# Atticuszz/GsplatLoc

Hardware: AMD Instinct MI355X
Metric: Gaussians/s fwd+bwd @1M splats 1200x680 (higher is better)
Workload: dtype f32

## Files before the change

gsplatloc_amd/_lib.py:

```python
from __future__ import annotations

import ctypes
import os
import subprocess
from ctypes import c_char_p, c_double, c_float, c_int, c_int64, c_size_t, c_void_p
from typing import Optional

_HERE = os.path.dirname(os.path.abspath(__file__))
_LIB_PATH = os.path.join(_HERE, "libgsloc_hip.so")
_lib: Optional[ctypes.CDLL] = None

P = c_void_p

_SIGNATURES = {
    "gsl_version": (c_char_p, []),
    "gsl_status_string": (c_char_p, [c_int]),
    "gsl_dev_poison_lds": (c_int, [ctypes.c_uint32, P]),
    "gsl_dev_tile_sort_launches": (c_int64, [c_int]),
    "gsl_project_fwd": (c_int, [P, P, P, P, P, c_int, c_int, c_int, c_float, c_float, c_float, c_float,
                                P, P, P, P, P, P]),
    "gsl_project_bwd_ws_bytes": (c_size_t, [c_int]),
    "gsl_project_bwd": (c_int, [P, P, P, P, P, c_int, c_int, c_int, c_float, P, P, P, P, P, P, P, P, P, P, P,
                                P, c_size_t, P]),
    "gsl_project_packed_ws_bytes": (c_size_t, [c_int, c_int]),
# ... 45 lines not shown
    "gsl_map_pose_align_batch": (c_int, [P, c_int64, P, c_int, c_float, c_float, c_float, c_float, P, c_int, c_int,
                                         c_float, c_float, c_float, c_float, c_int, c_double, c_int, c_double, c_double,
                                         c_double, c_double, P, P, P, P, P]),
    "gsl_map_photo_intensity": (c_int, [P, c_int, c_int, P, P]),
    "gsl_map_info_photo_max_rows": (c_int64, [c_float, c_float, c_float, c_float, c_int, c_int, c_float, c_float,
                                              c_float]),
    "gsl_map_pose_info_photo": (c_int, [P, c_int64, P, c_float, c_float, c_float, c_float, P, c_int, c_int, c_float,
                                        c_float, c_float, c_float, P, P, P, c_float, c_float, P, P]),
    "gsl_map_pose_align_photo": (c_int, [P, c_int64, P, c_float, c_float, c_float, c_float, P, c_int, c_int, c_float,
                                         c_float, c_float, c_float, c_int, c_double, c_int, c_double, c_double, c_double,
                                         c_double, P, P, P, P, P, P, c_float, c_float, P]),
    "gsl_map_pose_align_batch_photo": (c_int, [P, c_int64, P, c_int, c_float, c_float, c_float, c_float, P, c_int, c_int,
                                               c_float, c_float, c_float, c_float, c_int, c_double, c_int, c_double,
                                               c_double, c_double, c_double, P, P, P, P, P, P, c_float, c_float, P]),
    "gsl_map_pyramid_floats": (c_int64, [c_int, c_int, c_int]),
    "gsl_map_pyramid": (c_int, [P, P, c_int, c_int, c_int, c_float, P, P, P]),
    "gsl_map_place_cells": (c_int, []),
    "gsl_map_place_describe": (c_int, [P, c_int, c_int, P, P]),
    "gsl_map_place_match": (c_int, [P, P, c_int, P, P]),
    "gsl_map_refine": (c_int, [P, P, P, c_int64, P, c_float, c_float, c_float, c_float, c_float, c_float, c_float, P, P,
                               c_int, c_int, c_float, c_float, c_int, P, P]),
    "gsl_map_correct": (c_int, [P, P, c_int64, P, c_int, P, P]),
    "gsl_map_covis": (c_int, [P, P, c_int64, P, c_float, c_float, c_float, c_float, P, c_int, c_int, c_float, c_float,
                              c_float, c_int, P, P, P]),
    "gsl_sh_fwd": (c_int, [c_int, P, P, P, c_int, c_int, P, P]),
    "gsl_sh_bwd": (c_int, [c_int, P, P, P, c_int, c_int, P, P, P, P]),
    "gsl_isect_ws_bytes": (c_size_t, [c_int]),
    "gsl_isect_count": (c_int, [P, P, c_int, c_int, c_int, c_int, c_int, c_int, P, P, P, P, c_size_t, P]),
    "gsl_isect_fill": (c_int, [P, P, P, c_int, c_int, c_int, c_int, c_int, c_int, c_int, c_int, P, c_int64,
                               P, P, P, P, c_size_t, P]),
    "gsl_tile_sort": (c_int, [P, c_int, c_int, c_int64, P, P, P, c_int64, P]),
    "gsl_fused_ws_bytes": (c_size_t, [c_int, c_int]),
    "gsl_fused_project": (c_int, [P, P, P, P, P, c_int, c_int, P, P, c_int, c_int, c_int, c_float, c_float, c_float,
                                  c_float, c_int, c_int, c_int, c_int, c_int, P, P, P, P, P, P, P, P, P, c_size_t,
                                  P, P, c_int, P, P, P]),
    "gsl_fused_bin": (c_int, [P, P, c_int, c_int, c_int, c_int, c_int, c_int, P, c_int64, P, P, P, P, c_size_t, c_int,
                              P, c_int, P, P, c_int, P, P, P]),
    "gsl_fused_bin_clear": (c_int, [P, P, c_int, c_int, c_int, c_int, c_int, c_int, P, c_int64, P, P, P, P, c_size_t, c_int,
                                    P, c_int, P, P, c_int, P, P, P, P]),
    "gsl_fused_clear_rows": (c_int, [P, c_int, P]),
    "gsl_long_sort": (c_int, [P, c_int, c_int, c_int, c_int, c_int64, P, c_int, P, P, c_int, P, c_size_t, c_int, c_int, P,
                              P]),
    "gsl_fused_raster_fwd": (c_int, [P, P, P, c_int, c_int, c_int, c_int, c_int, c_int, c_int, c_int, P, P, c_int64,
                                     P, P, P, c_int, c_int, P, P, P, P, c_int, P, c_int, P, P, P, P]),
    "gsl_fused_raster_bwd": (c_int, [P, P, P, c_int, c_int, c_int, c_int, c_int, c_int, c_int, c_int, P, P, c_int64,
                                     P, P, P, P, P, P, c_int, c_int, P, P, P, P, c_int, P, P]),
    "gsl_long_ws_bytes": (c_size_t, [c_int]),
    "gsl_long_segment": (c_int, []),
    "gsl_long_sort_segment": (c_int, []),
    "gsl_long_raster_fwd": (c_int, [P, P, P, c_int, c_int, c_int, c_int, c_int, c_int, c_int, c_int, P, P, c_int64,
                                    P, P, P, c_int, c_int, P, P, c_int, P, c_size_t, c_int, c_int, P]),
    "gsl_long_raster_bwd": (c_int, [P, P, P, c_int, c_int, c_int, c_int, c_int, c_int, c_int, c_int, P, P, c_int64,
                                    P, P, P, P, P, P, c_int, c_int, P, P, c_int, P, c_int, P]),
    "gsl_loss_ws_bytes": (c_size_t, [c_int, c_int]),
    "gsl_loss_n_partials": (c_int, [c_int, c_int, c_int, c_int]),
    "gsl_tracking_loss": (c_int, [P, c_int, P, c_int, c_int, c_int, c_int, c_float, c_float, P, P, P, P, c_size_t,
                                  P]),
    "gsl_pose_init": (c_int, [P, P, P, c_float, c_float, P, P, P]),
    "gsl_normal_ws_bytes": (c_size_t, [c_int, c_int]),
    "gsl_normal_loss": (c_int, [P, c_int, P, c_int, c_int, c_int, c_int, c_float, c_float, c_float, c_float, c_float,
                                P, P, P, c_size_t, P]),
    "gsl_fused_viewmat_rows": (P, [P, c_int]),
    "gsl_pose_step": (c_int, [P, P, P, P, c_int, P, P, c_int, P, P, P, c_int, c_int, c_float, c_float, c_float, c_double, c_double,
                              c_float, c_float, c_float, c_double, c_int, c_int, c_int, c_int, P, P, P, P]),
    "gsl_pack_pose_reduce": (c_int, [P, P, c_int, P, P, P, c_int, P, P, P]),
    "gsl_photo_ws_bytes": (c_size_t, [c_int, c_int]),
    "gsl_photo_loss": (c_int, [P, c_int, P, c_int, c_int, c_float, c_float, P, P, P, c_size_t, P]),
    "gsl_pose_step_photo": (c_int, [P, P, P, P, c_int, P, P, c_int, P, P, P, c_int, c_int, c_float, c_float, c_float,
                                    c_double, c_double, c_float, c_float, c_float, c_double, c_int, c_int, c_int, c_int,
                                    P, P, P, P, P, c_float, c_float]),
    "gsl_pose_step_best": (c_int, [P, P, P, P, c_int, P, P, c_int, P, P, P, c_int, c_int, c_float, c_float, c_float,
                                   c_double, c_double, c_float, c_float, c_float, c_double, c_int, c_int, c_int, c_int,
                                   P, P, P, P, P, c_float, c_float, P]),
    "gsl_knn_ws_bytes": (c_size_t, [c_int]),
    "gsl_knn_cells": (c_int, []),
    "gsl_knn_count": (c_int, [P, c_int, P, P, c_size_t, P]),
    "gsl_knn_query": (c_int, [P, c_int, P, P, c_int, P, P, c_size_t, P]),
    "gsl_fused_project_bwd": (c_int, [P, P, P, P, P, c_int, c_int, P, P, c_int, c_int, c_int, c_float, c_int, c_int,
                                      P, P, P, P, P, P, P, P, P, P, P, c_size_t, c_int, P, P, P, P, c_int, c_int,
                                      c_int, c_int, c_int64, P, P, c_int, P, P]),
    "gsl_fused_project_bwd_keep": (c_int, [P, P, P, P, P, c_int, c_int, P, P, c_int, c_int, c_int, c_float, c_int, c_int,
                                           P, P, P, P, P, P, P, P, P, P, P, c_size_t, c_int, P, P, P, P, c_int, c_int,
                                           c_int, c_int, c_int64, P, P, c_int, P, P]),
    "gsl_tiny_raster_bwd": (c_int, [P, P, P, c_int, c_int, c_int, c_int, c_int, c_int, c_int, c_int, P, P, c_int64,
                                    P, P, P, P, P, P, P, c_int, c_int, P, c_int, P, c_float, c_float, P, P, P]),
    "gsl_isect_emit": (c_int, [P, P, P, P, c_int, c_int, c_int, c_int, c_int, c_int, c_int, P, P, P]),
    "gsl_isect_offsets": (c_int, [P, c_int64, c_int, c_int, c_int, P, P]),
    "gsl_rasterize_fwd": (c_int, [P, P, P, P, P, c_int, c_int, c_int, c_int, c_int, c_int, c_int, c_int, P, P,
                                  c_int64, P, P, P, P, P]),
    "gsl_vacc_bytes": (c_size_t, [c_int, c_int]),
    "gsl_rasterize_bwd": (c_int, [P, P, P, P, P, c_int, c_int, c_int, c_int, c_int, c_int, c_int, c_int, P, P,
                                  c_int64, P, P, P, P, P, P, P]),
    "gsl_vacc_unpack": (c_int, [P, c_int, c_int, P, P, P, P, P]),
    "gsl_fused_absgrad": (c_int, [P, P, P, c_int, c_int, c_int, c_int, c_int, c_int, P, P, c_int64, P, P, P, P, P, P,
                                  P, P, P]),
    "gsl_rasterize_absgrad": (c_int, [P, P, P, P, P, c_int, c_int, c_int, c_int, c_int, c_int, P, P, c_int64, P, P,
                                      P, P, P, P, P]),
}


def library_path() -> str:
    return _LIB_PATH


def exported_symbols():
    return sorted(_SIGNATURES)


def build_library(force: bool = False, verbose: bool = False) -> str:
    csrc = os.path.join(_HERE, "csrc")
    cmd = ["make", "-C", csrc, "-j", str(min(8, os.cpu_count() or 1)), "all"]
    if force:
        subprocess.run(["make", "-C", csrc, "clean"], check=True, capture_output=not verbose)
    res = subprocess.run(cmd, capture_output=True, text=True)
    if verbose or res.returncode != 0:
        print(res.stdout)
        print(res.stderr)
    if res.returncode != 0:
        raise RuntimeError("building libgsloc_hip.so failed:\n" + res.stderr[-4000:])
    return _LIB_PATH


def load_library() -> ctypes.CDLL:
    global _lib
    if _lib is not None:
        return _lib
    if not os.path.exists(_LIB_PATH):
        raise RuntimeError(
            f"{_LIB_PATH} not found: the HIP extension is required (no CPU fallback). "
            "Run `python -c 'import __graft_entry__ as g; g.build()'` or `make -C gsplatloc_amd/csrc`."
        )
    lib = ctypes.CDLL(_LIB_PATH)
    for name, (res, args) in _SIGNATURES.items():
        fn = getattr(lib, name)
        fn.restype = res
        fn.argtypes = args
    _lib = lib
    return lib


def check(status: int, what: str) -> None:
    if status != 0:
        msg = load_library().gsl_status_string(status).decode()
        raise RuntimeError(f"{what} failed: {msg} (status {status})")


def ptr(t) -> Optional[int]:
    return None if t is None else t.data_ptr()


def current_stream() -> int:
    import torch

    raw = getattr(torch._C, "_cuda_getCurrentRawStream", None)
    if raw is not None:
        return raw(torch.cuda.current_device())
    return torch.cuda.current_stream().cuda_stream
```

gsplatloc_amd/context.py:

```python
from __future__ import annotations

import math
import os
from typing import Dict, Optional, Tuple

import torch
from torch import Tensor

from . import stages
from ._lib import check, current_stream, load_library, ptr
from .stages import _MODES, MAX_STRIP_TILES, alloc_records, tile_n_bits


LONG_MIN = 2048
BIN_BYTES_MAX = 2 << 30
TINY_RCULL_MAX = 1.999
TINY_MAX_N = 400_000
FP16_EPS2D_MIN = 2e-5


class RenderContext:
    def __init__(self, N: int, width: int, height: int, render_mode: str = "RGB+ED", sh_degree: Optional[int] = 1,
                 K_sh: int = 4, device="cuda", eps2d: float = 0.3, near_plane: float = 0.01, far_plane: float = 1e10,
                 radius_clip: float = 0.0, antialiased: bool = False, tile_rows: Optional[Tuple[int, int]] = None,
                 capacity: Optional[int] = None, full_grads: bool = True,
                 pixel_rows: Optional[Tuple[int, int]] = None, staging: str = "fp32", deterministic: bool = False,
                 sort_in_forward: bool = False, reorder: Optional[bool] = None):
        if staging == "fp16" and not float(eps2d) >= FP16_EPS2D_MIN:
            raise ValueError(f"staging='fp16' needs eps2d >= {FP16_EPS2D_MIN} (got {eps2d}): the conic of a degenerate "
                             f"splat reaches 1/eps2d, and the half records end at 65504")
        self.lib = load_library()
        self.reorder = reorder
        self.order_ids = self.storage_of = None
        self._placed = None
        self._placed_key = None
        self._placed_src = None
        self.sort_in_forward = bool(sort_in_forward)
        self.N, self.W, self.H = int(N), int(width), int(height)
        self.mode = render_mode
        self.D, self.ed = _MODES[render_mode]
        self.rgb = self.D >= 3
        self.sh_degree = -1 if sh_degree is None else int(sh_degree)
        self.K_sh = int(K_sh) if (self.rgb and self.sh_degree >= 0) else 0
        self.eps2d, self.near, self.far, self.radius_clip = float(eps2d), float(near_plane), float(far_plane), float(radius_clip)
        self.antialiased = bool(antialiased)
        self.tw, self.th = (self.W + 15) // 16, (self.H + 15) // 16
        self.n_tiles = self.tw * self.th
        self.ty0, self.ty1 = tile_rows if tile_rows is not None else (0, self.th)
        assert 0 <= self.ty0 <= self.ty1 <= self.th
        assert (self.ty1 - self.ty0) * self.tw <= MAX_STRIP_TILES, "strip too large for the LDS tile histogram"
        lo, hi = self.ty0 * 16, min(self.ty1 * 16, self.H)
        self.row0, self.row1 = pixel_rows if pixel_rows is not None else (lo, hi)
        assert lo <= self.row0 <= self.row1 <= hi or self.ty0 == self.ty1, (pixel_rows, tile_rows)
        self.full_grads = bool(full_grads)
        dev = torch.device(device)
        self.device = dev
        f32, i32 = torch.float32, torch.int32
        N = self.N
        self.radii = torch.zeros(N, dtype=i32, device=dev)
        self.Q0, self.Q1, self.Q2 = alloc_records(N, self.rgb, dev, zero=True)
        assert staging in ("fp32", "fp16"), staging
        self.staging = staging
        self.Qh = torch.zeros(N, 8, dtype=i32, device=dev) if staging == "fp16" else None
        self.deterministic = bool(deterministic)
        self.vrow = None
        self.comps = torch.zeros(N, dtype=f32, device=dev) if self.antialiased else None
        self.offs = torch.zeros(self.n_tiles + 1, dtype=i32, device=dev)
        self.status = torch.zeros(8, dtype=i32, device=dev)
        self.n_is = self.status[4:5]
        self.hit_counts = torch.zeros(4 * self.n_tiles + 1, dtype=i32, device=dev)
        self.ws_bytes = self.lib.gsl_fused_ws_bytes(N, self.n_tiles)
        self.ws = torch.zeros(self.ws_bytes, dtype=torch.uint8, device=dev)
        self.render = torch.zeros(self.H, self.W, self.D, dtype=f32, device=dev)
        self.alphas = torch.zeros(self.H, self.W, 1, dtype=f32, device=dev)
        self.last_ids = torch.zeros(self.H, self.W, dtype=i32, device=dev)
        self.vacc = torch.zeros(N, 16, dtype=f32, device=dev)
        self._rows_dirty = False
        self._sort_cleared = False
        self.v_viewmat = torch.zeros(4, 4, dtype=f32, device=dev)
        if self.full_grads:
            self.v_means = torch.zeros(N, 3, dtype=f32, device=dev)
            self.v_quats = torch.zeros(N, 4, dtype=f32, device=dev)
            self.v_scales = torch.zeros(N, 3, dtype=f32, device=dev)
            self.v_opacities = torch.zeros(N, dtype=f32, device=dev)
            if self.rgb:
                shape = (N, self.K_sh, 3) if self.sh_degree >= 0 else (N, 3)
                self.v_colors = torch.zeros(*shape, dtype=f32, device=dev)
                self.vc_state = torch.ones(1, dtype=i32, device=dev)
            else:
                self.v_colors = None
        else:
            self.v_means = self.v_quats = self.v_scales = self.v_opacities = self.v_colors = None
        if not hasattr(self, "vc_state"):
            self.vc_state = None
        self.capacity = 0
        self.tiny = False
        self.flags = self.status[0:4]
        self.last_n_isects = 0
        self.tiles_per_gauss = None
        self.record_hits = True
        self.generation = 0
        self.bins, self.bin_cap = None, 0
        self._counters_dirty = False
        self._hits_valid = False
        self.trec = self.vcT = None
        self.long_min, self.max_seg, self.long_ws, self.long_ws_bytes, self.long_passes = 0, 0, None, 0, 0
        self._mean_list = 0.0
        self.keys = self.flatten_ids = self.hits = None
        if capacity is not None:
            self._alloc_isects(int(capacity))
        self._inputs = None

    def _alloc_isects(self, capacity: int) -> None:
        self.capacity = max(int(capacity), 1)
        self.keys = torch.zeros(self.capacity, dtype=torch.int64, device=self.device)
        self.flatten_ids = torch.zeros(self.capacity, dtype=torch.int32, device=self.device)
        self.hits = (torch.zeros(4 * self.capacity, dtype=torch.int32, device=self.device)
                     if self.capacity < (1 << 28) else None)
        if self.deterministic:
            self.vrow = torch.zeros(self.capacity, 16, dtype=torch.float32, device=self.device)

    def calibrate(self, means, quats, scales, opacities, colors, viewmat, K, headroom: float = 1.3) -> int:
        self.bins, self.bin_cap = None, 0
        self.order_ids = self.storage_of = self._placed = self._placed_key = self._placed_src = None
        self._project(means, quats, scales, opacities, colors, viewmat, K)
        if self._choose_placement():
            self._project(*self._place(means, quats, scales, opacities, colors), viewmat, K)
        n = int(self.n_is.item())
        self._alloc_isects(int(n * headroom) + 1024)
        sizes = (self.offs[1:] - self.offs[:-1]) if self.n_tiles else self.offs[:0]
        longest = int(sizes.max()) if self.n_tiles else 0
        self._alloc_bins(int(longest * max(headroom, 1.5)) + 64)
        self._choose_backward()
        self._alloc_long(sizes, headroom)
        return n

    REORDER_MIN_N = 65536
    REORDER_MAX_N = 1_500_000

    def _choose_placement(self) -> bool:
        want = self.reorder
        if want is None:
            want = (os.environ.get("GSLOC_REORDER", "1") != "0" and self.REORDER_MIN_N <= self.N <= self.REORDER_MAX_N
                    and not self.deterministic and not self._screen_coherent_order())
        if not want or self.N < 2:
            return False
        assert not self.deterministic, "deterministic mode finds a Gaussian's rows by key: no tile-order placement"
        vis = self.Q1[:, 3] > 0
        tx = torch.clamp(torch.floor(self.Q0[:, 0] / 16.0), 0, self.tw - 1).to(torch.int64)
        ty = torch.clamp(torch.floor(self.Q0[:, 1] / 16.0), 0, self.th - 1).to(torch.int64)
        tile = torch.where(vis, ty * self.tw + tx, torch.full_like(tx, self.n_tiles))
        perm = torch.sort(tile, stable=True).indices
        self.order_ids = perm.to(torch.int32).contiguous()
        self.storage_of = torch.empty_like(self.order_ids)
        self.storage_of[perm] = torch.arange(self.N, dtype=torch.int32, device=self.device)
        self._perm64 = perm.contiguous()
        return True

    def _place(self, means, quats, scales, opacities, colors):
# ... 142 lines not shown
                self.ws.zero_()
            self._counters_dirty = True
        stages.fused_project(means, quats, scales, opacities, colors if self.rgb else None, self.sh_degree, self.K_sh,
                             viewmat, K, self.N, self.W, self.H, self.eps2d, self.near, self.far, self.radius_clip,
                             int(self.antialiased), self.tw, self.th, self.ty0, self.ty1, self.radii, self.Q0, self.Q1,
                             self.Q2, self.comps, self.tiles_per_gauss, self.offs, self.n_is, self.ws, Qh=self.Qh,
                             bins=self.bins, bin_cap=self.bin_cap, flags=self.flags, order_ids=self.order_ids)

    def _bin(self) -> None:
        self._sort_cleared = False
        if self.sorts_in_forward():
            return
        args = (self.Q0, self.radii, self.N, self.tw, self.th, self.ty0, self.ty1, tile_n_bits(self.n_tiles), self.offs,
                self.capacity, self.keys, self.flatten_ids, self.ws)
        modes = dict(write_sorted_keys=int(self.deterministic), bins=self.bins, bin_cap=self.bin_cap, n_isects=self.n_is,
                     flags=self.flags, long_min=self.long_min if self.bins is not None else 0, order_ids=self.order_ids,
                     storage_of=self.storage_of)
        if self.sort_clears_rows():
            stages.fused_bin_clear(*args, self.vacc, **modes)
            self._rows_dirty, self._sort_cleared = False, True
        else:
            stages.fused_bin(*args, **modes)
        if self.long_min and self.bins is not None:
            stages.long_sort(self.offs, self.tw, self.th, self.ty0, self.ty1, self.capacity, self.bins, self.bin_cap,
                             self.keys, self.flatten_ids, self.long_min, self.long_ws, self.max_seg, self.long_passes,
                             storage_of=self.storage_of)

    def _frame(self) -> tuple:
        return (self.Q0, self.Q1, self.Q2, self.D, int(self.ed), self.W, self.H, self.tw, self.th, self.ty0, self.ty1,
                self.offs, self.flatten_ids, self.capacity, self.render, self.alphas, self.last_ids)

    def _raster_fwd(self) -> None:
        sif = self.sorts_in_forward()
        hits = self.hits if self.record_hits else None
        own_sort = dict(sort_bins=self.bins, bin_cap=self.bin_cap, n_isects=self.n_is, flags=self.flags,
                        storage_of=self.storage_of) if sif else {}
        stages.fused_raster_fwd(*self._frame(), self.row0, self.row1, Qh=self.Qh,
                                binned_ws=self.ws if self.bins is not None else None, isect_hits=hits,
                                isect_hit_counts=self.hit_counts if hits is not None else None,
                                long_min=self.long_min, **own_sort)
        if not sif:
            self._counters_dirty = False
        self._hits_valid = hits is not None
        if self.long_min:
            stages.long_raster_fwd(*self._frame(), self.row0, self.row1, self.long_min, self.long_ws, self.max_seg,
                                   int(self.bins is not None), Qh=self.Qh, isect_hits=hits)

    def _raster_bwd(self, v_render: Tensor, v_alphas: Tensor, tracking_loss=None) -> None:
        common = self._frame() + (v_render, v_alphas)
        clear = self.sorts_in_forward() and self._counters_dirty
        clear_ws = self.ws if clear else None
        hits = self.hits if self._hits_valid else None
        if self._rows_dirty:
            stages.fused_clear_rows(self.vacc, self.N)
            self._rows_dirty = False
        if self.tiny:
            depth_gt, depth_lambda, edge_lambda, partials = tracking_loss if tracking_loss is not None else (None, 0, 0, None)
            stages.tiny_raster_bwd(*common, self.trec, self.vcT, self.row0, self.row1, flags=self.flags,
                                   long_min=self.long_min, loss_depth_gt=depth_gt, depth_lambda=float(depth_lambda),
                                   edge_lambda=float(edge_lambda), loss_partials=partials, clear_ws=clear_ws)
        else:
            stages.fused_raster_bwd(*common, self.vacc, self.row0, self.row1, Qh=self.Qh, vrow=self.vrow, isect_hits=hits,
                                    isect_hit_counts=self.hit_counts if self._hits_valid else None,
                                    long_min=self.long_min, clear_ws=clear_ws)
        if clear:
            self._counters_dirty = False
        if self.long_min:
            stages.long_raster_bwd(*common, self.vacc, self.row0, self.row1, self.long_min, self.long_ws, self.max_seg,
                                   Qh=self.Qh, isect_hits=hits)

    def _project_bwd(self, full: bool, reduce: bool = True) -> None:
        means, quats, scales, opacities, colors, viewmat, K = self._inputs
        mode = {}
        if self.tiny:
            mode = dict(Q0=self.Q0, tiny_trec=self.trec, tiny_vcT=self.vcT)
        elif self.vrow is not None:
            mode = dict(vrow=self.vrow, sorted_keys=self.keys, tile_offsets=self.offs, Q0=self.Q0, tile_w=self.tw,
                        tile_h=self.th, ty0=self.ty0, ty1=self.ty1, capacity=self.capacity)
        grads = (self.v_means, self.v_quats, self.v_scales, self.v_opacities) if full else (None, None, None, None)
        project_bwd = stages.fused_project_bwd
        if self._sort_cleared and self.sort_clears_rows():
            project_bwd = stages.fused_project_bwd_keep
            self._rows_dirty = True
        project_bwd(means, quats, scales, opacities, colors if self.rgb else None, self.sh_degree, self.K_sh, viewmat, K,
                    self.N, self.W, self.H, self.eps2d, int(self.antialiased), self.D, self.radii, self.Q1, self.comps,
                    self.vacc if (not self.tiny or self.long_min) else None, *grads,
                    self.v_colors if (full and self.rgb) else None, self.v_viewmat, self.ws, self.n_tiles, int(reduce),
                    v_colors_state=self.vc_state if (full and self.rgb) else None, **mode)

    def forward(self, means: Tensor, quats: Tensor, scales: Tensor, opacities: Tensor, colors: Optional[Tensor],
                viewmat: Tensor, K: Tensor) -> Tuple[Tensor, Tensor]:
        assert self.keys is not None, "call calibrate() (or pass capacity=) before forward()"
        means, quats, scales, opacities, colors = self._place(means, quats, scales, opacities, colors)
        self._project(means, quats, scales, opacities, colors, viewmat, K)
        self._bin()
        self._raster_fwd()
        self._inputs = (means, quats, scales, opacities, colors, viewmat, K)
        self.generation += 1
        return self.render, self.alphas

    def forward_checked(self, means, quats, scales, opacities, colors, viewmat, K) -> Optional[str]:
        assert self.keys is not None, "call calibrate() (or pass capacity=) before forward()"
        means, quats, scales, opacities, colors = self._place(means, quats, scales, opacities, colors)
        self._project(means, quats, scales, opacities, colors, viewmat, K)
        self._bin()
        why = self.overflow_status()
        if why is not None:
            return why
        self._raster_fwd()
        self._inputs = (means, quats, scales, opacities, colors, viewmat, K)
        self.generation += 1
        return None

    def overflow_status(self) -> Optional[str]:
        st = self.status.tolist()
        self.last_n_isects = min(int(st[4]), self.capacity)
        if st[4] > self.capacity:
            return f"intersection capacity exceeded ({st[4]} > {self.capacity})"
        if self.bins is not None and st[1]:
            return f"a tile list outgrew its bin ({st[2]} > {self.bin_cap})"
        if self.bins is not None and st[3]:
            return "tile counters were not cleared"
        if self.tiny and st[0]:
            return "a splat outgrew the tiny-splat backward"
        if self.long_ws is not None and self.long_overflowed():
            return "long tile lists outgrew their workspace"
        return None

    def can_fuse_tracking_loss(self) -> bool:
        return bool(self.tiny and self.ty0 == 0 and self.ty1 == self.th and self.row0 == 0 and self.row1 >= self.H
                    and self.D in (1, 4))

    def backward(self, v_render: Tensor, v_alphas: Tensor, full: Optional[bool] = None,
                 reduce_viewmat: bool = True, tracking_loss=None) -> Dict[str, Tensor]:
        assert self._inputs is not None, "forward() first"
        full = self.full_grads if full is None else full
        assert not full or self.full_grads, "context was built with full_grads=False"
        assert tracking_loss is None or self.can_fuse_tracking_loss()
        self._raster_bwd(v_render, v_alphas, tracking_loss)
        self._project_bwd(full, reduce_viewmat)
        out = {"viewmat": self.v_viewmat}
        if full:
            out.update(means=self.v_means, quats=self.v_quats, scales=self.v_scales, opacities=self.v_opacities,
                       colors=self.v_colors)
        return out

    def render_autograd(self, means, quats, scales, opacities, colors, viewmat, K) -> Tuple[Tensor, Tensor]:
        return _CtxRender.apply(self, means, quats, scales, opacities, colors, viewmat, K)


class _CtxRender(torch.autograd.Function):
    @staticmethod
    def forward(ctx, rc: RenderContext, means, quats, scales, opacities, colors, viewmat, K):
        render, alphas = rc.forward(means, quats, scales, opacities, colors, viewmat, K)
        ctx.rc = rc
        ctx.mark_non_differentiable()
        return render, alphas

    @staticmethod
    def backward(ctx, v_render, v_alphas):
        rc = ctx.rc
        ni = ctx.needs_input_grad
        full = rc.full_grads and any(ni[1:6])
        g = rc.backward(v_render.contiguous(), v_alphas.contiguous(), full=full)
        if full:
            g = rc.grads_in_input_order(g)
        return (None, g["means"] if (full and ni[1]) else None, g["quats"] if (full and ni[2]) else None,
                g["scales"] if (full and ni[3]) else None, g["opacities"] if (full and ni[4]) else None,
# ... 39 lines not shown
```

gsplatloc_amd/csrc/fused_project.hip:

```cpp
#include "gsloc_internal.h"
#include "project_dev.h"
#include "sh_dev.h"
#include "tile_dev.h"

namespace gsl {

__device__ __forceinline__ float cull_radius(float ca, float cb, float cc, float op) {
  float tau = __logf(255.f * op) * 1.01f + 0.01f;
  float det = ca * cc - cb * cb;
  if (!(tau > 0.f)) return -1.f;
  if (!(det > 0.f) || !(ca > 0.f) || !(cc > 0.f)) return 1e30f;
  float hd = 0.5f * (ca - cc);
  float root = sqrtf(hd * hd + cb * cb);
  float lmin = det / (0.5f * (ca + cc) + root);
  if (!(lmin > 0.f)) return 1e30f;
  return sqrtf(2.f * tau / lmin) * 1.0001f + 1e-3f;
}

template <bool RGB, bool BINNED>
__global__ __launch_bounds__(GSL_BIN_THREADS) void k_fproject(
    const float* __restrict__ means, const float* __restrict__ quats, const float* __restrict__ scales,
    const float* __restrict__ opacities, const float* __restrict__ colors, int sh_degree, int K_sh,
    const float* __restrict__ V, const float* __restrict__ Kmat, int N, int W, int H, float eps2d, float near_plane,
    float far_plane, float radius_clip, int antialiased, int tile_w, int tile_h, int ty0, int ty1,
    int32_t* __restrict__ radii, float4* __restrict__ Q0, float4* __restrict__ Q1, float4* __restrict__ Q2,
    float* __restrict__ comps, int32_t* __restrict__ tiles_per_gauss, int32_t* __restrict__ tile_counts,
    uint4* __restrict__ Qh, uint64_t* __restrict__ bins, int bin_cap, int32_t* __restrict__ bin_state,
    int32_t* __restrict__ flags, const int32_t* __restrict__ order_ids) {
  extern __shared__ int s_hist[];
  int nst = (ty1 - ty0) * tile_w, tbase = ty0 * tile_w;
  if (BINNED && bin_state && nst > 0 && blockIdx.x == 0 && threadIdx.x == 0) {
    if (atomicExch(bin_state, 1) != 0 && flags) flags[3] = 1;
  }
  int* const s_rng = s_hist + nst;
  for (int k = threadIdx.x; k < nst; k += GSL_BIN_THREADS) s_hist[k] = 0;
  if (threadIdx.x == 0) { s_rng[0] = nst; s_rng[1] = -1; }
  __syncthreads();
  int i = blockIdx.x * GSL_BIN_THREADS + threadIdx.x;
  Cam cam = load_cam(V, Kmat);
  int xmin = 0, ymin = 0, xmax = 0, ymax = 0;
  uint64_t key = 0;
  if (i < N) {
    ProjMid p;
    float q[4], s[3];
    load_gaussian(means, quats, scales, i, cam, p, q, s);
    float op_in = opacities[i];
    float shc[12];
#pragma unroll
    for (int k = 0; k < 12; ++k) shc[k] = 0.f;
    if (RGB) {
      if (sh_degree < 0) {
#pragma unroll
        for (int k = 0; k < 3; ++k) shc[k] = colors[3 * (size_t)i + k];
      } else {
        const float* cf = colors + (size_t)i * K_sh * 3;
#pragma unroll
        for (int k = 0; k < 3; ++k) shc[k] = cf[k];
        if (sh_degree >= 1) {
#pragma unroll
          for (int k = 3; k < 12; ++k) shc[k] = cf[k];
        }
      }
    }
    asm volatile("" : "+v"(p.mean[0]), "+v"(p.mean[1]), "+v"(p.mean[2]), "+v"(q[0]), "+v"(q[1]), "+v"(q[2]), "+v"(q[3]),
                 "+v"(s[0]), "+v"(s[1]), "+v"(s[2]), "+v"(op_in), "+v"(shc[0]), "+v"(shc[1]), "+v"(shc[2]), "+v"(shc[3]),
                 "+v"(shc[4]), "+v"(shc[5]), "+v"(shc[6]), "+v"(shc[7]), "+v"(shc[8]), "+v"(shc[9]), "+v"(shc[10]),
                 "+v"(shc[11]));
    int radius = 0;
    float4 o0 = make_float4(0.f, 0.f, 0.f, 0.f), o1 = make_float4(0.f, 0.f, 0.f, -1.f);
    float comp = 0.f;
    if (p.mc[2] >= near_plane && p.mc[2] <= far_plane) {
      p.covar = quat_scale_to_covar(q, s);
      p.covar_c = mul_bt(mul(cam.R, p.covar), cam.R);
      persp_mid(cam, W, H, p);
      float a, b, c;
      cov2d_from(p.J, p.covar_c, a, b, c);
      float det_orig = a * c - b * b;
      a += eps2d;
      c += eps2d;
      float det = a * c - b * b;
      if (det > 0.f) {
        float bb = 0.5f * (a + c);
        float v1 = bb + sqrtf(fmaxf(0.01f, bb * bb - det));
        float rad = ceilf(3.f * sqrtf(v1));
        float mx = cam.fx * p.mc[0] * p.rz + cam.cx;
        float my = cam.fy * p.mc[1] * p.rz + cam.cy;
        bool ok = rad > radius_clip;
        ok = ok && !(mx + rad <= 0.f || mx - rad >= (float)W || my + rad <= 0.f || my - rad >= (float)H);
        if (ok) {
          float inv = 1.f / det;
          radius = (int)rad;
          comp = sqrtf(fmaxf(0.f, det_orig / det));
          float op = op_in;
          if (antialiased) op *= comp;
          float ca = c * inv, cb = -b * inv, cc = a * inv;
          o0 = make_float4(mx, my, p.mc[2], op);
          o1 = make_float4(ca, cb, cc, cull_radius(ca, cb, cc, op));
        }
      }
    }
    radii[i] = radius;
    GSL_Q(Q0, i) = o0;
    GSL_Q(Q1, i) = o1;
    if (comps) comps[i] = comp;
    float c0 = 0.f, c1 = 0.f, c2 = 0.f;
    if (RGB) {
      if (sh_degree < 0) {
        c0 = shc[0]; c1 = shc[1]; c2 = shc[2];
      } else {
        if (radius > 0) {
          M3 Ri;
          float cp[3];
          cam_inverse(cam, Ri, cp);
          float x = p.mean[0] - cp[0], y = p.mean[1] - cp[1], z = p.mean[2] - cp[2];
          float inorm = rsqrtf(x * x + y * y + z * z);
          float Y[16];
          sh_basis(sh_degree, x * inorm, y * inorm, z * inorm, Y);
          int nK = (sh_degree + 1) * (sh_degree + 1);
          const float* cf = colors + (size_t)i * K_sh * 3;
#pragma unroll
          for (int k = 0; k < 4; ++k)
            if (k < nK) { c0 += Y[k] * shc[3 * k]; c1 += Y[k] * shc[3 * k + 1]; c2 += Y[k] * shc[3 * k + 2]; }
          for (int k = 4; k < nK; ++k) {
            c0 += Y[k] * cf[3 * k]; c1 += Y[k] * cf[3 * k + 1]; c2 += Y[k] * cf[3 * k + 2];
          }
        }
        c0 = fmaxf(c0 + 0.5f, 0.f); c1 = fmaxf(c1 + 0.5f, 0.f); c2 = fmaxf(c2 + 0.5f, 0.f);
      }
      if (!Qh) GSL_Q(Q2, i) = make_float4(c0, c1, c2, 0.f);
    }
    if (Qh) store_half_record(Qh, (size_t)i, o0, o1, make_float4(c0, c1, c2, 0.f));
    if (radius > 0) {
      strip_rect(o0.x, o0.y, radius, 16, tile_w, tile_h, ty0, ty1, xmin, ymin, xmax, ymax);
      key = ((uint64_t)__float_as_uint(o0.z) << 32) | (uint32_t)(order_ids ? order_ids[i] : i);
    }
    if (tiles_per_gauss) tiles_per_gauss[i] = (xmax - xmin) * (ymax - ymin);
  }
  {
    const bool has = (ymin < ymax) && (xmin < xmax);
    int lo = has ? ymin * tile_w + xmin - tbase : nst, hi = has ? (ymax - 1) * tile_w + (xmax - 1) - tbase : -1;
#pragma unroll
    for (int o = 32; o >= 1; o >>= 1) {
      lo = min(lo, __shfl_xor(lo, o, 64));
      hi = max(hi, __shfl_xor(hi, o, 64));
    }
    if ((threadIdx.x & 63) == 0 && hi >= 0) { atomicMin(&s_rng[0], lo); atomicMax(&s_rng[1], hi); }
  }
  for (int y = ymin; y < ymax; ++y)
    for (int x = xmin; x < xmax; ++x) atomicAdd(&s_hist[y * tile_w + x - tbase], 1);
  __syncthreads();
  const int k_lo = __builtin_amdgcn_readfirstlane(s_rng[0]), k_hi = __builtin_amdgcn_readfirstlane(s_rng[1]);
  if (!BINNED) {
    for (int k = k_lo + (int)threadIdx.x; k <= k_hi; k += GSL_BIN_THREADS) {
      int c = s_hist[k];
      if (c) atomicAdd(&tile_counts[tbase + k], c);
    }
    return;
  }
  int res[GSL_MAX_STRIP_TILES / GSL_BIN_THREADS];
#pragma unroll
  for (int u = 0; u < GSL_MAX_STRIP_TILES / GSL_BIN_THREADS; ++u) {
    res[u] = 0;
    if (k_lo + u * GSL_BIN_THREADS <= k_hi) {
      int k = k_lo + (int)threadIdx.x + u * GSL_BIN_THREADS;
      int c = (k <= k_hi) ? s_hist[k] : 0;
      res[u] = c ? atomicAdd(&tile_counts[tbase + k], c) : 0;
    }
  }
#pragma unroll
  for (int u = 0; u < GSL_MAX_STRIP_TILES / GSL_BIN_THREADS; ++u) {
    if (k_lo + u * GSL_BIN_THREADS <= k_hi) {
      int k = k_lo + (int)threadIdx.x + u * GSL_BIN_THREADS;
      if (k <= k_hi && s_hist[k]) s_hist[k] = res[u];
    }
  }
  __syncthreads();
  for (int y = ymin; y < ymax; ++y)
    for (int x = xmin; x < xmax; ++x) {
      int lt = y * tile_w + x - tbase;
      int slot = atomicAdd(&s_hist[lt], 1);
      if (slot < bin_cap) bins[(size_t)(tbase + lt) * (size_t)bin_cap + slot] = key;
    }
}

}

extern "C" size_t gsl_fused_ws_bytes(int N, int n_tiles) {
  size_t nb = ((size_t)(N > 0 ? N : 1) + 255) / 256;
  return gsl::fused_vm_rows_offset(n_tiles > 0 ? n_tiles : 1) + (nb + GSL_VM_STAGE_ROWS) * 16 * sizeof(float);
}

extern "C" const float* gsl_fused_viewmat_rows(const void* ws, int n_tiles) {
  if (!ws || n_tiles <= 0) return nullptr;
  return (const float*)((const char*)ws + gsl::fused_vm_rows_offset(n_tiles));
}

extern "C" int gsl_fused_project(const float* means, const float* quats, const float* scales, const float* opacities,
                                 const float* colors, int sh_degree, int K_sh, const float* viewmat, const float* K,
                                 int N, int width, int height, float eps2d, float near_plane, float far_plane,
                                 float radius_clip, int antialiased, int tile_w, int tile_h, int ty0, int ty1,
                                 int32_t* radii, float* Q0, float* Q1, float* Q2, float* compensations,
                                 int32_t* tiles_per_gauss, int32_t* tile_offsets, int32_t* n_isects, void* ws,
                                 size_t ws_bytes, void* Qh, void* bins, int bin_cap, int32_t* flags,
                                 const int32_t* order_ids, void* stream) {
  if (N < 0 || width <= 0 || height <= 0 || tile_w <= 0 || tile_h <= 0 || ty0 < 0 || ty1 > tile_h || ty0 > ty1)
    return GSL_ERR_BAD_ARG;
  if (N > GSL_MAX_GAUSSIANS) return GSL_ERR_BAD_ARG;
  if (tile_w * 16 < width || tile_h * 16 < height) return GSL_ERR_BAD_ARG;
  int n_tiles = tile_w * tile_h, nst = (ty1 - ty0) * tile_w;
  if (nst > GSL_MAX_STRIP_TILES) return GSL_ERR_BAD_ARG;
  if (!viewmat || !K || !tile_offsets || !n_isects) return GSL_ERR_BAD_ARG;
  if (N > 0 && (!means || !quats || !scales || !opacities || !radii || !Q0 || !Q1)) return GSL_ERR_BAD_ARG;
  if (Q2 && !colors) return GSL_ERR_BAD_ARG;
  if (Q2 && sh_degree >= 0 && (sh_degree > 3 || K_sh < (sh_degree + 1) * (sh_degree + 1))) return GSL_ERR_BAD_ARG;
  if (antialiased && !compensations) return GSL_ERR_BAD_ARG;
  if (!ws || ws_bytes < gsl_fused_ws_bytes(N, n_tiles)) return GSL_ERR_WORKSPACE;
  if (bins && bin_cap <= 0) return GSL_ERR_BAD_ARG;
  hipStream_t st = (hipStream_t)stream;
  int32_t* counts = (int32_t*)ws;
  int32_t* cursors = counts + n_tiles;
  GSL_CLAMP_DEPTH_WINDOW(near_plane, far_plane);
  if (!bins && gsl::zero_u32(counts, (size_t)n_tiles, st) != GSL_OK) return GSL_ERR_HIP;
  if (N > 0) {
    dim3 grid((N + GSL_BIN_THREADS - 1) / GSL_BIN_THREADS), block(GSL_BIN_THREADS);
    size_t lds = (size_t)(nst + 2) * sizeof(int);
#define CALL_P(RGBV, BINV)                                                                                            \
  hipLaunchKernelGGL((gsl::k_fproject<RGBV, BINV>), grid, block, lds, st, means, quats, scales, opacities, colors,    \
                     sh_degree, K_sh, viewmat, K, N, width, height, eps2d, near_plane, far_plane, radius_clip,        \
                     antialiased, tile_w, tile_h, ty0, ty1, radii, (float4*)Q0, (float4*)Q1, (float4*)Q2,             \
                     compensations, tiles_per_gauss, counts, (uint4*)Qh, (uint64_t*)bins, bin_cap,                   \
                     bins ? gsl::fused_bin_state(ws, n_tiles) : (int32_t*)nullptr, flags, order_ids)
    if (Q2) { if (bins) CALL_P(true, true); else CALL_P(true, false); }
    else { if (bins) CALL_P(false, true); else CALL_P(false, false); }
#undef CALL_P
    GSL_CHECK_LAUNCH();
  }
  if (bins) return GSL_OK;
  gsl::launch_tile_scan(st, counts, n_tiles, tile_offsets, n_isects, cursors);
  GSL_CHECK_LAUNCH();
  return GSL_OK;
}

namespace gsl {
static int fused_bin(const float* Q0, const int32_t* radii, int N, int tile_w, int tile_h, int ty0, int ty1,
                     int32_t* tile_offsets, int64_t capacity, uint64_t* sort_keys, int32_t* flatten_ids,
                     int64_t* isect_ids, void* ws, size_t ws_bytes, int write_sorted_keys, void* bins, int bin_cap,
                     int32_t* n_isects, int32_t* flags, int long_min, const int32_t* order_ids,
                     const int32_t* storage_of, bool clear, float* rows, void* stream) {
  if (N < 0 || tile_w <= 0 || tile_h <= 0 || ty0 < 0 || ty1 > tile_h || ty0 > ty1 || capacity < 0)
    return GSL_ERR_BAD_ARG;
  if (clear && (N > GSL_MAX_GAUSSIANS || (N > 0 && !rows))) return GSL_ERR_BAD_ARG;
  if (!clear || N == 0) rows = nullptr;
  const int n_rows = rows ? N : 0;
  int n_tiles = tile_w * tile_h, nst = (ty1 - ty0) * tile_w;
  if (nst > GSL_MAX_STRIP_TILES || !tile_offsets) return GSL_ERR_BAD_ARG;
  if (bins) {
    if (bin_cap <= 0 || !n_isects) return GSL_ERR_BAD_ARG;
    if (!ws || ws_bytes < gsl_fused_ws_bytes(N, n_tiles)) return GSL_ERR_WORKSPACE;
    if (capacity > 0 && (!sort_keys || !flatten_ids)) return GSL_ERR_BAD_ARG;
    return gsl::tile_sort_keys(tile_offsets, 0, n_tiles, capacity, sort_keys, flatten_ids, isect_ids, 0,
                               write_sorted_keys, (uint64_t*)bins, bin_cap, (const int32_t*)ws, n_isects, flags,
                               write_sorted_keys ? 0 : long_min, nst, storage_of, rows, n_rows, stream);
  }
  if (N == 0 || capacity == 0 || nst == 0)
    return rows ? gsl::zero_u32(rows, (size_t)16 * (size_t)N, (hipStream_t)stream) : GSL_OK;
  if (!Q0 || !radii || !sort_keys || !flatten_ids) return GSL_ERR_BAD_ARG;
  if (!ws || ws_bytes < gsl_fused_ws_bytes(N, n_tiles)) return GSL_ERR_WORKSPACE;
  hipStream_t st = (hipStream_t)stream;
  int32_t* cursors = (int32_t*)ws + n_tiles;
  gsl::launch_record_scatter(st, Q0, radii, order_ids, N, tile_w, tile_h, ty0, ty1, tile_offsets, cursors,
                             (long long)capacity, sort_keys);
  GSL_CHECK_LAUNCH();
  return gsl::tile_sort_keys(tile_offsets, ty0 * tile_w, nst, capacity, sort_keys, flatten_ids, isect_ids, 0,
                             write_sorted_keys, nullptr, 0, nullptr, nullptr, nullptr, 0, 0, storage_of, rows, n_rows,
                             stream);
}
}

extern "C" int gsl_fused_bin(const float* Q0, const int32_t* radii, int N, int tile_w, int tile_h, int ty0, int ty1,
                             int tile_n_bits, int32_t* tile_offsets, int64_t capacity, uint64_t* sort_keys,
                             int32_t* flatten_ids, int64_t* isect_ids, void* ws, size_t ws_bytes,
                             int write_sorted_keys, void* bins, int bin_cap, int32_t* n_isects, int32_t* flags,
                             int long_min, const int32_t* order_ids, const int32_t* storage_of, void* stream) {
  (void)tile_n_bits;
  return gsl::fused_bin(Q0, radii, N, tile_w, tile_h, ty0, ty1, tile_offsets, capacity, sort_keys, flatten_ids, isect_ids,
                        ws, ws_bytes, write_sorted_keys, bins, bin_cap, n_isects, flags, long_min, order_ids, storage_of,
                        false, nullptr, stream);
}

extern "C" int gsl_fused_bin_clear(const float* Q0, const int32_t* radii, int N, int tile_w, int tile_h, int ty0, int ty1,
                                   int tile_n_bits, int32_t* tile_offsets, int64_t capacity, uint64_t* sort_keys,
                                   int32_t* flatten_ids, int64_t* isect_ids, void* ws, size_t ws_bytes,
                                   int write_sorted_keys, void* bins, int bin_cap, int32_t* n_isects, int32_t* flags,
                                   int long_min, const int32_t* order_ids, const int32_t* storage_of, float* rows,
                                   void* stream) {
  (void)tile_n_bits;
  return gsl::fused_bin(Q0, radii, N, tile_w, tile_h, ty0, ty1, tile_offsets, capacity, sort_keys, flatten_ids, isect_ids,
                        ws, ws_bytes, write_sorted_keys, bins, bin_cap, n_isects, flags, long_min, order_ids, storage_of,
                        true, rows, stream);
}

extern "C" int gsl_fused_clear_rows(float* rows, int N, void* stream) {
  if (N < 0 || (N > 0 && !rows)) return GSL_ERR_BAD_ARG;
  return gsl::zero_u32(rows, (size_t)16 * (size_t)N, (hipStream_t)stream);
}
```

gsplatloc_amd/csrc/fused_project_bwd.hip:

```cpp
#include "gsloc_internal.h"
#include "pose_dev.h"
#include "project_dev.h"
#include "sh_dev.h"
#include "tile_dev.h"
#include "tiny_dev.h"

namespace gsl {

template <bool FULL, int D, bool KEEP>
__global__ __launch_bounds__(256) void k_fproject_bwd(
    const float* __restrict__ means, const float* __restrict__ quats, const float* __restrict__ scales,
    const float* __restrict__ opacities, const float* __restrict__ colors, int sh_degree, int K_sh,
    const float* __restrict__ V, const float* __restrict__ Kmat, int N, int W, int H, float eps2d, int antialiased,
    const int32_t* __restrict__ radii, const float4* __restrict__ Q1, const float* __restrict__ comps,
    float4* __restrict__ vacc, float* __restrict__ v_means, float* __restrict__ v_quats,
    float* __restrict__ v_scales, float* __restrict__ v_opacities, float* __restrict__ v_colors,
    float* __restrict__ partials, const float4* __restrict__ vrow, const uint64_t* __restrict__ skeys,
    const int32_t* __restrict__ tile_offsets, const float4* __restrict__ Q0, int tile_w, int tile_h, int ty0, int ty1,
    long long capacity, float4* __restrict__ trec, const float* __restrict__ vcT, int32_t* __restrict__ vc_state) {
  constexpr bool RGB = D >= 3;
  int i = blockIdx.x * 256 + threadIdx.x;
  Cam cam = load_cam(V, Kmat);
  const bool vc_zero = FULL && RGB && vc_state && *vc_state == 1;
  __shared__ float4 srow[256][3];
  if (trec) {
#pragma unroll 1
    for (int half = 0; half < 2; ++half) {
      TinySlabIn in[2];
#pragma unroll
      for (int u = 0; u < 2; ++u) {
        int t = (2 * half + u) * 256 + threadIdx.x;
        in[u] = tiny_slab_load(radii, Q0, Q1, trec, blockIdx.x * 256 + (t >> 2), t & 3, N);
      }
      GSL_TINY_SLAB_PIN(in[0]);
      GSL_TINY_SLAB_PIN(in[1]);
#pragma unroll
      for (int u = 0; u < 2; ++u) {
        int t = (2 * half + u) * 256 + threadIdx.x;
        int lg = t >> 2, r = t & 3, gid = blockIdx.x * 256 + lg;
        float v[6 + D];
        tiny_slab_fold<D>(in[u], W, H, trec, vcT, gid, r, v);
        float pad[12];
#pragma unroll
        for (int k = 0; k < 12; ++k) pad[k] = (k < 6 + D) ? v[k] : 0.f;
        if (r == 0) srow[lg][0] = make_float4(pad[0], pad[1], pad[2], pad[3]);
        if (r == 1) srow[lg][1] = make_float4(pad[4], pad[5], pad[6], pad[7]);
        if (r == 2) srow[lg][2] = make_float4(pad[8], pad[9], pad[10], pad[11]);
      }
    }
    __syncthreads();
  }
  float acc15[15];
#pragma unroll
  for (int k = 0; k < 15; ++k) acc15[k] = 0.f;
  float vmean[3] = {0.f, 0.f, 0.f}, vq[4] = {0.f, 0.f, 0.f, 0.f}, vs[3] = {0.f, 0.f, 0.f};
  float vop = 0.f;
  float vrgb[3] = {0.f, 0.f, 0.f};
  bool live = (i < N) && (radii[i] > 0);
  bool sh_live = false;
  if (live) {
    float4 r0, r1, r2;
    float4 z = make_float4(0.f, 0.f, 0.f, 0.f);
    if (vrow) {
      r0 = r1 = r2 = z;
      float4 q0 = GSL_Q(Q0, i);
      int xmin, ymin, xmax, ymax;
      tile_rect(q0.x, q0.y, radii[i], 16, tile_w, tile_h, xmin, ymin, xmax, ymax);
      ymin = max(ymin, ty0);
      ymax = min(ymax, ty1);
      uint64_t want = ((uint64_t)__float_as_uint(q0.z) << 32) | (uint32_t)i;
      for (int y = ymin; y < ymax; ++y)
        for (int x = xmin; x < xmax; ++x) {
          long long lo = tile_offsets[y * tile_w + x], hi = tile_offsets[y * tile_w + x + 1];
          if (hi > capacity) hi = capacity;
          while (lo < hi) {
            long long mid = (lo + hi) >> 1;
            if (skeys[mid] < want) lo = mid + 1; else hi = mid;
          }
          if (lo < capacity && skeys[lo] == want) {
            float4 a = vrow[4 * lo], b = vrow[4 * lo + 1], c = vrow[4 * lo + 2];
            r0.x += a.x; r0.y += a.y; r0.z += a.z; r0.w += a.w;
            r1.x += b.x; r1.y += b.y; r1.z += b.z; r1.w += b.w;
            r2.x += c.x; r2.y += c.y; r2.z += c.z; r2.w += c.w;
          }
        }
    } else if (trec) {
      r0 = srow[threadIdx.x][0]; r1 = srow[threadIdx.x][1]; r2 = srow[threadIdx.x][2];
      if (vacc) {
        float4 a = vacc[4 * (size_t)i], b = vacc[4 * (size_t)i + 1], c = vacc[4 * (size_t)i + 2];
        if (a.x != 0.f || a.y != 0.f || a.z != 0.f || a.w != 0.f || b.x != 0.f || b.y != 0.f || b.z != 0.f || b.w != 0.f ||
            c.x != 0.f || c.y != 0.f || c.z != 0.f || c.w != 0.f) {
          r0.x += a.x; r0.y += a.y; r0.z += a.z; r0.w += a.w;
          r1.x += b.x; r1.y += b.y; r1.z += b.z; r1.w += b.w;
          r2.x += c.x; r2.y += c.y; r2.z += c.z; r2.w += c.w;
          vacc[4 * (size_t)i] = z; vacc[4 * (size_t)i + 1] = z; vacc[4 * (size_t)i + 2] = z;
        }
      }
    } else {
      r0 = vacc[4 * (size_t)i]; r1 = vacc[4 * (size_t)i + 1]; r2 = vacc[4 * (size_t)i + 2];
      if (!KEEP) { vacc[4 * (size_t)i] = z; vacc[4 * (size_t)i + 1] = z; vacc[4 * (size_t)i + 2] = z; }
    }
    float vm2x = r0.x, vm2y = r0.y, v_ca = r0.z, v_cb = r0.w, v_cc = r1.x, vop_eff = r1.y;
    float col[4] = {r1.z, r1.w, r2.x, r2.y};
    float vdepth = (D == 1) ? col[0] : ((D == 4) ? col[3] : 0.f);
    if (RGB) { vrgb[0] = col[0]; vrgb[1] = col[1]; vrgb[2] = col[2]; }
    float comp = 0.f, vcomp = 0.f;
    vop = vop_eff;
    if (antialiased) {
      comp = comps[i];
      vcomp = vop_eff * opacities[i];
      vop = vop_eff * comp;
    }
    ProjMid p;
    float q[4], s[3];
    load_gaussian(means, quats, scales, i, cam, p, q, s);
    p.covar = quat_scale_to_covar(q, s);
    p.covar_c = mul_bt(mul(cam.R, p.covar), cam.R);
    persp_mid(cam, W, H, p);
    float4 q1 = GSL_Q(Q1, i);
    project_vjp<FULL>(cam, eps2d, p, q, s, q1.x, q1.y, q1.z, vm2x, vm2y, vdepth, v_ca, v_cb, v_cc, antialiased != 0,
                      comp, vcomp, acc15, vmean, vq, vs);
    sh_live = RGB && (sh_degree >= 0) && (vrgb[0] != 0.f || vrgb[1] != 0.f || vrgb[2] != 0.f);
    if (sh_live) {
      M3 Ri;
      float cp[3];
      cam_inverse(cam, Ri, cp);
      float rx = p.mean[0] - cp[0], ry = p.mean[1] - cp[1], rz = p.mean[2] - cp[2];
      float inorm = rsqrtf(rx * rx + ry * ry + rz * rz);
      float x = rx * inorm, y = ry * inorm, zz = rz * inorm;
      float Y[16];
      sh_basis(sh_degree, x, y, zz, Y);
      int nK = (sh_degree + 1) * (sh_degree + 1);
      const float* cf = colors + (size_t)i * K_sh * 3;
      float c0 = 0.5f, c1 = 0.5f, c2 = 0.5f;
      for (int k = 0; k < nK; ++k) {
        c0 += Y[k] * cf[3 * k]; c1 += Y[k] * cf[3 * k + 1]; c2 += Y[k] * cf[3 * k + 2];
      }
      if (!(c0 > 0.f)) vrgb[0] = 0.f;
      if (!(c1 > 0.f)) vrgb[1] = 0.f;
      if (!(c2 > 0.f)) vrgb[2] = 0.f;
      float sk[16];
      for (int k = 0; k < nK; ++k) {
        sk[k] = cf[3 * k] * vrgb[0] + cf[3 * k + 1] * vrgb[1] + cf[3 * k + 2] * vrgb[2];
        if (FULL) {
          if (k == 0 && vc_state) *vc_state = 2;
          v_colors[((size_t)i * K_sh + k) * 3] = Y[k] * vrgb[0];
          v_colors[((size_t)i * K_sh + k) * 3 + 1] = Y[k] * vrgb[1];
          v_colors[((size_t)i * K_sh + k) * 3 + 2] = Y[k] * vrgb[2];
        }
      }
      if (FULL)
        for (int k = nK * 3; k < K_sh * 3; ++k) v_colors[(size_t)i * K_sh * 3 + k] = 0.f;
      float g[3];
      sh_basis_grad(sh_degree, x, y, zz, sk, g);
      float dd = g[0] * x + g[1] * y + g[2] * zz;
      float gd[3] = {(g[0] - dd * x) * inorm, (g[1] - dd * y) * inorm, (g[2] - dd * zz) * inorm};
#pragma unroll
      for (int k = 0; k < 3; ++k) {
        vmean[k] += gd[k];
        acc15[12 + k] = -gd[k];
      }
    }
  }
  if (FULL && i < N) {
#pragma unroll
    for (int k = 0; k < 3; ++k) v_means[3 * (size_t)i + k] = vmean[k];
#pragma unroll
    for (int k = 0; k < 4; ++k) v_quats[4 * (size_t)i + k] = vq[k];
#pragma unroll
    for (int k = 0; k < 3; ++k) v_scales[3 * (size_t)i + k] = vs[k];
    v_opacities[i] = vop;
    if (RGB && !sh_live) {
      if (sh_degree < 0) {
        const bool nz = vrgb[0] != 0.f || vrgb[1] != 0.f || vrgb[2] != 0.f;
        if (nz && vc_state) *vc_state = 2;
        if (nz || !vc_zero) {
          v_colors[3 * (size_t)i] = vrgb[0]; v_colors[3 * (size_t)i + 1] = vrgb[1]; v_colors[3 * (size_t)i + 2] = vrgb[2];
        }
      } else if (!vc_zero) {
        if (K_sh == 4) {
          float4* dst = reinterpret_cast<float4*>(v_colors + (size_t)i * 12);
          float4 z4 = make_float4(0.f, 0.f, 0.f, 0.f);
          dst[0] = z4; dst[1] = z4; dst[2] = z4;
        } else {
          for (int k = 0; k < K_sh * 3; ++k) v_colors[(size_t)i * K_sh * 3 + k] = 0.f;
        }
      }
    }
  }
  if (partials != nullptr) {
    __shared__ float red[4][15];
    int lane = threadIdx.x & 63, wv = threadIdx.x >> 6;
#pragma unroll
    for (int k = 0; k < 15; ++k) {
      float sum = wave_sum(acc15[k]);
      if (lane == 0) red[wv][k] = sum;
    }
    __syncthreads();
    if (threadIdx.x < 15)
      partials[(size_t)blockIdx.x * 16 + threadIdx.x] =
          red[0][threadIdx.x] + red[1][threadIdx.x] + red[2][threadIdx.x] + red[3][threadIdx.x];
  }
}

__global__ __launch_bounds__(256) void k_freduce_rows(const float* __restrict__ partials, int nb, float* __restrict__ out) {
  __shared__ float red[4][16];
  int span = (nb + (int)gridDim.x - 1) / (int)gridDim.x;
  int r0 = blockIdx.x * span, r1 = min(nb, r0 + span);
  int q = threadIdx.x & 3;
  const float4* rows = reinterpret_cast<const float4*>(partials) + q;
  float4 a = make_float4(0.f, 0.f, 0.f, 0.f);
  for (int b = r0 + (threadIdx.x >> 2); b < r1; b += 64) {
    float4 x = rows[(size_t)b * 4];
    a.x += x.x; a.y += x.y; a.z += x.z; a.w += x.w;
  }
  float v4[4] = {a.x, a.y, a.z, a.w};
  int lane = threadIdx.x & 63, wv = threadIdx.x >> 6;
#pragma unroll
  for (int c = 0; c < 4; ++c) {
    float x = v4[c];
#pragma unroll
    for (int o = 4; o < 64; o <<= 1) x += __shfl_xor(x, o, 64);
    if (lane < 4) red[wv][4 * q + c] = x;
  }
  __syncthreads();
  if (threadIdx.x < 16)
    out[(size_t)blockIdx.x * 16 + threadIdx.x] =
        threadIdx.x < 15 ? (red[0][threadIdx.x] + red[1][threadIdx.x]) + (red[2][threadIdx.x] + red[3][threadIdx.x]) : 0.f;
}

__global__ __launch_bounds__(1024) void k_freduce_viewmat(const float* __restrict__ partials, int nb,
                                                         const float* __restrict__ V, const float* __restrict__ Kmat,
                                                         float* __restrict__ v_viewmat, int32_t* __restrict__ vc_state) {
  __shared__ float red[16][15];
  __shared__ float tot[15];
  float v = reduce_viewmat_rows_wide(partials, nb, V, Kmat, red, tot);
  if (threadIdx.x < 16) v_viewmat[threadIdx.x] = v;
  if (vc_state && threadIdx.x == 0) *vc_state = (*vc_state == 2) ? 0 : 1;
}

static int fused_project_bwd(const float* means, const float* quats, const float* scales, const float* opacities,
                             const float* colors, int sh_degree, int K_sh, const float* viewmat, const float* K, int N,
                             int width, int height, float eps2d, int antialiased, int channels, const int32_t* radii,
                             const float* Q1, const float* compensations, float* vacc, float* v_means, float* v_quats,
                             float* v_scales, float* v_opacities, float* v_colors, float* v_viewmat, void* ws,
                             size_t ws_bytes, int n_tiles, const float* vrow, const uint64_t* sorted_keys,
                             const int32_t* tile_offsets, const float* Q0, int tile_w, int tile_h, int ty0, int ty1,
                             int64_t capacity, float* tiny_trec, const float* tiny_vcT, int reduce_viewmat,
                             int32_t* v_colors_state, bool keep, void* stream) {
  if (N < 0 || width <= 0 || height <= 0 || n_tiles <= 0) return GSL_ERR_BAD_ARG;
  if (keep && (vrow || tiny_trec || (N > 0 && !vacc))) return GSL_ERR_BAD_ARG;
  if (reduce_viewmat && !v_viewmat) return GSL_ERR_BAD_ARG;
  if (channels != 1 && channels != 3 && channels != 4) return GSL_ERR_BAD_ARG;
  bool full = v_means != nullptr;
  if (full != (v_quats != nullptr) || full != (v_scales != nullptr) || full != (v_opacities != nullptr))
    return GSL_ERR_BAD_ARG;
  if (full && channels >= 3 && !v_colors) return GSL_ERR_BAD_ARG;
  if (antialiased && !compensations) return GSL_ERR_BAD_ARG;
  hipStream_t st = (hipStream_t)stream;
  if (N == 0) {
    if (reduce_viewmat && gsl::zero_u32(v_viewmat, 16, st) != GSL_OK) return GSL_ERR_HIP;
    return GSL_OK;
  }
  if (!means || !quats || !scales || !opacities || !viewmat || !K || !radii || !Q1) return GSL_ERR_BAD_ARG;
  if (!vrow && !vacc && !tiny_trec) return GSL_ERR_BAD_ARG;
  if (tiny_trec && (!tiny_vcT || !Q0 || vrow)) return GSL_ERR_BAD_ARG;
  if (vrow && (!sorted_keys || !tile_offsets || !Q0 || tile_w <= 0 || tile_h <= 0 || tile_w * tile_h != n_tiles ||
               ty0 < 0 || ty1 > tile_h || ty0 > ty1 || capacity < 0))
    return GSL_ERR_BAD_ARG;
  if (channels >= 3 && !colors) return GSL_ERR_BAD_ARG;
  if (!ws || ws_bytes < gsl_fused_ws_bytes(N, n_tiles)) return GSL_ERR_WORKSPACE;
  float* partials = (float*)((char*)ws + gsl::fused_vm_rows_offset(n_tiles));
  int grid = (N + 255) / 256;
  int32_t* vcs = (full && channels >= 3) ? v_colors_state : nullptr;
#define CALL_PB(FF, DD)                                                                                               \
  do {                                                                                                                \
    auto kern = keep ? gsl::k_fproject_bwd<FF, DD, true> : gsl::k_fproject_bwd<FF, DD, false>;                        \
    hipLaunchKernelGGL(kern, dim3(grid), dim3(256), 0, st, means, quats, scales, opacities, colors, sh_degree, K_sh,  \
                       viewmat, K, N, width, height, eps2d, antialiased, radii, (const float4*)Q1, compensations,     \
                       (float4*)vacc, v_means, v_quats, v_scales, v_opacities, v_colors, partials,                    \
                       (const float4*)vrow, sorted_keys, tile_offsets, (const float4*)Q0, tile_w, tile_h, ty0, ty1,   \
                       (long long)capacity, (float4*)tiny_trec, tiny_vcT, vcs);                                       \
  } while (0)
  if (full) {
    if (channels == 1) CALL_PB(true, 1); else if (channels == 3) CALL_PB(true, 3); else CALL_PB(true, 4);
  } else {
    if (channels == 1) CALL_PB(false, 1); else if (channels == 3) CALL_PB(false, 3); else CALL_PB(false, 4);
  }
#undef CALL_PB
  GSL_CHECK_LAUNCH();
  if (reduce_viewmat) {
    if (grid > 8192) {
      float* stage = partials + (size_t)grid * 16;
      hipLaunchKernelGGL(gsl::k_freduce_rows, dim3(GSL_VM_STAGE_ROWS), dim3(256), 0, st, partials, grid, stage);
      hipLaunchKernelGGL(gsl::k_freduce_viewmat, dim3(1), dim3(1024), 0, st, stage, GSL_VM_STAGE_ROWS, viewmat, K, v_viewmat, vcs);
    } else {
      hipLaunchKernelGGL(gsl::k_freduce_viewmat, dim3(1), dim3(1024), 0, st, partials, grid, viewmat, K, v_viewmat, vcs);
    }
    GSL_CHECK_LAUNCH();
  }
  return GSL_OK;
}
}

#define GSL_PROJECT_BWD_PARAMS                                                                                         \
  const float *means, const float *quats, const float *scales, const float *opacities, const float *colors,           \
      int sh_degree, int K_sh, const float *viewmat, const float *K, int N, int width, int height, float eps2d,       \
      int antialiased, int channels, const int32_t *radii, const float *Q1, const float *compensations, float *vacc,  \
      float *v_means, float *v_quats, float *v_scales, float *v_opacities, float *v_colors, float *v_viewmat,         \
      void *ws, size_t ws_bytes, int n_tiles, const float *vrow, const uint64_t *sorted_keys,                         \
      const int32_t *tile_offsets, const float *Q0, int tile_w, int tile_h, int ty0, int ty1, int64_t capacity,       \
      float *tiny_trec, const float *tiny_vcT, int reduce_viewmat, int32_t *v_colors_state, void *stream
#define GSL_PROJECT_BWD_ARGS(KEEP)                                                                                    \
  means, quats, scales, opacities, colors, sh_degree, K_sh, viewmat, K, N, width, height, eps2d, antialiased,         \
      channels, radii, Q1, compensations, vacc, v_means, v_quats, v_scales, v_opacities, v_colors, v_viewmat, ws,     \
      ws_bytes, n_tiles, vrow, sorted_keys, tile_offsets, Q0, tile_w, tile_h, ty0, ty1, capacity, tiny_trec,          \
      tiny_vcT, reduce_viewmat, v_colors_state, KEEP, stream
extern "C" int gsl_fused_project_bwd(GSL_PROJECT_BWD_PARAMS) {
  return gsl::fused_project_bwd(GSL_PROJECT_BWD_ARGS(false));
}
extern "C" int gsl_fused_project_bwd_keep(GSL_PROJECT_BWD_PARAMS) {
  return gsl::fused_project_bwd(GSL_PROJECT_BWD_ARGS(true));
}
#undef GSL_PROJECT_BWD_PARAMS
#undef GSL_PROJECT_BWD_ARGS
```

gsplatloc_amd/csrc/gsloc_internal.h:

```cpp
#pragma once
#include "gsloc_common.h"

namespace gsl {

struct LongWs;
struct InfoPhoto;

int zero_u32(void* p, size_t n_dwords, hipStream_t st);

void launch_count_scan(hipStream_t st, const uint32_t* counts, int nb, uint32_t* bases, int32_t* total);

void launch_tile_scan(hipStream_t st, int32_t* counts, int n_tiles, int32_t* tile_offsets, int32_t* n_isects,
                      int32_t* cursors);
void launch_record_scatter(hipStream_t st, const float* Q0, const int32_t* radii, const int32_t* order_ids, int N,
                           int tile_w, int tile_h, int ty0, int ty1, const int32_t* tile_offsets, int32_t* cursors,
                           long long capacity, uint64_t* keys);

int tile_sort_keys(int32_t* tile_offsets, int tile_begin, int n_strip_tiles, int64_t capacity, uint64_t* sort_keys,
                   int32_t* flatten_ids, int64_t* isect_ids, int64_t cam_enc, int write_sorted_keys, uint64_t* bins,
                   int bin_cap, const int32_t* counts, int32_t* n_isects, int32_t* flags, int long_min, int occupied_tiles,
                   const int32_t* storage_of, float* clear_rows, int clear_n, void* stream);

void launch_long_map(hipStream_t st, const int32_t* tile_offsets, int tile_begin, int n_strip_tiles, long long capacity,
                     int long_min, int max_seg, int max_list, const LongWs& w);

int launch_mraster_bwd(const float* Q0, const float* Q1, const float* Q2, int channels, int ed, int width, int height,
                       int tile_w, int ty0, int ty1, const int32_t* tile_offsets, const int32_t* flatten_ids,
                       int64_t capacity, const float* render, const float* alphas, const int32_t* last_ids,
                       const float* v_render, const float* v_alphas, float* vrow, int row0, int row1, const void* Qh,
                       hipStream_t st);

int map_pose_info_launch(const float* means, int64_t n_rows, const float* w2c, float fx, float fy, float cx, float cy,
                         const float* depth, int width, int height, float keep, float beyond, float kappa,
                         float near_plane, int64_t* out, hipStream_t st);

int map_pose_info_photo_launch(const float* means, int64_t n_rows, const float* w2c, float fx, float fy, float cx,
                               float cy, const float* depth, int width, int height, float keep, float beyond,
                               float kappa, float near_plane, int64_t* out, const InfoPhoto& photo, int64_t* extra,
                               hipStream_t st);

#define GSL_VM_STAGE_ROWS 64
static inline size_t fused_vm_rows_offset(int n_tiles) { return ((size_t)2 * (size_t)n_tiles * sizeof(int32_t) + 15) & ~(size_t)15; }
static inline int32_t* fused_bin_state(void* ws, int n_tiles) {
  return (ws && n_tiles > 0) ? (int32_t*)((char*)ws + fused_vm_rows_offset(n_tiles)) + 15 : nullptr;
}

static inline bool frame_ok(int width, int height, int tile_w, int tile_h, int ty0, int ty1, int64_t capacity, int row0,
                            int row1, bool cover = true) {
  if (width <= 0 || height <= 0 || tile_w <= 0 || tile_h <= 0 || ty0 < 0 || ty1 > tile_h || ty0 > ty1 || capacity < 0 ||
      row0 < 0 || row0 > row1)
    return false;
  return !cover || (tile_w * 16 >= width && tile_h * 16 >= height);
}
static inline bool records_ok(const void* Qh, const float* Q0, const float* Q1, const float* Q2, int channels) {
  return Qh || (Q0 && Q1 && (channels < 3 || Q2));
}
static inline bool ed_ok(int channels, int ed) { return !(ed && channels == 3); }

}

#define GSL_DISPATCH_CH_ED(D, ED, CALL)                            \
  if (D == 1) { if (ED) CALL(1, true); else CALL(1, false); }      \
  else if (D == 3) { CALL(3, false); }                             \
  else if (D == 4) { if (ED) CALL(4, true); else CALL(4, false); } \
  else return GSL_ERR_BAD_ARG;
```

gsplatloc_amd/csrc/project_dev.h:

```cpp
#pragma once
#include "gsloc_common.h"

namespace gsl {

struct ProjOut {
  float mx, my, depth;
  float ca, cb, cc;
  float comp;
  int radius;
};

struct ProjMid {
  float mean[3];
  float mc[3];
  M3 covar;
  M3 covar_c;
  float J[6];
  float tx, ty, rz;
  bool x_in, y_in;
};

__device__ __forceinline__ void persp_mid(const Cam& cam, int W, int H, ProjMid& p) {
  float x = p.mc[0], y = p.mc[1], z = p.mc[2];
  float lim_x = 1.3f * (0.5f * (float)W / cam.fx);
  float lim_y = 1.3f * (0.5f * (float)H / cam.fy);
  float rz = 1.f / z;
  float rz2 = rz * rz;
  float xr = x * rz, yr = y * rz;
  p.x_in = (xr <= lim_x) && (xr >= -lim_x);
  p.y_in = (yr <= lim_y) && (yr >= -lim_y);
  p.tx = z * fminf(lim_x, fmaxf(-lim_x, xr));
  p.ty = z * fminf(lim_y, fmaxf(-lim_y, yr));
  p.rz = rz;
  p.J[0] = cam.fx * rz; p.J[1] = 0.f; p.J[2] = -cam.fx * p.tx * rz2;
  p.J[3] = 0.f; p.J[4] = cam.fy * rz; p.J[5] = -cam.fy * p.ty * rz2;
}

__device__ __forceinline__ void cov2d_from(const float J[6], const M3& Sc, float& a, float& b, float& c) {
  float r0[3], r1[3];
#pragma unroll
  for (int j = 0; j < 3; ++j) {
    r0[j] = J[0] * Sc(0, j) + J[1] * Sc(1, j) + J[2] * Sc(2, j);
    r1[j] = J[3] * Sc(0, j) + J[4] * Sc(1, j) + J[5] * Sc(2, j);
  }
  a = r0[0] * J[0] + r0[1] * J[1] + r0[2] * J[2];
  b = r0[0] * J[3] + r0[1] * J[4] + r0[2] * J[5];
  c = r1[0] * J[3] + r1[1] * J[4] + r1[2] * J[5];
}

__device__ __forceinline__ void load_gaussian(const float* __restrict__ means, const float* __restrict__ quats,
                                              const float* __restrict__ scales, int i, const Cam& cam,
                                              ProjMid& p, float q[4], float s[3]) {
#pragma unroll
  for (int k = 0; k < 3; ++k) p.mean[k] = means[3 * (size_t)i + k];
#pragma unroll
  for (int k = 0; k < 3; ++k)
    p.mc[k] = cam.R(k, 0) * p.mean[0] + cam.R(k, 1) * p.mean[1] + cam.R(k, 2) * p.mean[2] + cam.t[k];
#pragma unroll
  for (int k = 0; k < 4; ++k) q[k] = quats[4 * (size_t)i + k];
#pragma unroll
  for (int k = 0; k < 3; ++k) s[k] = scales[3 * (size_t)i + k];
}

__device__ __forceinline__ ProjOut project_pair(const float* __restrict__ means, const float* __restrict__ quats,
                                                const float* __restrict__ scales, int i, const Cam& cam, int W, int H,
                                                float eps2d, float near_plane, float far_plane, float radius_clip) {
  ProjMid p;
  float q[4], s[3];
  load_gaussian(means, quats, scales, i, cam, p, q, s);
  ProjOut o;
  o.radius = 0; o.mx = o.my = o.depth = o.ca = o.cb = o.cc = o.comp = 0.f;
  if (p.mc[2] >= near_plane && p.mc[2] <= far_plane) {
    p.covar = quat_scale_to_covar(q, s);
    p.covar_c = mul_bt(mul(cam.R, p.covar), cam.R);
    persp_mid(cam, W, H, p);
    float a, b, c;
    cov2d_from(p.J, p.covar_c, a, b, c);
    float det_orig = a * c - b * b;
    a += eps2d;
    c += eps2d;
    float det = a * c - b * b;
    if (det > 0.f) {
      float bb = 0.5f * (a + c);
      float v1 = bb + sqrtf(fmaxf(0.01f, bb * bb - det));
      float radius = ceilf(3.f * sqrtf(v1));
      float mx = cam.fx * p.mc[0] * p.rz + cam.cx;
      float my = cam.fy * p.mc[1] * p.rz + cam.cy;
      bool ok = radius > radius_clip;
      ok = ok && !(mx + radius <= 0.f || mx - radius >= (float)W || my + radius <= 0.f || my - radius >= (float)H);
      if (ok) {
        float inv = 1.f / det;
        o.radius = (int)radius;
        o.mx = mx; o.my = my; o.depth = p.mc[2];
        o.ca = c * inv; o.cb = -b * inv; o.cc = a * inv;
        o.comp = sqrtf(fmaxf(0.f, det_orig / det));
      }
    }
  }
  return o;
}

__device__ __forceinline__ void quat_vjp(const float qin[4], const M3& vR, float vq[4]) {
  float inv = rsqrtf(qin[0] * qin[0] + qin[1] * qin[1] + qin[2] * qin[2] + qin[3] * qin[3]);
  float w = qin[0] * inv, x = qin[1] * inv, y = qin[2] * inv, z = qin[3] * inv;
  float g[4];
  g[0] = 2.f * (x * (vR(2, 1) - vR(1, 2)) + y * (vR(0, 2) - vR(2, 0)) + z * (vR(1, 0) - vR(0, 1)));
  g[1] = 2.f * (-2.f * x * (vR(1, 1) + vR(2, 2)) + y * (vR(1, 0) + vR(0, 1)) + z * (vR(2, 0) + vR(0, 2)) +
                w * (vR(2, 1) - vR(1, 2)));
  g[2] = 2.f * (x * (vR(1, 0) + vR(0, 1)) - 2.f * y * (vR(0, 0) + vR(2, 2)) + z * (vR(2, 1) + vR(1, 2)) +
                w * (vR(0, 2) - vR(2, 0)));
  g[3] = 2.f * (x * (vR(2, 0) + vR(0, 2)) + y * (vR(2, 1) + vR(1, 2)) - 2.f * z * (vR(0, 0) + vR(1, 1)) +
                w * (vR(1, 0) - vR(0, 1)));
  float d = g[0] * w + g[1] * x + g[2] * y + g[3] * z;
  vq[0] = (g[0] - d * w) * inv;
  vq[1] = (g[1] - d * x) * inv;
  vq[2] = (g[2] - d * y) * inv;
  vq[3] = (g[3] - d * z) * inv;
}


template <bool FULL>
__device__ __forceinline__ void project_vjp(const Cam& cam, float eps2d, const ProjMid& p, const float q[4],
                                            const float s[3], float ca, float cb, float cc, float vm2x, float vm2y,
                                            float vdepth, float v_ca, float v_cb, float v_cc, bool has_comp,
                                            float comp, float vcomp, float vRt[12], float vmean[3], float vq[4],
                                            float vs[3]) {
  {
    float va = v_ca, vb = 0.5f * v_cb, vc = v_cc;
    float t00 = ca * va + cb * vb, t01 = ca * vb + cb * vc;
    float t10 = cb * va + cc * vb, t11 = cb * vb + cc * vc;
    float g00 = -(t00 * ca + t01 * cb), g01 = -(t00 * cb + t01 * cc);
    float g10 = -(t10 * ca + t11 * cb), g11 = -(t10 * cb + t11 * cc);
    if (has_comp) {
      float det_conic = ca * cc - cb * cb;
      float v_sqr = vcomp * 0.5f / (comp + 1e-6f);
      float om = 1.f - comp * comp;
      g00 += v_sqr * (om * ca - eps2d * det_conic);
      g01 += v_sqr * (om * cb);
      g10 += v_sqr * (om * cb);
      g11 += v_sqr * (om * cc - eps2d * det_conic);
    }
    const float* J = p.J;
    float GJ0[3], GJ1[3];
#pragma unroll
    for (int j = 0; j < 3; ++j) {
      GJ0[j] = g00 * J[j] + g01 * J[3 + j];
      GJ1[j] = g10 * J[j] + g11 * J[3 + j];
    }
    M3 vSc;
#pragma unroll
    for (int r = 0; r < 3; ++r)
#pragma unroll
      for (int c = 0; c < 3; ++c) vSc(r, c) = J[r] * GJ0[c] + J[3 + r] * GJ1[c];
    float GtJ0[3], GtJ1[3];
#pragma unroll
    for (int j = 0; j < 3; ++j) {
      GtJ0[j] = g00 * J[j] + g10 * J[3 + j];
      GtJ1[j] = g01 * J[j] + g11 * J[3 + j];
    }
    float vJ[6];
#pragma unroll
    for (int c = 0; c < 3; ++c) {
      float a0 = 0.f, a1 = 0.f;
#pragma unroll
      for (int k = 0; k < 3; ++k) {
        a0 += GJ0[k] * p.covar_c(c, k) + GtJ0[k] * p.covar_c(k, c);
        a1 += GJ1[k] * p.covar_c(c, k) + GtJ1[k] * p.covar_c(k, c);
      }
      vJ[c] = a0;
      vJ[3 + c] = a1;
    }
    float x = p.mc[0], y = p.mc[1];
    float rz = p.rz, rz2 = rz * rz, rz3 = rz2 * rz;
    float vmc[3];
    vmc[0] = cam.fx * rz * vm2x;
    vmc[1] = cam.fy * rz * vm2y;
    vmc[2] = -(cam.fx * x * vm2x + cam.fy * y * vm2y) * rz2;
// ... 46 lines not shown
```

gsplatloc_amd/csrc/raster_g16.hip:

```cpp
#include "gsloc_internal.h"
#include "composite_dev.h"
#include "long_dev.h"

namespace gsl {

#define G16_M_LO8 0x00FF00FF00FF00FFull
#define G16_M_B2 0x0F0F0F0F0F0F0F0Full
#define G16_M_B1 0x3333333333333333ull
#define G16_M_B0 0x5555555555555555ull

constexpr int G16_NG = GSL_NG;
constexpr int G16_GL = 64 / G16_NG;
static_assert(G16_NG == 4 || G16_NG == 8, "pixel groups are DPP rows or half rows");

__device__ __forceinline__ float row_scatter8(const float (&v)[8]) {
  float n0, n1, n2, n3, m0, m1;
  asm volatile(
      "s_nop 1\n\t"
      "v_add_f32_dpp %0, %6, %6 row_mirror row_mask:0xf bank_mask:0xf\n\t"
      "v_add_f32_dpp %1, %7, %7 row_mirror row_mask:0xf bank_mask:0xf\n\t"
      "v_add_f32_dpp %2, %8, %8 row_mirror row_mask:0xf bank_mask:0xf\n\t"
      "v_add_f32_dpp %3, %9, %9 row_mirror row_mask:0xf bank_mask:0xf\n\t"
      "v_add_f32_dpp %0, %10, %10 row_mirror row_mask:0xf bank_mask:0xc\n\t"
      "v_add_f32_dpp %1, %11, %11 row_mirror row_mask:0xf bank_mask:0xc\n\t"
// ... 17 lines not shown
    float keep = sel(G16_M_LO8, v[i], v[i + 8]), send = sel(G16_M_LO8, v[i + 8], v[i]);
    a[i] = keep + dpp_get<0x140>(send);
  }
  float n[4], m[2];
#pragma unroll
  for (int i = 0; i < 4; ++i) {
    float keep = sel(G16_M_B2, a[i], a[i + 4]), send = sel(G16_M_B2, a[i + 4], a[i]);
    n[i] = keep + dpp_get<0x141>(send);
  }
#pragma unroll
  for (int i = 0; i < 2; ++i) {
    float keep = sel(G16_M_B1, n[i], n[i + 2]), send = sel(G16_M_B1, n[i + 2], n[i]);
    m[i] = keep + dpp_get<0x4E>(send);
  }
  float keep = sel(G16_M_B0, m[0], m[1]), send = sel(G16_M_B0, m[1], m[0]);
  return keep + dpp_get<0xB1>(send);
}

__device__ __forceinline__ float4 half_scatter8(const float (&v)[8]) {
  float n0, n1, n2, n3;
  asm volatile(
      "s_nop 1\n\t"
      "v_add_f32_dpp %0, %4, %4 row_half_mirror row_mask:0xf bank_mask:0xf\n\t"
      "v_add_f32_dpp %1, %5, %5 row_half_mirror row_mask:0xf bank_mask:0xf\n\t"
      "v_add_f32_dpp %2, %6, %6 row_half_mirror row_mask:0xf bank_mask:0xf\n\t"
      "v_add_f32_dpp %3, %7, %7 row_half_mirror row_mask:0xf bank_mask:0xf\n\t"
      "v_add_f32_dpp %0, %8, %8 row_half_mirror row_mask:0xf bank_mask:0xa\n\t"
      "v_add_f32_dpp %1, %9, %9 row_half_mirror row_mask:0xf bank_mask:0xa\n\t"
      "v_add_f32_dpp %2, %10, %10 row_half_mirror row_mask:0xf bank_mask:0xa\n\t"
      "s_nop 1\n\t"
      : "=&v"(n0), "=&v"(n1), "=&v"(n2), "=&v"(n3)
      : "v"(v[0]), "v"(v[1]), "v"(v[2]), "v"(v[3]), "v"(v[4]), "v"(v[5]), "v"(v[6]));
  n0 += dpp_get<0x4E>(n0); n1 += dpp_get<0x4E>(n1); n2 += dpp_get<0x4E>(n2); n3 += dpp_get<0x4E>(n3);
  n0 += dpp_get<0xB1>(n0); n1 += dpp_get<0xB1>(n1); n2 += dpp_get<0xB1>(n2); n3 += dpp_get<0xB1>(n3);
  return make_float4(n0, n1, n2, n3);
}

__device__ __forceinline__ void half_scatter16(const float (&v)[16], float4& lo, float4& hi) {
  float a[8];
#pragma unroll
  for (int i = 0; i < 8; ++i) {
    float keep = sel(G16_M_B2, v[i], v[i + 8]), send = sel(G16_M_B2, v[i + 8], v[i]);
    a[i] = keep + dpp_get<0x141>(send);
  }
#pragma unroll
  for (int i = 0; i < 8; ++i) a[i] += dpp_get<0x4E>(a[i]);
#pragma unroll
  for (int i = 0; i < 8; ++i) a[i] += dpp_get<0xB1>(a[i]);
  lo = make_float4(a[0], a[1], a[2], a[3]);
  hi = make_float4(a[4], a[5], a[6], a[7]);
}

#ifdef GSL_G16_STATS
__device__ unsigned long long g16_stats[8];
#define G16_STAT(i, n) do { unsigned long long n__ = (unsigned long long)(n); if (lane == 0) atomicAdd(&g16_stats[i], n__); } while (0)
#else
#define G16_STAT(i, n) do { } while (0)
#endif

#ifndef GSL_QB
#define GSL_QB 64
#endif
#define GSL_QBS (GSL_QB + 1)
#ifndef GSL_Q_LCAP
#define GSL_Q_LCAP 24
#endif

template <int D, int CG>
struct QStage {
  static constexpr int NV = 6 + CG;
  static constexpr int NS = (NV <= 8) ? 8 : 16;
  static constexpr int A = 6 + D;
  static constexpr int LCAP = ((NS == 8) ? GSL_Q_LCAP : GSL_Q_LCAP / 2) * 4 / G16_NG;
  float4 s0[GSL_QBS];
  float4 s1[GSL_QBS];
  float4 s2[(D >= 3 && CG == D) ? GSL_QBS : 1];
  int32_t id[GSL_QBS];
  uint32_t posn[G16_NG / 4][GSL_QBS];
  alignas(16) float pair[G16_NG * LCAP * NS];
  uint8_t rlist[G16_NG][GSL_QBS + 4];
  uint8_t nzlist[64];
};

template <int D, int CG>
__device__ __forceinline__ void qraster_bwd_body(
    QStage<D, CG>& sb, const float4* __restrict__ Q0, const float4* __restrict__ Q1, const float4* __restrict__ Q2,
    const uint4* __restrict__ Qh, const int32_t* __restrict__ flatten_ids, float* __restrict__ vacc, long long rs,
    long long re, int lane, int quad, float px, float py, float tx0, float ty0, int bin_final, float T_init,
    float Bp_init, const float (&vc)[D], const uint32_t* __restrict__ qhits, int n_qhits) {
  constexpr bool RGB = D >= 3;
  constexpr int NV = QStage<D, CG>::NV;
  constexpr int NS = QStage<D, CG>::NS;
  constexpr int A = QStage<D, CG>::A;
  constexpr int LCAP = QStage<D, CG>::LCAP;
  constexpr int NG = G16_NG, GL = G16_GL;
  constexpr int PP = 12;
  static_assert(A <= PP && NG * LCAP * NS >= 64 * PP, "64 packed gradient rows reuse the pair slots");
  static_assert(GSL_QB < 127 && GSL_QB >= 64, "7-bit list positions with 127 reserved; a chunk appends up to 64 entries");
  const int grp = lane / GL, p = lane & (GL - 1);
  const float tcx = tx0 + 8.f, tcy = ty0 + 8.f;
  const float lx = px - tcx, ly = py - tcy;
  const float lxx = lx * lx, lxy = lx * ly, lyy = ly * ly;
  float T = T_init;
  float Bp = Bp_init;
  const int myslot = (NG == 8) ? (p >> 2) * (NS / 2) : ((NS == 8) ? (p >> 1) : p);
  const bool writer = (NG == 8) ? ((p & 3) == 0) : ((NS == 8) ? ((p & 1) == 0) : true);
  float* const mypair = &sb.pair[grp * LCAP * NS + myslot];
  uint8_t* const mylist = sb.rlist[grp];
  const unsigned long long lt = (1ull << lane) - 1ull;
  const float qx0 = tx0 + 8.f * (float)(quad & 1), qy0 = ty0 + 8.f * (float)(quad >> 1);
  int grp_final[NG];
  {
    int rf = bin_final;
    rf = max(rf, __shfl_xor(rf, 1, 64));
    rf = max(rf, __shfl_xor(rf, 2, 64));
    rf = max(rf, __shfl_xor(rf, 4, 64));
    if (GL == 16) rf = max(rf, __shfl_xor(rf, 8, 64));
#pragma unroll
    for (int g = 0; g < NG; ++g) grp_final[g] = __builtin_amdgcn_readlane(rf, GL * g);
  }
  if (lane == 0) {
    sb.s0[GSL_QB] = make_float4(0.f, 0.f, 0.f, 0.f);
    sb.s1[GSL_QB] = make_float4(0.f, 0.f, 0.f, 0.f);
    if (RGB && CG == D) sb.s2[GSL_QB] = make_float4(0.f, 0.f, 0.f, 0.f);
  }
  int pos = __builtin_amdgcn_readfirstlane(qhits ? n_qhits : (int)re);
  const int pos_end = __builtin_amdgcn_readfirstlane(qhits ? 0 : (int)rs);
  while (pos > pos_end) {
    int staged = 0;
    int cnt[NG];
#pragma unroll
    for (int g = 0; g < NG; ++g) cnt[g] = 0;
    __syncthreads();
    while (pos > pos_end && staged <= GSL_QB - 64) {
      long long idx = (long long)(pos - 1 - lane);
      bool in = idx >= (long long)pos_end;
      unsigned nib = 0;
      int gid = 0;
      float4 r0 = make_float4(0.f, 0.f, 0.f, 0.f), r1 = r0, r2 = r0;
      if (in) {
        if (qhits) {
          unsigned e = qhits[idx];
          nib = e >> GSL_HIT_SHIFT;
          idx = (long long)(e & GSL_HIT_INDEX_MASK);
          gid = flatten_ids[idx];
          load_record(Q0, Q1, Q2, Qh, gid, RGB && CG == D, r0, r1, r2);
        } else {
          gid = flatten_ids[idx];
          load_record(Q0, Q1, Q2, Qh, gid, RGB && CG == D, r0, r1, r2);
          if (r1.w >= 0.f) {
            float rr = r1.w * r1.w;
#pragma unroll
            for (int g = 0; g < NG; ++g) {
              const int b = (NG == 8) ? (g >> 1) : g;
              const float cy = (NG == 8) ? 2.f * (float)(g & 1) + 1.f : 2.f, hy = (NG == 8) ? 0.5f : 1.5f;
              float ex = fmaxf(fabsf(r0.x - (qx0 + 4.f * (float)(b & 1) + 2.f)) - 1.5f, 0.f);
              float ey = fmaxf(fabsf(r0.y - (qy0 + 4.f * (float)(b >> 1) + cy)) - hy, 0.f);
              bool h = (ex * ex + ey * ey <= rr) && ((int)idx <= grp_final[g]);
              nib |= (h ? 1u : 0u) << g;
            }
          }
        }
      }
      unsigned long long R = __ballot(nib != 0);
      int slot = staged + __popcll(R & lt);
      unsigned pack[NG / 4];
#pragma unroll
      for (int w = 0; w < NG / 4; ++w) pack[w] = 0x0FFFFFFFu;
#pragma unroll
      for (int g = 0; g < NG; ++g) {
        unsigned long long Bg = __ballot(nib & (1u << g));
        if (__builtin_amdgcn_inverse_ballot_w64(Bg)) {
          int q = cnt[g] + __popcll(Bg & lt);
          sb.rlist[g][q] = (uint8_t)slot;
          pack[g >> 2] ^= (127u ^ (unsigned)q) << (7 * (g & 3));
        }
        cnt[g] += __popcll(Bg);
      }
      if (__builtin_amdgcn_inverse_ballot_w64(R)) {
        sb.id[slot] = gid;
        sb.s0[slot] = r0;
        const float3 cn = stage_conic(r1);
        sb.s1[slot] = make_float4(cn.x, cn.y, cn.z, __int_as_float((int)idx));
        if (RGB && CG == D) sb.s2[slot] = r2;
#pragma unroll
        for (int w = 0; w < NG / 4; ++w) sb.posn[w][slot] = pack[w];
      }
      staged += __popcll(R);
      pos -= 64;
    }
    if (staged == 0) continue;
    int kmax = 0, cnt_tot = 0, cnt_my = 0;
#pragma unroll
    for (int g = 0; g < NG; ++g) {
      kmax = max(kmax, cnt[g]);
      cnt_tot += cnt[g];
      cnt_my = (grp == g) ? cnt[g] : cnt_my;
    }
    G16_STAT(6, kmax);
    G16_STAT(7, cnt_tot);
    (void)cnt_tot;
    for (int k = cnt_my + p; k < kmax + 3; k += GL) mylist[k] = (uint8_t)GSL_QB;
    __syncthreads();
    constexpr int NU = (GSL_QB + 63) / 64;
    float mo[NU][NV];
#pragma unroll
    for (int u = 0; u < NU; ++u)
#pragma unroll
      for (int q = 0; q < NV; ++q) mo[u][q] = 0.f;
    auto trip = [&](int t, const float4& c0, const float4& c1, float4& r, float4& r2) {
      float dx = c0.x - px, dy = c0.y - py;
      float sigma = sigma_log2e(c1.x, c1.y, c1.z, dx, dy);
      float vis = __builtin_amdgcn_exp2f(-sigma);
      float opv = c0.w * vis;
      float alpha = fminf(GSL_ALPHA_MAX, opv);
      unsigned long long validm = __ballot(__float_as_int(c1.w) <= bin_final) & __ballot(sigma >= 0.f) &
                                  __ballot(alpha >= GSL_ALPHA_MIN);
      G16_STAT(0, 1);
      r = make_float4(0.f, 0.f, 0.f, 0.f);
      r2 = r;
      if (validm) {
        G16_STAT(1, 1);
#ifdef GSL_G16_STATS
        {
          int groups_hit = 0;
          for (int g = 0; g < NG; ++g) groups_hit += ((validm >> (GL * g)) & ((1ull << GL) - 1ull)) != 0;
          G16_STAT(3, groups_hit);
        }
#endif
        G16_STAT(5, __popcll(validm));
        unsigned long long capm = __ballot(opv <= GSL_ALPHA_MAX);
        float am = sel(validm, alpha, 0.f);
        float ra = __builtin_amdgcn_rcpf(1.f - am);
        T *= ra;
        float fac = am * T;
        const float cdot = (CG == D) ? colour_dot<D>(sb.s2, t, c0.z, vc) : c0.z * vc[D - 1];
        float v_alpha = T * cdot - ra * Bp;
        Bp += fac * cdot;
        float w = sel(validm & capm, vis, 0.f) * v_alpha;
        float val[NS];
        val[0] = w; val[1] = w * lx; val[2] = w * ly; val[3] = w * lxx; val[4] = w * lxy; val[5] = w * lyy;
        if (CG == D) {
#pragma unroll
          for (int ch = 0; ch < D; ++ch) val[6 + ch] = fac * vc[ch];
        } else {
          val[6] = fac * vc[D - 1];
        }
#pragma unroll
        for (int q = NV; q < NS; ++q) val[q] = 0.f;
        static_assert(NS != 8 || NV == 7, "the 8-value scatters treat value 7 as padding");
        if (NG == 8) {
          if (NS == 8) r = half_scatter8(reinterpret_cast<const float(&)[8]>(val));
          else half_scatter16(reinterpret_cast<const float(&)[16]>(val), r, r2);
        } else {
          if (NS == 8) r.x = row_scatter8(reinterpret_cast<const float(&)[8]>(val));
          else r.x = row_scatter16(reinterpret_cast<const float(&)[16]>(val));
        }
      }
    };
    auto put = [&](float* dst, const float4& r, const float4& r2) {
      if (NG == 8) {
        *reinterpret_cast<float4*>(dst) = r;
        if (NS == 16) *reinterpret_cast<float4*>(dst + 4) = r2;
// ... 24 lines not shown
      if (writer) put(dst - NS, rb, rb2);
      __syncthreads();
#pragma unroll
      for (int u = 0; u < NU; ++u) {
        int slot = lane + 64 * u;
        if (slot < staged) {
#pragma unroll
          for (int w = 0; w < NG / 4; ++w) {
            unsigned pk = sb.posn[w][slot];
#pragma unroll
            for (int g4 = 0; g4 < 4; ++g4) {
              const int g = 4 * w + g4;
              const unsigned q = ((pk >> (7 * g4)) & 127u) - (unsigned)k0;
              if (q < (unsigned)LCAP) {
                const float4* src = reinterpret_cast<const float4*>(&sb.pair[(g * LCAP + q) * NS]);
                float4 a = src[0], c = src[1];
                mo[u][0] += a.x; mo[u][1] += a.y; mo[u][2] += a.z; mo[u][3] += a.w;
                mo[u][4] += c.x; mo[u][5] += c.y; mo[u][6] += c.z;
                if (NV > 7) mo[u][7 < NV ? 7 : 0] += c.w;
                if (NS == 16) {
                  float4 e = src[2];
                  if (NV > 8) mo[u][8 < NV ? 8 : 0] += e.x;
                  if (NV > 9) mo[u][9 < NV ? 9 : 0] += e.y;
                }
              }
            }
          }
        }
      }
      __syncthreads();
    }
#pragma unroll
    for (int u = 0; u < NU; ++u) {
      int slot = lane + 64 * u;
      bool nz = false;
      float row[A];
#pragma unroll
      for (int k = 0; k < A; ++k) row[k] = 0.f;
      if (slot < staged) {
        {
          unsigned bits = 0u;
#pragma unroll
          for (int k = 0; k < NV; ++k) bits |= __float_as_uint(mo[u][k]);
          nz = (bits << 1) != 0u;
        }
        if (nz) {
          float4 r0 = sb.s0[slot], r1 = sb.s1[slot];
          float X = r0.x - tcx, Y = r0.y - tcy, S = mo[u][0];
          float Sx = X * S - mo[u][1], Sy = Y * S - mo[u][2];
          float Sxx = X * (X * S - 2.f * mo[u][1]) + mo[u][3];
          float Sxy = X * (Y * S - mo[u][2]) - Y * mo[u][1] + mo[u][4];
          float Syy = Y * (Y * S - 2.f * mo[u][2]) + mo[u][5];
          float no = -r0.w;
          r1.x *= 2.f / GSL_LOG2E; r1.y *= 1.f / GSL_LOG2E; r1.z *= 2.f / GSL_LOG2E;
          row[0] = no * (r1.x * Sx + r1.y * Sy);
          row[1] = no * (r1.y * Sx + r1.z * Sy);
          row[2] = 0.5f * no * Sxx;
          row[3] = no * Sxy;
          row[4] = 0.5f * no * Syy;
          row[5] = S;
          if (CG == D) {
#pragma unroll
            for (int ch = 0; ch < D; ++ch) row[6 + ch] = mo[u][6 + ch];
          } else {
            row[6 + D - 1] = mo[u][6];
          }
        }
      }
      float* packed = sb.pair;
      if (nz) {
#pragma unroll
        for (int k = 0; k < A; ++k) packed[lane * PP + k] = row[k];
      }
      unsigned long long mask = __ballot(nz);
      int cntz = __popcll(mask);
      if (nz) sb.nzlist[__popcll(mask & lt)] = (uint8_t)lane;
      __syncthreads();
      constexpr int RPI = 64 / A;
      const int arow = lane / A, f = lane - arow * A;
      for (int i0 = 0; i0 < cntz; i0 += RPI) {
        int gi = i0 + arow;
        if (gi < cntz && arow < RPI) {
          int sl = sb.nzlist[gi];
          const unsigned off = ((unsigned)sb.id[sl + 64 * u] << 6) | ((unsigned)f << 2);
          atomicAdd(reinterpret_cast<float*>(reinterpret_cast<char*>(vacc) + off), packed[sl * PP + f]);
        }
      }
      __syncthreads();
    }
  }
}

template <int D, bool ED, int CG, bool LONG>
__device__ __forceinline__ void qraster_bwd_item(
    QStage<D, CG>& sb, int b, int n_items, const float4* __restrict__ Q0, const float4* __restrict__ Q1,
    const float4* __restrict__ Q2, int W, int H, int tile_w, int ty0, const int32_t* __restrict__ tile_offsets,
    const int32_t* __restrict__ flatten_ids, long long capacity, const float* __restrict__ render,
    const float* __restrict__ alphas, const int32_t* __restrict__ last_ids, const float* __restrict__ v_render,
    const float* __restrict__ v_alphas, float* __restrict__ vacc, int row0, int row1, const uint4* __restrict__ Qh,
    const uint32_t* __restrict__ isect_hits, int32_t* __restrict__ isect_hit_counts, int long_min, LongWs lw,
    int32_t* __restrict__ rgb_flag, int32_t* __restrict__ clear_counts, int32_t* __restrict__ clear_state) {
  if (!LONG && (CG == 1 || D == 3) && clear_counts && (b & 3) == 0 && threadIdx.x == 0) {
    clear_counts[ty0 * tile_w + (b >> 2)] = 0;
    if (b == 0 && clear_state) *clear_state = 0;
  }
  const int wi = LONG ? b : xcd_span_item(b, n_items);
  const int quad = wi & 3, item = wi >> 2;
  int tile, sgm = 0, gseg = 0;
  if (LONG) {
    gseg = item;
    if (gseg >= lw.n_seg[0]) return;
    tile = lw.seg_tile[gseg];
    sgm = lw.seg_idx[gseg];
    if (tile < 0) return;
  } else {
    tile = ty0 * tile_w + item;
  }
  const int lane = threadIdx.x;
  const TilePixel tp = quadrant_pixel<true>(tile, tile_w, quad, lane);
  bool inside = pixel_inside(tp, W, H, row0, row1);

  ListSpan sp = tile_span(tile_offsets, tile, capacity);
  if (sp.rs >= sp.re) return;
  if (!LONG && long_min > 0 && sp.re - sp.rs > long_min) return;
  if (LONG) sp = segment_span(sp, sgm);
  size_t pid = pixel_index(tp, W, inside);
  int bin_final = last_composited(last_ids, pid, inside);
  trim_span(sp, wave_max(bin_final));
  if (sp.rs >= sp.re) return;
  float vc[D];
  load_upstream<D>(v_render, pid, inside, vc);
  if (D == 4) {
    bool rgb_grad = (vc[0] != 0.f) || (vc[1] != 0.f) || (vc[2] != 0.f);
    bool any_rgb = __ballot(rgb_grad) != 0ull;
    if ((CG == 1) == any_rgb) {
      if (CG == 1 && rgb_flag && lane == 0) atomicOr(rgb_flag, 1);
      return;
    }
  }
  const BwdStart st = bwd_start<D, ED>(alphas, render, v_alphas, pid, inside, vc);
  float T_init = st.T_final, Bp_init = st.Bp();
  if (LONG) {
    int nseg = lw.seg_cnt[gseg];
    long long seg_end = min(tile_offsets[tile] + (long long)(sgm + 1) * GSL_SEG, (long long)tile_offsets[tile + 1]);
    int pslot = quad * 64 + lane;
    if (inside && (long long)bin_final >= seg_end) {
      T_init = fabsf(lw.Tend[(size_t)gseg * 256 + pslot]);
      const float4* C4 = reinterpret_cast<const float4*>(lw.C);
      bool stop = false;
      for (int s0 = sgm + 1; s0 < nseg && !stop; s0 += 8) {
        float t8[8];
        float4 c8[8];
#pragma unroll
        for (int u = 0; u < 8; ++u) {
          size_t slot = (size_t)(gseg - sgm + min(s0 + u, nseg - 1)) * 256 + pslot;
          t8[u] = lw.Tend[slot];
          c8[u] = C4[slot];
        }
#pragma unroll
        for (int u = 0; u < 8; ++u) {
          if (stop || s0 + u >= nseg) continue;
          if (t8[u] == 2.f) { stop = true; continue; }
          float cc[4] = {c8[u].x, c8[u].y, c8[u].z, c8[u].w};
          float dot = 0.f;
#pragma unroll
          for (int k = 0; k < D; ++k) dot += vc[k] * cc[k];
          Bp_init += dot;
          if (t8[u] < 0.f) stop = true;
        }
      }
    }
  }
  const uint32_t* qh = nullptr;
  int nqh = 0;
  if (isect_hits) {
    const ListSpan whole = tile_span(tile_offsets, tile, capacity), list = LONG ? segment_span(whole, sgm) : whole;
    nqh = LONG ? lw.seg_qcnt[gseg * 4 + quad] : isect_hit_counts[tile * 4 + quad];
    qh = isect_hits + 4 * list.rs + (long long)quad * (list.re - list.rs);
    if (nqh == 0) return;
  }
  qraster_bwd_body<D, CG>(sb, Q0, Q1, Q2, Qh, flatten_ids, vacc, sp.rs, sp.re, lane, quad, tp.px, tp.py, (float)(tp.txi * 16),
                          (float)(tp.tyi * 16), bin_final, T_init, Bp_init, vc, qh, nqh);
}

template <int D, bool ED, int CG, bool LONG>
__global__ __launch_bounds__(64) void k_qraster_bwd(
    const float4* __restrict__ Q0, const float4* __restrict__ Q1, const float4* __restrict__ Q2, int W, int H,
    int tile_w, int ty0, const int32_t* __restrict__ tile_offsets, const int32_t* __restrict__ flatten_ids,
    long long capacity, const float* __restrict__ render, const float* __restrict__ alphas,
    const int32_t* __restrict__ last_ids, const float* __restrict__ v_render, const float* __restrict__ v_alphas,
    float* __restrict__ vacc, int row0, int row1, const uint4* __restrict__ Qh,
    const uint32_t* __restrict__ isect_hits, int32_t* __restrict__ isect_hit_counts, int long_min, LongWs lw,
    int32_t* __restrict__ rgb_flag, int32_t* __restrict__ clear_counts, int32_t* __restrict__ clear_state, int n_items) {
  __shared__ QStage<D, CG> sb;
  if (D == 4 && CG == D && rgb_flag && *rgb_flag == 0) return;
  for (int b = (int)blockIdx.x; b < n_items; b += (int)gridDim.x) {
    qraster_bwd_item<D, ED, CG, LONG>(sb, b, n_items, Q0, Q1, Q2, W, H, tile_w, ty0, tile_offsets, flatten_ids, capacity,
                                      render, alphas, last_ids, v_render, v_alphas, vacc, row0, row1, Qh, isect_hits,
                                      isect_hit_counts, long_min, lw, rgb_flag, clear_counts, clear_state);
    __syncthreads();
  }
}

}

#ifdef GSL_G16_STATS
extern "C" int gsl_g16_stats(unsigned long long* host_out, int reset) {
  if (hipMemcpyFromSymbol(host_out, HIP_SYMBOL(gsl::g16_stats), sizeof(unsigned long long) * 8) != hipSuccess) return -3;
  if (reset) {
    unsigned long long z[8] = {0};
    if (hipMemcpyToSymbol(HIP_SYMBOL(gsl::g16_stats), z, sizeof(z)) != hipSuccess) return -3;
  }
  return 0;
}
#endif

static int g16_raster_bwd_launch(const float* Q0, const float* Q1, const float* Q2, int channels, int ed, int width,
                                 int height, int tile_w, int ty0, int ty1, const int32_t* tile_offsets,
                                 const int32_t* flatten_ids, int64_t capacity, const float* render,
                                 const float* alphas, const int32_t* last_ids, const float* v_render,
                                 const float* v_alphas, float* vacc, int row0, int row1, const void* Qh,
                                 const uint32_t* isect_hits, const int32_t* isect_hit_counts, int long_min,
                                 void* long_ws, int max_seg, int rgb_flag_index, void* clear_ws, void* stream) {
  hipStream_t st = (hipStream_t)stream;
  int nblk = long_ws ? max_seg : (ty1 - ty0) * tile_w;
  gsl::LongWs lw = gsl::long_ws_views(long_ws ? long_ws : (void*)0, long_ws ? max_seg : 0);
  const bool lng = long_ws != nullptr;
  int32_t* rgb_flag = isect_hit_counts ? const_cast<int32_t*>(isect_hit_counts) + rgb_flag_index : nullptr;
  int32_t* clear_counts = (int32_t*)clear_ws;
  int32_t* clear_state = gsl::fused_bin_state(clear_ws, rgb_flag_index / 4);
#define CALL_QL(DD, EE, CC, LL)                                                                                  \
  hipLaunchKernelGGL((gsl::k_qraster_bwd<DD, EE, CC, LL>), dim3(grid), dim3(64), 0, st, (const float4*)Q0,       \
                     (const float4*)Q1, (const float4*)Q2, width, height, tile_w, ty0, tile_offsets, flatten_ids, \
                     (long long)capacity, render, alphas, last_ids, v_render, v_alphas, vacc, row0, row1,         \
                     (const uint4*)Qh, isect_hits, const_cast<int32_t*>(isect_hit_counts), long_min, lw, rgb_flag, \
                     clear_counts, clear_state, n_items)
#define CALL_Q(DD, EE, CC)                                                                    \
  do {                                                                                        \
    const int n_items = 4 * nblk;                                                             \
    const int grid = ((DD) == 4 && (CC) == 4 && rgb_flag && n_items > 2048) ? 2048 : n_items; \
    if (lng) CALL_QL(DD, EE, CC, true); else CALL_QL(DD, EE, CC, false);                      \
  } while (0)
#define CALL_QD(DD, EE) do { CALL_Q(DD, EE, ((DD) == 4 ? 1 : (DD))); if ((DD) == 4) CALL_Q(DD, EE, DD); } while (0)
  GSL_DISPATCH_CH_ED(channels, ed, CALL_QD)
#undef CALL_QD
#undef CALL_Q
#undef CALL_QL
  GSL_CHECK_LAUNCH();
  return GSL_OK;
}

extern "C" int gsl_fused_raster_bwd(const float* Q0, const float* Q1, const float* Q2, int channels, int ed,
                                   int width, int height, int tile_w, int tile_h, int ty0, int ty1,
                                   const int32_t* tile_offsets, const int32_t* flatten_ids, int64_t capacity,
                                   const float* render, const float* alphas, const int32_t* last_ids,
                                   const float* v_render, const float* v_alphas, float* vacc, int row0, int row1,
                                   const void* Qh, float* vrow, const uint32_t* isect_hits,
                                   const int32_t* isect_hit_counts, int long_min, void* clear_ws, void* stream) {
  if (!gsl::frame_ok(width, height, tile_w, tile_h, ty0, ty1, capacity, row0, row1)) return GSL_ERR_BAD_ARG;
  if (!tile_offsets || !render || !alphas || !last_ids || !v_render || !v_alphas) return GSL_ERR_BAD_ARG;
  if (!gsl::ed_ok(channels, ed)) return GSL_ERR_BAD_ARG;
  if (capacity == 0 || ty0 == ty1 || row0 == row1) return GSL_OK;
  if (!flatten_ids || (!vacc && !vrow)) return GSL_ERR_BAD_ARG;
  if (isect_hits && !isect_hit_counts) return GSL_ERR_BAD_ARG;
  if (!gsl::records_ok(Qh, Q0, Q1, Q2, channels)) return GSL_ERR_BAD_ARG;
  if (vrow && clear_ws) return GSL_ERR_BAD_ARG;
  if (vrow)
    return gsl::launch_mraster_bwd(Q0, Q1, Q2, channels, ed, width, height, tile_w, ty0, ty1, tile_offsets, flatten_ids,
                                   capacity, render, alphas, last_ids, v_render, v_alphas, vrow, row0, row1, Qh,
                                   (hipStream_t)stream);
  return g16_raster_bwd_launch(Q0, Q1, Q2, channels, ed, width, height, tile_w, ty0, ty1, tile_offsets, flatten_ids,
                               capacity, render, alphas, last_ids, v_render, v_alphas, vacc, row0, row1, Qh,
                               isect_hits, isect_hit_counts, long_min, nullptr, 0, 4 * tile_w * tile_h, clear_ws,
                                   stream);
}

extern "C" int gsl_long_raster_bwd(const float* Q0, const float* Q1, const float* Q2, int channels, int ed, int width,
                                   int height, int tile_w, int tile_h, int ty0, int ty1, const int32_t* tile_offsets,
                                   const int32_t* flatten_ids, int64_t capacity, const float* render,
                                   const float* alphas, const int32_t* last_ids, const float* v_render,
                                   const float* v_alphas, float* vacc, int row0, int row1, const void* Qh,
                                   const uint32_t* isect_hits, int long_min, void* long_ws, int max_seg,
                                   void* stream) {
  if (!gsl::frame_ok(width, height, tile_w, tile_h, ty0, ty1, capacity, row0, row1, false) || long_min <= 0 ||
      max_seg <= 0 || !long_ws)
    return GSL_ERR_BAD_ARG;
  if (!tile_offsets || !render || !alphas || !last_ids || !v_render || !v_alphas || !vacc) return GSL_ERR_BAD_ARG;
  if (!gsl::ed_ok(channels, ed)) return GSL_ERR_BAD_ARG;
  if (capacity == 0 || ty0 == ty1 || row0 == row1) return GSL_OK;
  if (!flatten_ids || !gsl::records_ok(Qh, Q0, Q1, Q2, channels)) return GSL_ERR_BAD_ARG;
  return g16_raster_bwd_launch(Q0, Q1, Q2, channels, ed, width, height, tile_w, ty0, ty1, tile_offsets, flatten_ids,
                               capacity, render, alphas, last_ids, v_render, v_alphas, vacc, row0, row1, Qh,
                               isect_hits, nullptr, long_min, long_ws, max_seg, 0, nullptr, stream);
}
```

gsplatloc_amd/csrc/sort_dev.h:

```cpp
#pragma once
#include "gsloc_common.h"

namespace gsl {

__device__ __forceinline__ uint64_t shfl_xor_u64(uint64_t v, int mask) {
  unsigned lo = (unsigned)v, hi = (unsigned)(v >> 32);
  lo = (unsigned)__shfl_xor((int)lo, mask, 64);
  hi = (unsigned)__shfl_xor((int)hi, mask, 64);
  return ((uint64_t)hi << 32) | lo;
}
#define GSL_SORT_PAD 0x7FF0000000000000ull
__device__ __forceinline__ void cswap(uint64_t& a, uint64_t& b) {
  const double x = __longlong_as_double((long long)a), y = __longlong_as_double((long long)b);
  double lo, hi;
  asm("v_min_f64 %0, %1, %2" : "=v"(lo) : "v"(x), "v"(y));
  asm("v_max_f64 %0, %1, %2" : "=v"(hi) : "v"(x), "v"(y));
  a = (uint64_t)__double_as_longlong(lo);
  b = (uint64_t)__double_as_longlong(hi);
}
__device__ __forceinline__ uint64_t pick(uint64_t a, uint64_t o, unsigned long long keep_min_mask) {
  const unsigned long long take = ~(__ballot(o < a) ^ keep_min_mask);
  return ((uint64_t)sel(take, (unsigned)(o >> 32), (unsigned)(a >> 32)) << 32) |
         sel(take, (unsigned)o, (unsigned)a);
}
// ... 55 lines not shown
  }
#pragma unroll 1
  for (int tb = 1; tb <= 6; ++tb) {
    int mask = (1 << tb) - 1;
    const unsigned long long keep_min = __ballot(((lane >> (tb - 1)) & 1) == 0);
    switch (tb) {
      case 1: flip_stage<KPT>(k, XDpp<0xB1>(), keep_min); break;
      case 2: flip_stage<KPT>(k, XDpp<0x1B>(), keep_min); break;
      case 3: flip_stage<KPT>(k, XDpp<0x141>(), keep_min); break;
      case 4: flip_stage<KPT>(k, XDpp<0x140>(), keep_min); break;
      default: flip_stage<KPT>(k, XShfl{mask}, keep_min); break;
    }
#pragma unroll 1
    for (int b = tb - 2; b >= 0; --b) {
      const unsigned long long km = __ballot(((lane >> b) & 1) == 0);
      switch (b) {
        case 0: clean_stage<KPT>(k, XDpp<0xB1>(), km); break;
        case 1: clean_stage<KPT>(k, XDpp<0x4E>(), km); break;
        case 2: clean_stage<KPT>(k, XDppXor4(), km); break;
        case 3: clean_stage<KPT>(k, XDpp<0x128>(), km); break;
        default: clean_stage<KPT>(k, XShfl{1 << b}, km); break;
      }
    }
#pragma unroll
    for (int lj = LK - 1; lj >= 0; --lj)
#pragma unroll
      for (int r = 0; r < KPT; ++r) {
        int p = r ^ (1 << lj);
        if (r < p) cswap(k[r], k[p]);
      }
  }
}

__device__ __forceinline__ int prefix_count_share(const int32_t* __restrict__ counts, int n, int cap, int tid) {
  int acc = 0;
  for (int base = 0; base < n; base += 256 * 8) {
    int v[8];
#pragma unroll
    for (int u = 0; u < 8; ++u) {
      const int i = base + u * 256 + tid;
      v[u] = (i < n) ? counts[i] : 0;
    }
#pragma unroll
    for (int u = 0; u < 8; ++u) acc += min(v[u], cap);
  }
  return acc;
}

__device__ __forceinline__ void binned_tile_span(const int32_t* counts, int t, bool last, int bin_cap, int32_t* tile_offsets,
                                                 int32_t* n_isects, int32_t* flags, int* s_scan, int tid, long long& s,
                                                 long long& e) {
  const int lane = tid & 63, wv = tid >> 6;
  int acc = prefix_count_share(counts, t, bin_cap, tid);
#pragma unroll
  for (int o = 32; o >= 1; o >>= 1) acc += __shfl_xor(acc, o, 64);
  if (lane == 0) s_scan[wv] = acc;
  if (tid == 0) {
    int c_own = counts[t];
    s_scan[4] = min(c_own, bin_cap);
    if (c_own > bin_cap && flags) { flags[1] = 1; atomicMax(&flags[2], c_own); }
  }
  __syncthreads();
  s = s_scan[0] + s_scan[1] + s_scan[2] + s_scan[3];
  e = s + s_scan[4];
  if (tid == 0) {
    tile_offsets[t] = (int32_t)s;
    if (last) {
      tile_offsets[t + 1] = (int32_t)e;
      if (n_isects) n_isects[0] = (int32_t)e;
    }
  }
}

__device__ __forceinline__ void write_sorted_key(uint64_t v, long long pos, int t, uint64_t* __restrict__ keys_out,
                                                 int32_t* __restrict__ flatten_ids, int64_t* __restrict__ isect_ids,
                                                 int64_t cam_enc, const int32_t* __restrict__ storage_of) {
  flatten_ids[pos] = list_id(storage_of, v);
  if (isect_ids) isect_ids[pos] = cam_enc | ((int64_t)t << 32) | (int64_t)(v >> 32);
  if (keys_out) keys_out[pos] = v;
}

struct RowClear {
  float4* rows;
  int n4, per;
  __device__ __forceinline__ void run(int part, int t, int width) const {
    const int b = part * per, e = min(n4, b + per);
    const float4 z = make_float4(0.f, 0.f, 0.f, 0.f);
    for (int i = b + t; i < e; i += width) rows[i] = z;
  }
};
__device__ __forceinline__ void keys_arrived() { __builtin_amdgcn_s_waitcnt(0x0F70); }

__device__ __forceinline__ int merge_diag(const uint64_t* __restrict__ A, int lenA, const uint64_t* __restrict__ B, int lenB,
                                          int d) {
  int lo = max(0, d - lenB), hi = min(d, lenA);
  while (lo < hi) {
    int mid = (lo + hi) >> 1;
    if (A[mid] <= B[d - 1 - mid]) lo = mid + 1;
    else hi = mid;
  }
  return lo;
}

template <int LK, bool CLR = false>
__device__ __forceinline__ void wg_sort_tile(const uint64_t* __restrict__ src, int n, long long s, int t, int tid,
                                             uint64_t* __restrict__ lds, uint64_t* __restrict__ keys_out,
                                             int32_t* __restrict__ flatten_ids, int64_t* __restrict__ isect_ids,
                                             int64_t cam_enc, const int32_t* __restrict__ storage_of = nullptr,
                                             const RowClear clr = RowClear{nullptr, 0, 0}, int clr_part = 0) {
  constexpr int KPT = 1 << LK, RUN = 64 * KPT;
  const int lane = tid & 63, wv = tid >> 6;
  uint64_t k[KPT];
  const int e0 = wv * RUN + lane * KPT;
#pragma unroll
  for (int r = 0; r < KPT; ++r) k[r] = (e0 + r < n) ? src[e0 + r] : GSL_SORT_PAD;
  if (CLR) {
    keys_arrived();
    if (clr.rows) clr.run(clr_part, tid, 256);
  }
  wave_sort_regs<LK>(k, lane);
  uint64_t* bufA = lds;
  uint64_t* bufB = lds + 4 * RUN;
#pragma unroll
  for (int r = 0; r < KPT; ++r) bufA[e0 + r] = k[r];
  __syncthreads();
  {
    const int p = tid >> 7, l = tid & 127;
    const uint64_t* A = bufA + p * 2 * RUN;
    const uint64_t* B = A + RUN;
    const int d0 = l * KPT;
    int ia = merge_diag(A, RUN, B, RUN, d0), ib = d0 - ia;
#pragma unroll
    for (int q = 0; q < KPT; ++q) {
      uint64_t v;
      if (ib >= RUN || (ia < RUN && A[ia] <= B[ib])) v = A[ia++];
      else v = B[ib++];
      bufB[p * 2 * RUN + d0 + q] = v;
    }
  }
  __syncthreads();
  {
    const uint64_t* A = bufB;
    const uint64_t* B = bufB + 2 * RUN;
    const int d0 = tid * KPT;
    if (d0 < n) {
      int ia = merge_diag(A, 2 * RUN, B, 2 * RUN, d0), ib = d0 - ia;
#pragma unroll
      for (int q = 0; q < KPT; ++q) {
        uint64_t v;
        if (ib >= 2 * RUN || (ia < 2 * RUN && A[ia] <= B[ib])) v = A[ia++];
        else v = B[ib++];
        if (d0 + q < n) write_sorted_key(v, s + d0 + q, t, keys_out, flatten_ids, isect_ids, cam_enc, storage_of);
      }
    }
  }
}

}
```

gsplatloc_amd/csrc/tile_sort.hip:

```cpp
#include <atomic>
#include <cstdlib>
#include <cstring>
#include "gsloc_internal.h"
#include "long_dev.h"
#include "sort_dev.h"

namespace gsl {

#define GSL_SORT_LDS_CAP 4096

__device__ __forceinline__ void bitonic_flip_step(uint64_t* a, int n, int half, int k, int tid, int nthreads) {
  int hk = k >> 1;
  for (int i = tid; i < half; i += nthreads) {
    int blk = i / hk, off = i - blk * hk;
    int lo = blk * k + off;
    int hi = blk * k + (k - 1 - off);
    if (hi < n) {
      uint64_t x = a[lo], y = a[hi];
      if (x > y) { a[lo] = y; a[hi] = x; }
    }
  }
  __syncthreads();
}
__device__ __forceinline__ void bitonic_half_step(uint64_t* a, int n, int half, int j, int tid, int nthreads) {
// ... 292 lines not shown
  {
    int ia_lo = merge_diag_wave(A, lenA, B, lenB, o, lane);
    int ia_hi = merge_diag_wave(A, lenA, B, lenB, o + out_len, lane);
    if (lane == 0) {
      s_split[0] = ia_lo;
      s_split[1] = o - ia_lo;
      s_split[2] = ia_hi;
      s_split[3] = o + out_len - ia_hi;
    }
  }
  __syncthreads();
  int ia0 = s_split[0], ib0 = s_split[1], na = s_split[2] - ia0, nb = s_split[3] - ib0;
  for (int q = lane; q < na; q += 64) sk[q] = A[ia0 + q];
  for (int q = lane; q < nb; q += 64) sk[na + q] = B[ib0 + q];
  __syncthreads();
  constexpr int KPL = GSL_SORT_SEG / 64;
  int d0 = min(lane * KPL, out_len), d1 = min(lane * KPL + KPL, out_len);
  int ia = merge_diag(sk, na, sk + na, nb, d0), ib = d0 - ia;
  for (int d = d0; d < d1; ++d) {
    uint64_t v;
    if (ib >= nb || (ia < na && sk[ia] <= sk[na + ib])) v = sk[ia++];
    else v = sk[na + ib++];
    dst[pair_start + o + d] = v;
    if (last) flatten_ids[s + pair_start + o + d] = list_id(storage_of, v);
  }
}

__global__ __launch_bounds__(256) void k_tile_sort_wg(int32_t* __restrict__ tile_offsets, int tile_begin,
                                                      int n_strip_tiles, long long capacity,
                                                      uint64_t* __restrict__ keys, int32_t* __restrict__ flatten_ids,
                                                      int64_t* __restrict__ isect_ids, int64_t cam_enc,
                                                      int write_sorted_keys, uint64_t* __restrict__ bins, int bin_cap,
                                                      const int32_t* __restrict__ counts, int32_t* __restrict__ n_isects,
                                                      int32_t* __restrict__ flags, int long_min,
                                                      const int32_t* __restrict__ storage_of, const RowClear clr) {
  __shared__ uint64_t skeys[GSL_SORT_LDS_CAP];
  __shared__ int s_scan[5];
  const int tid = threadIdx.x;
  const int t = tile_begin + blockIdx.x;
  long long s, e;
  if (counts) {
    binned_tile_span(counts, t, (int)blockIdx.x == n_strip_tiles - 1, bin_cap, tile_offsets, n_isects, flags, s_scan, tid, s, e);
  } else {
    s = tile_offsets[t];
    e = tile_offsets[t + 1];
  }
  if (e > capacity) e = capacity;
  int n = (int)max(e - s, (long long)0);
  if (bins && n > bin_cap) n = bin_cap;
  if (clr.rows && (n == 0 || n > 2048)) clr.run(blockIdx.x, tid, 256);
  if (n == 0) return;
  uint64_t* src = bins ? bins + (size_t)t * (size_t)bin_cap : keys + s;
  uint64_t* kout = write_sorted_keys ? keys : nullptr;
  if (n <= 1024) {
    wg_sort_tile<2, true>(src, n, s, t, tid, skeys, kout, flatten_ids, isect_ids, cam_enc, storage_of, clr, blockIdx.x);
  } else if (n <= 2048) {
    wg_sort_tile<3, true>(src, n, s, t, tid, skeys, kout, flatten_ids, isect_ids, cam_enc, storage_of, clr, blockIdx.x);
  } else {
    if (long_min > 0 && bins && n > long_min) return;
    bitonic_sort_long(src, n, skeys, tid);
    for (int i = tid; i < n; i += 256)
      write_sorted_key(src[i], s + i, t, write_sorted_keys && bins ? keys : nullptr, flatten_ids, isect_ids, cam_enc, storage_of);
  }
}

}

namespace gsl {
static std::atomic<int64_t> g_tile_sort_launches[3];
}

extern "C" int64_t gsl_dev_tile_sort_launches(int variant) {
  if (variant < 0 || variant > 2) return -1;
  return gsl::g_tile_sort_launches[variant].load(std::memory_order_relaxed);
}

extern "C" int gsl_tile_sort(const int32_t* tile_offsets, int tile_begin, int n_strip_tiles, int64_t capacity,
                             uint64_t* sort_keys, int32_t* flatten_ids, int64_t* isect_ids, int64_t cam_enc,
                             void* stream) {
  if (!tile_offsets || tile_begin < 0 || n_strip_tiles < 0 || capacity < 0) return GSL_ERR_BAD_ARG;
  if (n_strip_tiles == 0 || capacity == 0) return GSL_OK;
  if (!sort_keys || !flatten_ids) return GSL_ERR_BAD_ARG;
  return gsl::tile_sort_keys(const_cast<int32_t*>(tile_offsets), tile_begin, n_strip_tiles, capacity, sort_keys, flatten_ids,
                             isect_ids, cam_enc, 0, nullptr, 0, nullptr, nullptr, nullptr, 0, 0, nullptr, nullptr, 0, stream);
}

int gsl::tile_sort_keys(int32_t* tile_offsets, int tile_begin, int n_strip_tiles, int64_t capacity, uint64_t* sort_keys,
                        int32_t* flatten_ids, int64_t* isect_ids, int64_t cam_enc, int write_sorted_keys, uint64_t* bins,
                        int bin_cap, const int32_t* counts, int32_t* n_isects, int32_t* flags, int long_min,
                        int occupied_tiles, const int32_t* storage_of, float* clear_rows, int clear_n, void* stream) {
  if (!tile_offsets || tile_begin < 0 || n_strip_tiles < 0 || capacity < 0) return GSL_ERR_BAD_ARG;
  if (counts && (!bins || tile_begin != 0)) return GSL_ERR_BAD_ARG;
  if (clear_n < 0 || clear_n > GSL_MAX_GAUSSIANS || (clear_n > 0 && !clear_rows)) return GSL_ERR_BAD_ARG;
  if (clear_n == 0) clear_rows = nullptr;
  if (n_strip_tiles == 0 || (capacity == 0 && !counts))
    return clear_rows ? gsl::zero_u32(clear_rows, (size_t)16 * (size_t)clear_n, (hipStream_t)stream) : GSL_OK;
  if (capacity > 0 && (!sort_keys || !flatten_ids)) return GSL_ERR_BAD_ARG;
  const int occ = occupied_tiles > 0 ? occupied_tiles : n_strip_tiles;
  const long long mean_list = capacity / (long long)occ;
  const char* force = getenv("GSL_DEV_TILE_SORT");
  int variant;
  if (force && !strcmp(force, "wg")) variant = 2;
  else if (force && !strcmp(force, "wave16")) variant = 0;
  else if (force && !strcmp(force, "wave32")) variant = 1;
  else if (!(force && !strcmp(force, "wave")) && mean_list > 320 && occ <= 2048) variant = 2;
  else variant = mean_list <= 1150 ? 0 : 1;
  const int parts = variant == 2 ? n_strip_tiles : (n_strip_tiles + 3) / 4 * 4, width = variant == 2 ? 256 : 64;
  const int n4 = 4 * clear_n;
  const gsl::RowClear clr{(float4*)clear_rows, n4, ((n4 + parts - 1) / parts + width - 1) / width * width};
  auto launch = [&](auto kernel, int tiles_per_wg) {
    hipLaunchKernelGGL(kernel, dim3((n_strip_tiles + tiles_per_wg - 1) / tiles_per_wg), dim3(256), 0, (hipStream_t)stream,
                       tile_offsets, tile_begin, n_strip_tiles, (long long)capacity, sort_keys, flatten_ids, isect_ids,
                       cam_enc, write_sorted_keys, bins, bin_cap, counts, n_isects, flags, long_min, storage_of, clr);
  };
  if (variant == 2) launch(gsl::k_tile_sort_wg, 1);
  else if (variant == 0) launch(gsl::k_tile_sort<4>, 4);
  else launch(gsl::k_tile_sort<5>, 4);
  gsl::g_tile_sort_launches[variant].fetch_add(1, std::memory_order_relaxed);
  GSL_CHECK_LAUNCH();
  return GSL_OK;
}

extern "C" int gsl_long_sort(const int32_t* tile_offsets, int tile_w, int tile_h, int ty0, int ty1, int64_t capacity,
                             uint64_t* bins, int bin_cap, uint64_t* sort_keys, int32_t* flatten_ids, int long_min,
                             void* long_ws, size_t long_ws_bytes, int max_seg, int passes, const int32_t* storage_of,
                             void* stream) {
  if (tile_w <= 0 || tile_h <= 0 || ty0 < 0 || ty1 > tile_h || ty0 > ty1 || capacity < 0 || long_min <= 0 ||
      max_seg <= 0 || passes < 0 || passes > 12 || bin_cap <= 0)
    return GSL_ERR_BAD_ARG;
  if (!tile_offsets || !bins || !sort_keys || !flatten_ids || !long_ws) return GSL_ERR_BAD_ARG;
  if (long_ws_bytes < gsl_long_ws_bytes(max_seg)) return GSL_ERR_WORKSPACE;
  if (ty0 == ty1 || capacity == 0) return GSL_OK;
  hipStream_t st = (hipStream_t)stream;
  gsl::LongWs w = gsl::long_ws_views(long_ws, max_seg);
  gsl::launch_long_map(st, tile_offsets, ty0 * tile_w, (ty1 - ty0) * tile_w, (long long)capacity, long_min, max_seg,
                       GSL_SORT_SEG << passes, w);
  hipLaunchKernelGGL(gsl::k_long_sort_seg, dim3(max_seg), dim3(64), 0, st, tile_offsets, (long long)capacity, bins,
                     bin_cap, sort_keys, w);
  for (int p = 0; p < passes; ++p)
    hipLaunchKernelGGL(gsl::k_long_merge, dim3(max_seg), dim3(64), 0, st, tile_offsets, (long long)capacity, bins, bin_cap,
                       sort_keys, p, p == passes - 1 ? 1 : 0, flatten_ids, w, storage_of);
  GSL_CHECK_LAUNCH();
  return GSL_OK;
}
```

gsplatloc_amd/stages.py:

```python
from __future__ import annotations

import math

import torch

from ._lib import check, current_stream, load_library, ptr

MAX_STRIP_TILES = 8192
_MODES = {"RGB": (3, False), "D": (1, False), "ED": (1, True), "RGB+D": (4, False), "RGB+ED": (4, True)}


def tile_n_bits(n_tiles: int) -> int:
    return int(math.floor(math.log2(n_tiles))) + 1


def alloc_records(N: int, rgb: bool, dev, zero: bool = False):
    make = torch.zeros if zero else torch.empty
    Q0, Q1 = (make(N, 4, dtype=torch.float32, device=dev) for _ in range(2))
    Q2 = make(N, 4, dtype=torch.float32, device=dev) if rgb else None
    return Q0, Q1, Q2


def fused_project(means, quats, scales, opacities, colors, sh_degree, K_sh, viewmat, K, N, width, height, eps2d, near_plane,
                  far_plane, radius_clip, antialiased, tile_w, tile_h, ty0, ty1, radii, Q0, Q1, Q2, compensations,
                  tiles_per_gauss, tile_offsets, n_isects, ws, *, Qh=None, bins=None, bin_cap=0, flags=None, order_ids=None):
    check(load_library().gsl_fused_project(
        means.data_ptr(), quats.data_ptr(), scales.data_ptr(), opacities.data_ptr(), ptr(colors), sh_degree, K_sh,
        viewmat.data_ptr(), K.data_ptr(), N, width, height, eps2d, near_plane, far_plane, radius_clip, antialiased, tile_w,
        tile_h, ty0, ty1, radii.data_ptr(), Q0.data_ptr(), Q1.data_ptr(), ptr(Q2), ptr(compensations), ptr(tiles_per_gauss),
        tile_offsets.data_ptr(), n_isects.data_ptr(), ws.data_ptr(), ws.numel(), ptr(Qh), ptr(bins), bin_cap, ptr(flags),
        ptr(order_ids), current_stream()), "gsl_fused_project")


def fused_bin(Q0, radii, N, tile_w, tile_h, ty0, ty1, tile_n_bits, tile_offsets, capacity, sort_keys, flatten_ids, ws, *,
              isect_ids=None, write_sorted_keys=0, bins=None, bin_cap=0, n_isects=None, flags=None, long_min=0,
              order_ids=None, storage_of=None):
    check(load_library().gsl_fused_bin(
        Q0.data_ptr(), radii.data_ptr(), N, tile_w, tile_h, ty0, ty1, tile_n_bits, tile_offsets.data_ptr(), capacity,
        sort_keys.data_ptr(), ptr(flatten_ids), ptr(isect_ids), ws.data_ptr(), ws.numel(), write_sorted_keys, ptr(bins),
        bin_cap, ptr(n_isects), ptr(flags), long_min, ptr(order_ids), ptr(storage_of), current_stream()), "gsl_fused_bin")


def fused_bin_clear(Q0, radii, N, tile_w, tile_h, ty0, ty1, tile_n_bits, tile_offsets, capacity, sort_keys, flatten_ids, ws,
                    rows, *, isect_ids=None, write_sorted_keys=0, bins=None, bin_cap=0, n_isects=None, flags=None,
                    long_min=0, order_ids=None, storage_of=None):
    check(load_library().gsl_fused_bin_clear(
        Q0.data_ptr(), radii.data_ptr(), N, tile_w, tile_h, ty0, ty1, tile_n_bits, tile_offsets.data_ptr(), capacity,
        sort_keys.data_ptr(), ptr(flatten_ids), ptr(isect_ids), ws.data_ptr(), ws.numel(), write_sorted_keys, ptr(bins),
        bin_cap, ptr(n_isects), ptr(flags), long_min, ptr(order_ids), ptr(storage_of), ptr(rows), current_stream()),
        "gsl_fused_bin_clear")


def fused_clear_rows(rows, N):
    check(load_library().gsl_fused_clear_rows(ptr(rows), N, current_stream()), "gsl_fused_clear_rows")


def fused_raster_fwd(Q0, Q1, Q2, channels, ed, width, height, tile_w, tile_h, ty0, ty1, tile_offsets, flatten_ids, capacity,
                     render, alphas, last_ids, row0, row1, *, Qh=None, binned_ws=None, isect_hits=None, isect_hit_counts=None,
                     long_min=0, sort_bins=None, bin_cap=0, n_isects=None, flags=None, storage_of=None):
    check(load_library().gsl_fused_raster_fwd(
        ptr(Q0), ptr(Q1), ptr(Q2), channels, ed, width, height, tile_w, tile_h, ty0, ty1, tile_offsets.data_ptr(),
        ptr(flatten_ids), capacity, render.data_ptr(), alphas.data_ptr(), last_ids.data_ptr(), row0, row1, ptr(Qh),
        ptr(binned_ws), ptr(isect_hits), ptr(isect_hit_counts), long_min, ptr(sort_bins), bin_cap, ptr(n_isects), ptr(flags),
        ptr(storage_of), current_stream()), "gsl_fused_raster_fwd")


def fused_raster_bwd(Q0, Q1, Q2, channels, ed, width, height, tile_w, tile_h, ty0, ty1, tile_offsets, flatten_ids, capacity,
                     render, alphas, last_ids, v_render, v_alphas, vacc, row0, row1, *, Qh=None, vrow=None, isect_hits=None,
                     isect_hit_counts=None, long_min=0, clear_ws=None):
    check(load_library().gsl_fused_raster_bwd(
        ptr(Q0), ptr(Q1), ptr(Q2), channels, ed, width, height, tile_w, tile_h, ty0, ty1, tile_offsets.data_ptr(),
        ptr(flatten_ids), capacity, render.data_ptr(), alphas.data_ptr(), last_ids.data_ptr(), v_render.data_ptr(),
        v_alphas.data_ptr(), ptr(vacc), row0, row1, ptr(Qh), ptr(vrow), ptr(isect_hits), ptr(isect_hit_counts), long_min,
        ptr(clear_ws), current_stream()), "gsl_fused_raster_bwd")


def tiny_raster_bwd(Q0, Q1, Q2, channels, ed, width, height, tile_w, tile_h, ty0, ty1, tile_offsets, flatten_ids, capacity,
                    render, alphas, last_ids, v_render, v_alphas, trec, vcT, row0, row1, *, flags=None, long_min=0,
                    loss_depth_gt=None, depth_lambda=0.0, edge_lambda=0.0, loss_partials=None, clear_ws=None):
    check(load_library().gsl_tiny_raster_bwd(
        ptr(Q0), ptr(Q1), ptr(Q2), channels, ed, width, height, tile_w, tile_h, ty0, ty1, tile_offsets.data_ptr(),
        ptr(flatten_ids), capacity, render.data_ptr(), alphas.data_ptr(), last_ids.data_ptr(), v_render.data_ptr(),
        v_alphas.data_ptr(), trec.data_ptr(), vcT.data_ptr(), row0, row1, ptr(flags), long_min, ptr(loss_depth_gt),
        depth_lambda, edge_lambda, ptr(loss_partials), ptr(clear_ws), current_stream()), "gsl_tiny_raster_bwd")


def long_sort(tile_offsets, tile_w, tile_h, ty0, ty1, capacity, bins, bin_cap, sort_keys, flatten_ids, long_min, long_ws,
              max_seg, passes, *, storage_of=None):
    check(load_library().gsl_long_sort(
        tile_offsets.data_ptr(), tile_w, tile_h, ty0, ty1, capacity, bins.data_ptr(), bin_cap, sort_keys.data_ptr(),
        flatten_ids.data_ptr(), long_min, long_ws.data_ptr(), long_ws.numel(), max_seg, passes, ptr(storage_of),
        current_stream()), "gsl_long_sort")


def long_raster_fwd(Q0, Q1, Q2, channels, ed, width, height, tile_w, tile_h, ty0, ty1, tile_offsets, flatten_ids, capacity,
                    render, alphas, last_ids, row0, row1, long_min, long_ws, max_seg, map_ready, *, Qh=None, isect_hits=None):
    check(load_library().gsl_long_raster_fwd(
        ptr(Q0), ptr(Q1), ptr(Q2), channels, ed, width, height, tile_w, tile_h, ty0, ty1, tile_offsets.data_ptr(),
        flatten_ids.data_ptr(), capacity, render.data_ptr(), alphas.data_ptr(), last_ids.data_ptr(), row0, row1, ptr(Qh),
        ptr(isect_hits), long_min, long_ws.data_ptr(), long_ws.numel(), max_seg, map_ready, current_stream()),
        "gsl_long_raster_fwd")


def long_raster_bwd(Q0, Q1, Q2, channels, ed, width, height, tile_w, tile_h, ty0, ty1, tile_offsets, flatten_ids, capacity,
                    render, alphas, last_ids, v_render, v_alphas, vacc, row0, row1, long_min, long_ws, max_seg, *, Qh=None,
                    isect_hits=None):
    check(load_library().gsl_long_raster_bwd(
        ptr(Q0), ptr(Q1), ptr(Q2), channels, ed, width, height, tile_w, tile_h, ty0, ty1, tile_offsets.data_ptr(),
        flatten_ids.data_ptr(), capacity, render.data_ptr(), alphas.data_ptr(), last_ids.data_ptr(), v_render.data_ptr(),
        v_alphas.data_ptr(), vacc.data_ptr(), row0, row1, ptr(Qh), ptr(isect_hits), long_min, long_ws.data_ptr(), max_seg,
        current_stream()), "gsl_long_raster_bwd")


def fused_project_bwd(means, quats, scales, opacities, colors, sh_degree, K_sh, viewmat, K, N, width, height, eps2d,
                      antialiased, channels, radii, Q1, compensations, vacc, v_means, v_quats, v_scales, v_opacities,
                      v_colors, v_viewmat, ws, n_tiles, reduce_viewmat, *, vrow=None, sorted_keys=None, tile_offsets=None,
                      Q0=None, tile_w=0, tile_h=0, ty0=0, ty1=0, capacity=0, tiny_trec=None, tiny_vcT=None,
                      v_colors_state=None):
    check(load_library().gsl_fused_project_bwd(
        means.data_ptr(), quats.data_ptr(), scales.data_ptr(), opacities.data_ptr(), ptr(colors), sh_degree, K_sh,
        viewmat.data_ptr(), K.data_ptr(), N, width, height, eps2d, antialiased, channels, radii.data_ptr(), Q1.data_ptr(),
        ptr(compensations), ptr(vacc), ptr(v_means), ptr(v_quats), ptr(v_scales), ptr(v_opacities), ptr(v_colors),
        ptr(v_viewmat), ws.data_ptr(), ws.numel(), n_tiles, ptr(vrow), ptr(sorted_keys), ptr(tile_offsets), ptr(Q0), tile_w,
        tile_h, ty0, ty1, capacity, ptr(tiny_trec), ptr(tiny_vcT), reduce_viewmat, ptr(v_colors_state), current_stream()),
        "gsl_fused_project_bwd")


def fused_project_bwd_keep(means, quats, scales, opacities, colors, sh_degree, K_sh, viewmat, K, N, width, height, eps2d,
                           antialiased, channels, radii, Q1, compensations, vacc, v_means, v_quats, v_scales, v_opacities,
                           v_colors, v_viewmat, ws, n_tiles, reduce_viewmat, *, vrow=None, sorted_keys=None,
                           tile_offsets=None, Q0=None, tile_w=0, tile_h=0, ty0=0, ty1=0, capacity=0, tiny_trec=None,
                           tiny_vcT=None, v_colors_state=None):
    check(load_library().gsl_fused_project_bwd_keep(
        means.data_ptr(), quats.data_ptr(), scales.data_ptr(), opacities.data_ptr(), ptr(colors), sh_degree, K_sh,
        viewmat.data_ptr(), K.data_ptr(), N, width, height, eps2d, antialiased, channels, radii.data_ptr(), Q1.data_ptr(),
        ptr(compensations), ptr(vacc), ptr(v_means), ptr(v_quats), ptr(v_scales), ptr(v_opacities), ptr(v_colors),
        ptr(v_viewmat), ws.data_ptr(), ws.numel(), n_tiles, ptr(vrow), ptr(sorted_keys), ptr(tile_offsets), ptr(Q0), tile_w,
        tile_h, ty0, ty1, capacity, ptr(tiny_trec), ptr(tiny_vcT), reduce_viewmat, ptr(v_colors_state), current_stream()),
        "gsl_fused_project_bwd_keep")


def fused_absgrad(Q0, Q1, Q2, channels, ed, width, height, tile_w, tile_h, tile_offsets, flatten_ids, capacity, render,
                  alphas, last_ids, v_render, v_alphas, absgrad, *, isect_hits=None, isect_hit_counts=None):
    check(load_library().gsl_fused_absgrad(
        ptr(Q0), ptr(Q1), ptr(Q2), channels, ed, width, height, tile_w, tile_h, tile_offsets.data_ptr(), ptr(flatten_ids),
        capacity, render.data_ptr(), alphas.data_ptr(), last_ids.data_ptr(), v_render.data_ptr(), v_alphas.data_ptr(),
        ptr(isect_hits), ptr(isect_hit_counts), absgrad.data_ptr(), current_stream()), "gsl_fused_absgrad")
```

include/gsloc_hip.h:

```cpp
#ifndef GSLOC_HIP_H
#define GSLOC_HIP_H

#include <stddef.h>
#include <stdint.h>

#ifdef __cplusplus
extern "C" {
#endif

typedef enum gsl_status {
  GSL_OK = 0,
  GSL_ERR_BAD_ARG = -1,
  GSL_ERR_WORKSPACE = -2,
  GSL_ERR_HIP = -3
} gsl_status;

const char* gsl_version(void);
const char* gsl_status_string(int status);
int gsl_dev_poison_lds(uint32_t pattern, void* stream);
int64_t gsl_dev_tile_sort_launches(int variant);
int gsl_project_fwd(const float* means, const float* quats, const float* scales,
                    const float* viewmat, const float* K, int N, int width, int height,
                    float eps2d, float near_plane, float far_plane, float radius_clip,
                    int32_t* radii, float* means2d, float* depths, float* conics,
// ... 201 lines not shown
                      const float* opacities, const float* backgrounds, int channels, int width,
                      int height, int tile_size, int tile_w, int tile_h, int ty0, int ty1,
                      const int32_t* tile_offsets, const int32_t* flatten_ids, int64_t capacity,
                      const float* render_alphas, const int32_t* last_ids, const float* t_final,
                      const float* v_render_colors, const float* v_render_alphas, float* vacc,
                      void* stream);
int gsl_vacc_unpack(const float* vacc, int n_gaussians, int channels, float* v_means2d,
                    float* v_conics, float* v_colors, float* v_opacities, void* stream);

size_t gsl_fused_ws_bytes(int N, int n_tiles);
int gsl_fused_project(const float* means, const float* quats, const float* scales,
                      const float* opacities, const float* colors, int sh_degree, int K_sh,
                      const float* viewmat, const float* K, int N, int width, int height,
                      float eps2d, float near_plane, float far_plane, float radius_clip,
                      int antialiased, int tile_w, int tile_h, int ty0, int ty1, int32_t* radii,
                      float* Q0, float* Q1, float* Q2, float* compensations,
                      int32_t* tiles_per_gauss, int32_t* tile_offsets, int32_t* n_isects, void* ws,
                      size_t ws_bytes, void* Qh, void* bins, int bin_cap, int32_t* flags,
                      const int32_t* order_ids, void* stream);
int gsl_fused_bin(const float* Q0, const int32_t* radii, int N, int tile_w, int tile_h, int ty0,
                  int ty1, int tile_n_bits, int32_t* tile_offsets, int64_t capacity,
                  uint64_t* sort_keys, int32_t* flatten_ids, int64_t* isect_ids, void* ws,
                  size_t ws_bytes, int write_sorted_keys, void* bins, int bin_cap, int32_t* n_isects,
                  int32_t* flags, int long_min, const int32_t* order_ids, const int32_t* storage_of, void* stream);
int gsl_fused_bin_clear(const float* Q0, const int32_t* radii, int N, int tile_w, int tile_h, int ty0,
                        int ty1, int tile_n_bits, int32_t* tile_offsets, int64_t capacity,
                        uint64_t* sort_keys, int32_t* flatten_ids, int64_t* isect_ids, void* ws,
                        size_t ws_bytes, int write_sorted_keys, void* bins, int bin_cap, int32_t* n_isects,
                        int32_t* flags, int long_min, const int32_t* order_ids, const int32_t* storage_of,
                        float* rows, void* stream);
int gsl_fused_clear_rows(float* rows, int N, void* stream);
int gsl_fused_raster_fwd(const float* Q0, const float* Q1, const float* Q2, int channels, int ed,
                         int width, int height, int tile_w, int tile_h, int ty0, int ty1,
                         const int32_t* tile_offsets, const int32_t* flatten_ids, int64_t capacity,
                         float* render, float* alphas, int32_t* last_ids, int row0, int row1, const void* Qh,
                         void* binned_ws, uint32_t* isect_hits, int32_t* isect_hit_counts, int long_min,
                         void* sort_bins, int bin_cap, int32_t* n_isects, int32_t* flags,
                         const int32_t* storage_of, void* stream);
int gsl_fused_raster_bwd(const float* Q0, const float* Q1, const float* Q2, int channels, int ed,
                         int width, int height, int tile_w, int tile_h, int ty0, int ty1,
                         const int32_t* tile_offsets, const int32_t* flatten_ids, int64_t capacity,
                         const float* render, const float* alphas, const int32_t* last_ids,
                         const float* v_render, const float* v_alphas, float* vacc, int row0, int row1,
                         const void* Qh, float* vrow, const uint32_t* isect_hits,
                         const int32_t* isect_hit_counts, int long_min, void* clear_ws, void* stream);
size_t gsl_long_ws_bytes(int max_seg);
int gsl_long_segment(void);
int gsl_long_sort_segment(void);
int gsl_long_sort(const int32_t* tile_offsets, int tile_w, int tile_h, int ty0, int ty1, int64_t capacity,
                  uint64_t* bins, int bin_cap, uint64_t* sort_keys, int32_t* flatten_ids, int long_min,
                  void* long_ws, size_t long_ws_bytes, int max_seg, int passes, const int32_t* storage_of,
                  void* stream);
int gsl_long_raster_fwd(const float* Q0, const float* Q1, const float* Q2, int channels, int ed, int width,
                        int height, int tile_w, int tile_h, int ty0, int ty1, const int32_t* tile_offsets,
                        const int32_t* flatten_ids, int64_t capacity, float* render, float* alphas,
                        int32_t* last_ids, int row0, int row1, const void* Qh, uint32_t* isect_hits,
                        int long_min, void* long_ws, size_t long_ws_bytes, int max_seg, int map_ready, void* stream);
int gsl_long_raster_bwd(const float* Q0, const float* Q1, const float* Q2, int channels, int ed, int width,
                        int height, int tile_w, int tile_h, int ty0, int ty1, const int32_t* tile_offsets,
                        const int32_t* flatten_ids, int64_t capacity, const float* render,
                        const float* alphas, const int32_t* last_ids, const float* v_render,
                        const float* v_alphas, float* vacc, int row0, int row1, const void* Qh,
                        const uint32_t* isect_hits, int long_min, void* long_ws, int max_seg, void* stream);
int gsl_fused_project_bwd(const float* means, const float* quats, const float* scales,
                          const float* opacities, const float* colors, int sh_degree, int K_sh,
                          const float* viewmat, const float* K, int N, int width, int height,
                          float eps2d, int antialiased, int channels, const int32_t* radii,
                          const float* Q1, const float* compensations, float* vacc, float* v_means,
                          float* v_quats, float* v_scales, float* v_opacities, float* v_colors,
                          float* v_viewmat, void* ws, size_t ws_bytes, int n_tiles, const float* vrow,
                          const uint64_t* sorted_keys, const int32_t* tile_offsets, const float* Q0, int tile_w,
                          int tile_h, int ty0, int ty1, int64_t capacity, float* tiny_trec, const float* tiny_vcT,
                          int reduce_viewmat, int32_t* v_colors_state, void* stream);
int gsl_fused_project_bwd_keep(const float* means, const float* quats, const float* scales,
                               const float* opacities, const float* colors, int sh_degree, int K_sh,
                               const float* viewmat, const float* K, int N, int width, int height,
                               float eps2d, int antialiased, int channels, const int32_t* radii,
                               const float* Q1, const float* compensations, float* vacc, float* v_means,
                               float* v_quats, float* v_scales, float* v_opacities, float* v_colors,
                               float* v_viewmat, void* ws, size_t ws_bytes, int n_tiles, const float* vrow,
                               const uint64_t* sorted_keys, const int32_t* tile_offsets, const float* Q0, int tile_w,
                               int tile_h, int ty0, int ty1, int64_t capacity, float* tiny_trec, const float* tiny_vcT,
                               int reduce_viewmat, int32_t* v_colors_state, void* stream);
const float* gsl_fused_viewmat_rows(const void* ws, int n_tiles);

int gsl_tiny_raster_bwd(const float* Q0, const float* Q1, const float* Q2, int channels, int ed,
                        int width, int height, int tile_w, int tile_h, int ty0, int ty1,
                        const int32_t* tile_offsets, const int32_t* flatten_ids, int64_t capacity,
                        const float* render, const float* alphas, const int32_t* last_ids,
                        const float* v_render, const float* v_alphas, float* trec, float* vcT,
                        int row0, int row1, int32_t* flags, int long_min, const float* loss_depth_gt,
                        float depth_lambda, float edge_lambda, float* loss_partials, void* clear_ws, void* stream);

size_t gsl_photo_ws_bytes(int width, int height);
int gsl_photo_loss(const float* render, int channels, const float* pixels, int width, int height, float rgb_lambda,
                   float ssim_lambda, float* v_render, float* photo_sums, void* ws, size_t ws_bytes, void* stream);
int gsl_pose_step_photo(float* pose_f, int* pose_i, const float* v_viewmat, const float* vm_rows, int n_vm_rows,
                        const float* K, const float* loss_partials, int n_partials, const float* loss_sums,
                        const float* normal_sum, const float* gt_c2w, int width, int height, float depth_lambda,
                        float edge_lambda, float normal_lambda, double beta1, double beta2, float eps, float wd_quat,
                        float wd_trans, double gamma, int min_step, int patience, int early_stop, int max_steps,
                        float* c2w, float* viewmat, float* loss_hist, void* stream, const float* photo_sums,
                        float rgb_lambda, float ssim_lambda);
int gsl_pose_step_best(float* pose_f, int* pose_i, const float* v_viewmat, const float* vm_rows, int n_vm_rows,
                       const float* K, const float* loss_partials, int n_partials, const float* loss_sums,
                       const float* normal_sum, const float* gt_c2w, int width, int height, float depth_lambda,
                       float edge_lambda, float normal_lambda, double beta1, double beta2, float eps, float wd_quat,
                       float wd_trans, double gamma, int min_step, int patience, int early_stop, int max_steps,
                       float* c2w, float* viewmat, float* loss_hist, void* stream, const float* photo_sums,
                       float rgb_lambda, float ssim_lambda, float* best_pose);
size_t gsl_loss_ws_bytes(int width, int height);
int gsl_loss_n_partials(int width, int height, int row0, int row1);
size_t gsl_normal_ws_bytes(int width, int height);
int gsl_normal_loss(const float* render, int channels, const float* depth_gt, int width, int height, int row0,
                    int row1, float fx, float fy, float cx, float cy, float normal_lambda, float* v_render,
                    float* normal_sum, void* ws, size_t ws_bytes, void* stream);
int gsl_tracking_loss(const float* render, int channels, const float* depth_gt, int width, int height,
                      int row0, int row1, float depth_lambda, float edge_lambda, float* v_render,
                      float* loss_partials, int* n_partials_host, void* ws, size_t ws_bytes, void* stream);
int gsl_pose_init(float* pose_f, int* pose_i, const float* init_c2w, float lr_quat, float lr_trans,
                  float* c2w, float* viewmat, void* stream);
int gsl_pose_step(float* pose_f, int* pose_i, const float* v_viewmat, const float* vm_rows, int n_vm_rows,
                  const float* K, const float* loss_partials, int n_partials, const float* loss_sums, const float* normal_sum, const float* gt_c2w,
                  int width, int height, float depth_lambda, float edge_lambda, float normal_lambda,
                  double beta1, double beta2, float eps,
                  float wd_quat, float wd_trans, double gamma, int min_step, int patience, int early_stop,
                  int max_steps, float* c2w, float* viewmat, float* loss_hist, void* stream);
int gsl_pack_pose_reduce(const float* v_viewmat, const float* vm_rows, int n_vm_rows, const float* viewmat,
                         const float* K, const float* loss_partials, int n_partials, const float* normal_sum,
                         float* out16, void* stream);

size_t gsl_knn_ws_bytes(int N);
int gsl_knn_cells(void);
int gsl_knn_count(const float* points, int N, const float* bbox, void* ws, size_t ws_bytes, void* stream);
int gsl_knn_query(const float* points, int N, const float* bbox, const int32_t* incl_offsets, int k,
                  float* dists, void* ws, size_t ws_bytes, void* stream);

int gsl_fused_absgrad(const float* Q0, const float* Q1, const float* Q2, int channels, int ed, int width, int height,
                      int tile_w, int tile_h, const int32_t* tile_offsets, const int32_t* flatten_ids, int64_t capacity,
                      const float* render, const float* alphas, const int32_t* last_ids, const float* v_render,
                      const float* v_alphas, const uint32_t* isect_hits, const int32_t* isect_hit_counts,
                      float* absgrad, void* stream);
int gsl_rasterize_absgrad(const float* means2d, const float* conics, const float* colors, const float* opacities,
                          const float* backgrounds, int channels, int width, int height, int tile_size, int tile_w,
                          int tile_h, const int32_t* tile_offsets, const int32_t* flatten_ids, int64_t capacity,
                          const float* render_alphas, const int32_t* last_ids, const float* t_final,
                          const float* v_render_colors, const float* v_render_alphas, float* absgrad, void* stream);

#ifdef __cplusplus
}
#endif
#endif
```

Measured before the change: 2.489 billion.

## Add packed-pitch gradient rows and recompute conics instead of reading Q1

```diff
diff --git a/gsplatloc_amd/_lib.py b/gsplatloc_amd/_lib.py
--- a/gsplatloc_amd/_lib.py
+++ b/gsplatloc_amd/_lib.py
@@ -151,6 +151,16 @@
     "gsl_fused_project_bwd_keep": (c_int, [P, P, P, P, P, c_int, c_int, P, P, c_int, c_int, c_int, c_float, c_int, c_int,
                                            P, P, P, P, P, P, P, P, P, P, P, c_size_t, c_int, P, P, P, P, c_int, c_int,
                                            c_int, c_int, c_int64, P, P, c_int, P, P]),
+    "gsl_fused_bin_clear_pitch": (c_int, [P, P, c_int, c_int, c_int, c_int, c_int, c_int, P, c_int64, P, P, P, P, c_size_t,
+                                          c_int, P, c_int, P, P, c_int, P, P, P, c_int, P]),
+    "gsl_fused_clear_rows_pitch": (c_int, [P, c_int, c_int, P]),
+    "gsl_fused_raster_bwd_pitch": (c_int, [P, P, P, c_int, c_int, c_int, c_int, c_int, c_int, c_int, c_int, P, P, c_int64,
+                                           P, P, P, P, P, P, c_int, c_int, P, P, P, P, c_int, P, c_int, P]),
+    "gsl_long_raster_bwd_pitch": (c_int, [P, P, P, c_int, c_int, c_int, c_int, c_int, c_int, c_int, c_int, P, P, c_int64,
+                                          P, P, P, P, P, P, c_int, c_int, P, P, c_int, P, c_int, c_int, P]),
+    "gsl_fused_project_bwd_pitch": (c_int, [P, P, P, P, P, c_int, c_int, P, P, c_int, c_int, c_int, c_float, c_int, c_int,
+                                            P, P, P, P, P, P, P, P, P, P, P, c_size_t, c_int, P, P, P, P, c_int, c_int,
+                                            c_int, c_int, c_int64, P, P, c_int, P, c_int, c_int, P]),
     "gsl_tiny_raster_bwd": (c_int, [P, P, P, c_int, c_int, c_int, c_int, c_int, c_int, c_int, c_int, P, P, c_int64,
                                     P, P, P, P, P, P, P, c_int, c_int, P, c_int, P, c_float, c_float, P, P, P]),
     "gsl_isect_emit": (c_int, [P, P, P, P, c_int, c_int, c_int, c_int, c_int, c_int, c_int, P, P, P]),
diff --git a/gsplatloc_amd/context.py b/gsplatloc_amd/context.py
--- a/gsplatloc_amd/context.py
+++ b/gsplatloc_amd/context.py
@@ -74,7 +74,10 @@
         self.render = torch.zeros(self.H, self.W, self.D, dtype=f32, device=dev)
         self.alphas = torch.zeros(self.H, self.W, 1, dtype=f32, device=dev)
         self.last_ids = torch.zeros(self.H, self.W, dtype=i32, device=dev)
-        self.vacc = torch.zeros(N, 16, dtype=f32, device=dev)
+        dense = os.environ.get("GSLOC_DENSE_ROWS", "0") == "1" and not deterministic
+        self.row_pitch = (6 + self.D + 1) // 2 * 2 if dense else 16
+        self._vacc_store = torch.zeros((N * self.row_pitch + 3) // 4 * 4, dtype=f32, device=dev)
+        self.vacc = self._vacc_store[:N * self.row_pitch].view(N, self.row_pitch)
         self._rows_dirty = False
         self._sort_cleared = False
         self.v_viewmat = torch.zeros(4, 4, dtype=f32, device=dev)
@@ -383,8 +386,9 @@
         if self._sort_cleared and self.sort_clears_rows():
             project_bwd = stages.fused_project_bwd_keep
             self._rows_dirty = True
+        Q1 = self.Q1 if self.tiny else None
         project_bwd(means, quats, scales, opacities, colors if self.rgb else None, self.sh_degree, self.K_sh, viewmat, K,
-                    self.N, self.W, self.H, self.eps2d, int(self.antialiased), self.D, self.radii, self.Q1, self.comps,
+                    self.N, self.W, self.H, self.eps2d, int(self.antialiased), self.D, self.radii, Q1, self.comps,
                     self.vacc if (not self.tiny or self.long_min) else None, *grads,
                     self.v_colors if (full and self.rgb) else None, self.v_viewmat, self.ws, self.n_tiles, int(reduce),
                     v_colors_state=self.vc_state if (full and self.rgb) else None, **mode)
diff --git a/gsplatloc_amd/csrc/fused_project.hip b/gsplatloc_amd/csrc/fused_project.hip
--- a/gsplatloc_amd/csrc/fused_project.hip
+++ b/gsplatloc_amd/csrc/fused_project.hip
@@ -73,12 +73,8 @@
       p.covar = quat_scale_to_covar(q, s);
       p.covar_c = mul_bt(mul(cam.R, p.covar), cam.R);
       persp_mid(cam, W, H, p);
-      float a, b, c;
-      cov2d_from(p.J, p.covar_c, a, b, c);
-      float det_orig = a * c - b * b;
-      a += eps2d;
-      c += eps2d;
-      float det = a * c - b * b;
+      float a, b, c, det_orig, det;
+      blurred_cov2d(p, eps2d, a, b, c, det_orig, det);
       if (det > 0.f) {
         float bb = 0.5f * (a + c);
         float v1 = bb + sqrtf(fmaxf(0.01f, bb * bb - det));
@@ -88,12 +84,12 @@
         bool ok = rad > radius_clip;
         ok = ok && !(mx + rad <= 0.f || mx - rad >= (float)W || my + rad <= 0.f || my - rad >= (float)H);
         if (ok) {
-          float inv = 1.f / det;
           radius = (int)rad;
           comp = sqrtf(fmaxf(0.f, det_orig / det));
           float op = op_in;
           if (antialiased) op *= comp;
-          float ca = c * inv, cb = -b * inv, cc = a * inv;
+          float ca, cb, cc;
+          conic_of(a, b, c, det, ca, cb, cc);
           o0 = make_float4(mx, my, p.mc[2], op);
           o1 = make_float4(ca, cb, cc, cull_radius(ca, cb, cc, op));
         }
@@ -246,10 +242,10 @@
                      int32_t* tile_offsets, int64_t capacity, uint64_t* sort_keys, int32_t* flatten_ids,
                      int64_t* isect_ids, void* ws, size_t ws_bytes, int write_sorted_keys, void* bins, int bin_cap,
                      int32_t* n_isects, int32_t* flags, int long_min, const int32_t* order_ids,
-                     const int32_t* storage_of, bool clear, float* rows, void* stream) {
+                     const int32_t* storage_of, bool clear, float* rows, int row_pitch, void* stream) {
   if (N < 0 || tile_w <= 0 || tile_h <= 0 || ty0 < 0 || ty1 > tile_h || ty0 > ty1 || capacity < 0)
     return GSL_ERR_BAD_ARG;
-  if (clear && (N > GSL_MAX_GAUSSIANS || (N > 0 && !rows))) return GSL_ERR_BAD_ARG;
+  if (clear && (N > GSL_MAX_GAUSSIANS || (N > 0 && !rows) || !gsl::row_pitch_ok(row_pitch, 0))) return GSL_ERR_BAD_ARG;
   if (!clear || N == 0) rows = nullptr;
   const int n_rows = rows ? N : 0;
   int n_tiles = tile_w * tile_h, nst = (ty1 - ty0) * tile_w;
@@ -260,10 +256,10 @@
     if (capacity > 0 && (!sort_keys || !flatten_ids)) return GSL_ERR_BAD_ARG;
     return gsl::tile_sort_keys(tile_offsets, 0, n_tiles, capacity, sort_keys, flatten_ids, isect_ids, 0,
                                write_sorted_keys, (uint64_t*)bins, bin_cap, (const int32_t*)ws, n_isects, flags,
-                               write_sorted_keys ? 0 : long_min, nst, storage_of, rows, n_rows, stream);
+                               write_sorted_keys ? 0 : long_min, nst, storage_of, rows, n_rows, row_pitch, stream);
   }
   if (N == 0 || capacity == 0 || nst == 0)
-    return rows ? gsl::zero_u32(rows, (size_t)16 * (size_t)N, (hipStream_t)stream) : GSL_OK;
+    return rows ? gsl::zero_u32(rows, (size_t)row_pitch * (size_t)N, (hipStream_t)stream) : GSL_OK;
   if (!Q0 || !radii || !sort_keys || !flatten_ids) return GSL_ERR_BAD_ARG;
   if (!ws || ws_bytes < gsl_fused_ws_bytes(N, n_tiles)) return GSL_ERR_WORKSPACE;
   hipStream_t st = (hipStream_t)stream;
@@ -273,7 +269,7 @@
   GSL_CHECK_LAUNCH();
   return gsl::tile_sort_keys(tile_offsets, ty0 * tile_w, nst, capacity, sort_keys, flatten_ids, isect_ids, 0,
                              write_sorted_keys, nullptr, 0, nullptr, nullptr, nullptr, 0, 0, storage_of, rows, n_rows,
-                             stream);
+                             row_pitch, stream);
 }
 }
 
@@ -285,7 +281,7 @@
   (void)tile_n_bits;
   return gsl::fused_bin(Q0, radii, N, tile_w, tile_h, ty0, ty1, tile_offsets, capacity, sort_keys, flatten_ids, isect_ids,
                         ws, ws_bytes, write_sorted_keys, bins, bin_cap, n_isects, flags, long_min, order_ids, storage_of,
-                        false, nullptr, stream);
+                        false, nullptr, 16, stream);
 }
 
 extern "C" int gsl_fused_bin_clear(const float* Q0, const int32_t* radii, int N, int tile_w, int tile_h, int ty0, int ty1,
@@ -297,10 +293,26 @@
   (void)tile_n_bits;
   return gsl::fused_bin(Q0, radii, N, tile_w, tile_h, ty0, ty1, tile_offsets, capacity, sort_keys, flatten_ids, isect_ids,
                         ws, ws_bytes, write_sorted_keys, bins, bin_cap, n_isects, flags, long_min, order_ids, storage_of,
-                        true, rows, stream);
+                        true, rows, 16, stream);
+}
+
+extern "C" int gsl_fused_bin_clear_pitch(const float* Q0, const int32_t* radii, int N, int tile_w, int tile_h, int ty0,
+                                         int ty1, int tile_n_bits, int32_t* tile_offsets, int64_t capacity,
+                                         uint64_t* sort_keys, int32_t* flatten_ids, int64_t* isect_ids, void* ws,
+                                         size_t ws_bytes, int write_sorted_keys, void* bins, int bin_cap,
+                                         int32_t* n_isects, int32_t* flags, int long_min, const int32_t* order_ids,
+                                         const int32_t* storage_of, float* rows, int row_pitch, void* stream) {
+  (void)tile_n_bits;
+  return gsl::fused_bin(Q0, radii, N, tile_w, tile_h, ty0, ty1, tile_offsets, capacity, sort_keys, flatten_ids, isect_ids,
+                        ws, ws_bytes, write_sorted_keys, bins, bin_cap, n_isects, flags, long_min, order_ids, storage_of,
+                        true, rows, row_pitch, stream);
 }
 
 extern "C" int gsl_fused_clear_rows(float* rows, int N, void* stream) {
-  if (N < 0 || (N > 0 && !rows)) return GSL_ERR_BAD_ARG;
-  return gsl::zero_u32(rows, (size_t)16 * (size_t)N, (hipStream_t)stream);
-}
+  return gsl_fused_clear_rows_pitch(rows, N, 16, stream);
+}
+
+extern "C" int gsl_fused_clear_rows_pitch(float* rows, int N, int row_pitch, void* stream) {
+  if (N < 0 || N > GSL_MAX_GAUSSIANS || (N > 0 && !rows) || !gsl::row_pitch_ok(row_pitch, 0)) return GSL_ERR_BAD_ARG;
+  return gsl::zero_u32(rows, (size_t)row_pitch * (size_t)N, (hipStream_t)stream);
+}
diff --git a/gsplatloc_amd/csrc/fused_project_bwd.hip b/gsplatloc_amd/csrc/fused_project_bwd.hip
--- a/gsplatloc_amd/csrc/fused_project_bwd.hip
+++ b/gsplatloc_amd/csrc/fused_project_bwd.hip
@@ -7,17 +7,40 @@
 
 namespace gsl {
 
+template <int D, bool CLEAR>
+__device__ __forceinline__ void take_row(float* __restrict__ vacc, size_t i, int pitch, float4& r0, float4& r1, float4& r2) {
+  if (pitch == 16) {
+    float4* row = reinterpret_cast<float4*>(vacc) + 4 * i;
+    r0 = row[0]; r1 = row[1]; r2 = row[2];
+    if (CLEAR) { const float4 z = make_float4(0.f, 0.f, 0.f, 0.f); row[0] = z; row[1] = z; row[2] = z; }
+  } else {
+    constexpr int P2 = (6 + D + 1) / 2;
+    float2* row = reinterpret_cast<float2*>(vacc) + P2 * i;
+    float2 v[5];
+#pragma unroll
+    for (int k = 0; k < 5; ++k) v[k] = (k < P2) ? row[k] : make_float2(0.f, 0.f);
+    r0 = make_float4(v[0].x, v[0].y, v[1].x, v[1].y);
+    r1 = make_float4(v[2].x, v[2].y, v[3].x, v[3].y);
+    r2 = make_float4(v[4].x, v[4].y, 0.f, 0.f);
+    if (CLEAR) {
+#pragma unroll
+      for (int k = 0; k < P2; ++k) row[k] = make_float2(0.f, 0.f);
+    }
+  }
+}
+
 template <bool FULL, int D, bool KEEP>
 __global__ __launch_bounds__(256) void k_fproject_bwd(
     const float* __restrict__ means, const float* __restrict__ quats, const float* __restrict__ scales,
     const float* __restrict__ opacities, const float* __restrict__ colors, int sh_degree, int K_sh,
     const float* __restrict__ V, const float* __restrict__ Kmat, int N, int W, int H, float eps2d, int antialiased,
     const int32_t* __restrict__ radii, const float4* __restrict__ Q1, const float* __restrict__ comps,
-    float4* __restrict__ vacc, float* __restrict__ v_means, float* __restrict__ v_quats,
+    float* __restrict__ vacc, float* __restrict__ v_means, float* __restrict__ v_quats,
     float* __restrict__ v_scales, float* __restrict__ v_opacities, float* __restrict__ v_colors,
     float* __restrict__ partials, const float4* __restrict__ vrow, const uint64_t* __restrict__ skeys,
     const int32_t* __restrict__ tile_offsets, const float4* __restrict__ Q0, int tile_w, int tile_h, int ty0, int ty1,
-    long long capacity, float4* __restrict__ trec, const float* __restrict__ vcT, int32_t* __restrict__ vc_state) {
+    long long capacity, float4* __restrict__ trec, const float* __restrict__ vcT, int32_t* __restrict__ vc_state,
+    int pitch) {
   constexpr bool RGB = D >= 3;
   int i = blockIdx.x * 256 + threadIdx.x;
   Cam cam = load_cam(V, Kmat);
@@ -87,18 +110,19 @@
     } else if (trec) {
       r0 = srow[threadIdx.x][0]; r1 = srow[threadIdx.x][1]; r2 = srow[threadIdx.x][2];
       if (vacc) {
-        float4 a = vacc[4 * (size_t)i], b = vacc[4 * (size_t)i + 1], c = vacc[4 * (size_t)i + 2];
+        float4 a, b, c;
+        take_row<D, false>(vacc, (size_t)i, pitch, a, b, c);
         if (a.x != 0.f || a.y != 0.f || a.z != 0.f || a.w != 0.f || b.x != 0.f || b.y != 0.f || b.z != 0.f || b.w != 0.f ||
             c.x != 0.f || c.y != 0.f || c.z != 0.f || c.w != 0.f) {
           r0.x += a.x; r0.y += a.y; r0.z += a.z; r0.w += a.w;
           r1.x += b.x; r1.y += b.y; r1.z += b.z; r1.w += b.w;
           r2.x += c.x; r2.y += c.y; r2.z += c.z; r2.w += c.w;
-          vacc[4 * (size_t)i] = z; vacc[4 * (size_t)i + 1] = z; vacc[4 * (size_t)i + 2] = z;
+          float4 t0, t1, t2;
+          take_row<D, true>(vacc, (size_t)i, pitch, t0, t1, t2);
         }
       }
     } else {
-      r0 = vacc[4 * (size_t)i]; r1 = vacc[4 * (size_t)i + 1]; r2 = vacc[4 * (size_t)i + 2];
-      if (!KEEP) { vacc[4 * (size_t)i] = z; vacc[4 * (size_t)i + 1] = z; vacc[4 * (size_t)i + 2] = z; }
+      take_row<D, !KEEP>(vacc, (size_t)i, pitch, r0, r1, r2);
     }
     float vm2x = r0.x, vm2y = r0.y, v_ca = r0.z, v_cb = r0.w, v_cc = r1.x, vop_eff = r1.y;
     float col[4] = {r1.z, r1.w, r2.x, r2.y};
@@ -117,8 +141,16 @@
     p.covar = quat_scale_to_covar(q, s);
     p.covar_c = mul_bt(mul(cam.R, p.covar), cam.R);
     persp_mid(cam, W, H, p);
-    float4 q1 = GSL_Q(Q1, i);
-    project_vjp<FULL>(cam, eps2d, p, q, s, q1.x, q1.y, q1.z, vm2x, vm2y, vdepth, v_ca, v_cb, v_cc, antialiased != 0,
+    float ca, cb, cc;
+    if (Q1) {
+      float4 q1 = GSL_Q(Q1, i);
+      ca = q1.x; cb = q1.y; cc = q1.z;
+    } else {
+      float a2, b2, c2, det_orig, det;
+      blurred_cov2d(p, eps2d, a2, b2, c2, det_orig, det);
+      conic_of(a2, b2, c2, det, ca, cb, cc);
+    }
+    project_vjp<FULL>(cam, eps2d, p, q, s, ca, cb, cc, vm2x, vm2y, vdepth, v_ca, v_cb, v_cc, antialiased != 0,
                       comp, vcomp, acc15, vmean, vq, vs);
     sh_live = RGB && (sh_degree >= 0) && (vrgb[0] != 0.f || vrgb[1] != 0.f || vrgb[2] != 0.f);
     if (sh_live) {
@@ -247,9 +279,10 @@
                              size_t ws_bytes, int n_tiles, const float* vrow, const uint64_t* sorted_keys,
                              const int32_t* tile_offsets, const float* Q0, int tile_w, int tile_h, int ty0, int ty1,
                              int64_t capacity, float* tiny_trec, const float* tiny_vcT, int reduce_viewmat,
-                             int32_t* v_colors_state, bool keep, void* stream) {
+                             int32_t* v_colors_state, bool keep, int row_pitch, bool no_q1_ok, void* stream) {
   if (N < 0 || width <= 0 || height <= 0 || n_tiles <= 0) return GSL_ERR_BAD_ARG;
   if (keep && (vrow || tiny_trec || (N > 0 && !vacc))) return GSL_ERR_BAD_ARG;
+  if (!gsl::row_pitch_ok(row_pitch, channels)) return GSL_ERR_BAD_ARG;
   if (reduce_viewmat && !v_viewmat) return GSL_ERR_BAD_ARG;
   if (channels != 1 && channels != 3 && channels != 4) return GSL_ERR_BAD_ARG;
   bool full = v_means != nullptr;
@@ -262,7 +295,8 @@
     if (reduce_viewmat && gsl::zero_u32(v_viewmat, 16, st) != GSL_OK) return GSL_ERR_HIP;
     return GSL_OK;
   }
-  if (!means || !quats || !scales || !opacities || !viewmat || !K || !radii || !Q1) return GSL_ERR_BAD_ARG;
+  if (!means || !quats || !scales || !opacities || !viewmat || !K || !radii) return GSL_ERR_BAD_ARG;
+  if (!Q1 && (!no_q1_ok || tiny_trec)) return GSL_ERR_BAD_ARG;
   if (!vrow && !vacc && !tiny_trec) return GSL_ERR_BAD_ARG;
   if (tiny_trec && (!tiny_vcT || !Q0 || vrow)) return GSL_ERR_BAD_ARG;
   if (vrow && (!sorted_keys || !tile_offsets || !Q0 || tile_w <= 0 || tile_h <= 0 || tile_w * tile_h != n_tiles ||
@@ -278,9 +312,9 @@
     auto kern = keep ? gsl::k_fproject_bwd<FF, DD, true> : gsl::k_fproject_bwd<FF, DD, false>;                        \
     hipLaunchKernelGGL(kern, dim3(grid), dim3(256), 0, st, means, quats, scales, opacities, colors, sh_degree, K_sh,  \
                        viewmat, K, N, width, height, eps2d, antialiased, radii, (const float4*)Q1, compensations,     \
-                       (float4*)vacc, v_means, v_quats, v_scales, v_opacities, v_colors, partials,                    \
+                       vacc, v_means, v_quats, v_scales, v_opacities, v_colors, partials,                             \
                        (const float4*)vrow, sorted_keys, tile_offsets, (const float4*)Q0, tile_w, tile_h, ty0, ty1,   \
-                       (long long)capacity, (float4*)tiny_trec, tiny_vcT, vcs);                                       \
+                       (long long)capacity, (float4*)tiny_trec, tiny_vcT, vcs, row_pitch);                            \
   } while (0)
   if (full) {
     if (channels == 1) CALL_PB(true, 1); else if (channels == 3) CALL_PB(true, 3); else CALL_PB(true, 4);
@@ -310,17 +344,20 @@
       float *v_means, float *v_quats, float *v_scales, float *v_opacities, float *v_colors, float *v_viewmat,         \
       void *ws, size_t ws_bytes, int n_tiles, const float *vrow, const uint64_t *sorted_keys,                         \
       const int32_t *tile_offsets, const float *Q0, int tile_w, int tile_h, int ty0, int ty1, int64_t capacity,       \
-      float *tiny_trec, const float *tiny_vcT, int reduce_viewmat, int32_t *v_colors_state, void *stream
-#define GSL_PROJECT_BWD_ARGS(KEEP)                                                                                    \
+      float *tiny_trec, const float *tiny_vcT, int reduce_viewmat, int32_t *v_colors_state
+#define GSL_PROJECT_BWD_ARGS(KEEP, PITCH, NO_Q1)                                                                      \
   means, quats, scales, opacities, colors, sh_degree, K_sh, viewmat, K, N, width, height, eps2d, antialiased,         \
       channels, radii, Q1, compensations, vacc, v_means, v_quats, v_scales, v_opacities, v_colors, v_viewmat, ws,     \
       ws_bytes, n_tiles, vrow, sorted_keys, tile_offsets, Q0, tile_w, tile_h, ty0, ty1, capacity, tiny_trec,          \
-      tiny_vcT, reduce_viewmat, v_colors_state, KEEP, stream
-extern "C" int gsl_fused_project_bwd(GSL_PROJECT_BWD_PARAMS) {
-  return gsl::fused_project_bwd(GSL_PROJECT_BWD_ARGS(false));
-}
-extern "C" int gsl_fused_project_bwd_keep(GSL_PROJECT_BWD_PARAMS) {
-  return gsl::fused_project_bwd(GSL_PROJECT_BWD_ARGS(true));
+      tiny_vcT, reduce_viewmat, v_colors_state, KEEP, PITCH, NO_Q1, stream
+extern "C" int gsl_fused_project_bwd(GSL_PROJECT_BWD_PARAMS, void* stream) {
+  return gsl::fused_project_bwd(GSL_PROJECT_BWD_ARGS(false, 16, false));
+}
+extern "C" int gsl_fused_project_bwd_keep(GSL_PROJECT_BWD_PARAMS, void* stream) {
+  return gsl::fused_project_bwd(GSL_PROJECT_BWD_ARGS(true, 16, false));
+}
+extern "C" int gsl_fused_project_bwd_pitch(GSL_PROJECT_BWD_PARAMS, int keep, int row_pitch, void* stream) {
+  return gsl::fused_project_bwd(GSL_PROJECT_BWD_ARGS(keep != 0, row_pitch, true));
 }
 #undef GSL_PROJECT_BWD_PARAMS
 #undef GSL_PROJECT_BWD_ARGS
diff --git a/gsplatloc_amd/csrc/gsloc_internal.h b/gsplatloc_amd/csrc/gsloc_internal.h
--- a/gsplatloc_amd/csrc/gsloc_internal.h
+++ b/gsplatloc_amd/csrc/gsloc_internal.h
@@ -19,7 +19,7 @@
 int tile_sort_keys(int32_t* tile_offsets, int tile_begin, int n_strip_tiles, int64_t capacity, uint64_t* sort_keys,
                    int32_t* flatten_ids, int64_t* isect_ids, int64_t cam_enc, int write_sorted_keys, uint64_t* bins,
                    int bin_cap, const int32_t* counts, int32_t* n_isects, int32_t* flags, int long_min, int occupied_tiles,
-                   const int32_t* storage_of, float* clear_rows, int clear_n, void* stream);
+                   const int32_t* storage_of, float* clear_rows, int clear_n, int clear_pitch, void* stream);
 
 void launch_long_map(hipStream_t st, const int32_t* tile_offsets, int tile_begin, int n_strip_tiles, long long capacity,
                      int long_min, int max_seg, int max_list, const LongWs& w);
@@ -56,6 +56,12 @@
   return Qh || (Q0 && Q1 && (channels < 3 || Q2));
 }
 static inline bool ed_ok(int channels, int ed) { return !(ed && channels == 3); }
+static inline int dense_row_pitch(int channels) { return (6 + channels + 1) & ~1; }
+static inline bool row_pitch_ok(int pitch, int channels) {
+  if (pitch == 16) return true;
+  if (channels == 0) return pitch == dense_row_pitch(1) || pitch == dense_row_pitch(4);
+  return (channels == 1 || channels == 3 || channels == 4) && pitch == dense_row_pitch(channels);
+}
 
 }
 
diff --git a/gsplatloc_amd/csrc/project_dev.h b/gsplatloc_amd/csrc/project_dev.h
--- a/gsplatloc_amd/csrc/project_dev.h
+++ b/gsplatloc_amd/csrc/project_dev.h
@@ -48,6 +48,19 @@
   c = r1[0] * J[3] + r1[1] * J[4] + r1[2] * J[5];
 }
 
+__device__ __forceinline__ void blurred_cov2d(const ProjMid& p, float eps2d, float& a, float& b, float& c, float& det_orig,
+                                              float& det) {
+  cov2d_from(p.J, p.covar_c, a, b, c);
+  det_orig = a * c - b * b;
+  a += eps2d;
+  c += eps2d;
+  det = a * c - b * b;
+}
+__device__ __forceinline__ void conic_of(float a, float b, float c, float det, float& ca, float& cb, float& cc) {
+  float inv = 1.f / det;
+  ca = c * inv; cb = -b * inv; cc = a * inv;
+}
+
 __device__ __forceinline__ void load_gaussian(const float* __restrict__ means, const float* __restrict__ quats,
                                               const float* __restrict__ scales, int i, const Cam& cam,
                                               ProjMid& p, float q[4], float s[3]) {
@@ -74,12 +87,8 @@
     p.covar = quat_scale_to_covar(q, s);
     p.covar_c = mul_bt(mul(cam.R, p.covar), cam.R);
     persp_mid(cam, W, H, p);
-    float a, b, c;
-    cov2d_from(p.J, p.covar_c, a, b, c);
-    float det_orig = a * c - b * b;
-    a += eps2d;
-    c += eps2d;
-    float det = a * c - b * b;
+    float a, b, c, det_orig, det;
+    blurred_cov2d(p, eps2d, a, b, c, det_orig, det);
     if (det > 0.f) {
       float bb = 0.5f * (a + c);
       float v1 = bb + sqrtf(fmaxf(0.01f, bb * bb - det));
@@ -89,10 +98,9 @@
       bool ok = radius > radius_clip;
       ok = ok && !(mx + radius <= 0.f || mx - radius >= (float)W || my + radius <= 0.f || my - radius >= (float)H);
       if (ok) {
-        float inv = 1.f / det;
         o.radius = (int)radius;
         o.mx = mx; o.my = my; o.depth = p.mc[2];
-        o.ca = c * inv; o.cb = -b * inv; o.cc = a * inv;
+        conic_of(a, b, c, det, o.ca, o.cb, o.cc);
         o.comp = sqrtf(fmaxf(0.f, det_orig / det));
       }
     }
diff --git a/gsplatloc_amd/csrc/raster_g16.hip b/gsplatloc_amd/csrc/raster_g16.hip
--- a/gsplatloc_amd/csrc/raster_g16.hip
+++ b/gsplatloc_amd/csrc/raster_g16.hip
@@ -123,7 +123,7 @@
   uint8_t nzlist[64];
 };
 
-template <int D, int CG>
+template <int D, int CG, bool DENSE>
 __device__ __forceinline__ void qraster_bwd_body(
     QStage<D, CG>& sb, const float4* __restrict__ Q0, const float4* __restrict__ Q1, const float4* __restrict__ Q2,
     const uint4* __restrict__ Qh, const int32_t* __restrict__ flatten_ids, float* __restrict__ vacc, long long rs,
@@ -219,7 +219,7 @@
         cnt[g] += __popcll(Bg);
       }
       if (__builtin_amdgcn_inverse_ballot_w64(R)) {
-        sb.id[slot] = gid;
+        sb.id[slot] = (int32_t)((unsigned)gid * (DENSE ? 4u * (unsigned)((A + 1) & ~1) : 64u));
         sb.s0[slot] = r0;
         const float3 cn = stage_conic(r1);
         sb.s1[slot] = make_float4(cn.x, cn.y, cn.z, __int_as_float((int)idx));
@@ -410,7 +410,7 @@
         int gi = i0 + arow;
         if (gi < cntz && arow < RPI) {
           int sl = sb.nzlist[gi];
-          const unsigned off = ((unsigned)sb.id[sl + 64 * u] << 6) | ((unsigned)f << 2);
+          const unsigned off = (unsigned)sb.id[sl + 64 * u] + ((unsigned)f << 2);
           atomicAdd(reinterpret_cast<float*>(reinterpret_cast<char*>(vacc) + off), packed[sl * PP + f]);
         }
       }
@@ -419,7 +419,7 @@
   }
 }
 
-template <int D, bool ED, int CG, bool LONG>
+template <int D, bool ED, int CG, bool LONG, bool DENSE>
 __device__ __forceinline__ void qraster_bwd_item(
     QStage<D, CG>& sb, int b, int n_items, const float4* __restrict__ Q0, const float4* __restrict__ Q1,
     const float4* __restrict__ Q2, int W, int H, int tile_w, int ty0, const int32_t* __restrict__ tile_offsets,
@@ -507,28 +507,45 @@
     qh = isect_hits + 4 * list.rs + (long long)quad * (list.re - list.rs);
     if (nqh == 0) return;
   }
-  qraster_bwd_body<D, CG>(sb, Q0, Q1, Q2, Qh, flatten_ids, vacc, sp.rs, sp.re, lane, quad, tp.px, tp.py, (float)(tp.txi * 16),
+  qraster_bwd_body<D, CG, DENSE>(sb, Q0, Q1, Q2, Qh, flatten_ids, vacc, sp.rs, sp.re, lane, quad, tp.px, tp.py, (float)(tp.txi * 16),
                           (float)(tp.tyi * 16), bin_final, T_init, Bp_init, vc, qh, nqh);
 }
 
-template <int D, bool ED, int CG, bool LONG>
-__global__ __launch_bounds__(64) void k_qraster_bwd(
-    const float4* __restrict__ Q0, const float4* __restrict__ Q1, const float4* __restrict__ Q2, int W, int H,
-    int tile_w, int ty0, const int32_t* __restrict__ tile_offsets, const int32_t* __restrict__ flatten_ids,
-    long long capacity, const float* __restrict__ render, const float* __restrict__ alphas,
-    const int32_t* __restrict__ last_ids, const float* __restrict__ v_render, const float* __restrict__ v_alphas,
-    float* __restrict__ vacc, int row0, int row1, const uint4* __restrict__ Qh,
-    const uint32_t* __restrict__ isect_hits, int32_t* __restrict__ isect_hit_counts, int long_min, LongWs lw,
-    int32_t* __restrict__ rgb_flag, int32_t* __restrict__ clear_counts, int32_t* __restrict__ clear_state, int n_items) {
-  __shared__ QStage<D, CG> sb;
+#define GSL_QBWD_PARAMS                                                                                                \
+  const float4 *__restrict__ Q0, const float4 *__restrict__ Q1, const float4 *__restrict__ Q2, int W, int H,          \
+      int tile_w, int ty0, const int32_t *__restrict__ tile_offsets, const int32_t *__restrict__ flatten_ids,         \
+      long long capacity, const float *__restrict__ render, const float *__restrict__ alphas,                         \
+      const int32_t *__restrict__ last_ids, const float *__restrict__ v_render, const float *__restrict__ v_alphas,   \
+      float *__restrict__ vacc, int row0, int row1, const uint4 *__restrict__ Qh,                                     \
+      const uint32_t *__restrict__ isect_hits, int32_t *__restrict__ isect_hit_counts, int long_min, LongWs lw,       \
+      int32_t *__restrict__ rgb_flag, int32_t *__restrict__ clear_counts, int32_t *__restrict__ clear_state,          \
+      int n_items
+template <int D, bool ED, int CG, bool LONG, bool DENSE>
+__device__ __forceinline__ void qraster_bwd_items(QStage<D, CG>& sb, GSL_QBWD_PARAMS) {
   if (D == 4 && CG == D && rgb_flag && *rgb_flag == 0) return;
   for (int b = (int)blockIdx.x; b < n_items; b += (int)gridDim.x) {
-    qraster_bwd_item<D, ED, CG, LONG>(sb, b, n_items, Q0, Q1, Q2, W, H, tile_w, ty0, tile_offsets, flatten_ids, capacity,
-                                      render, alphas, last_ids, v_render, v_alphas, vacc, row0, row1, Qh, isect_hits,
-                                      isect_hit_counts, long_min, lw, rgb_flag, clear_counts, clear_state);
+    qraster_bwd_item<D, ED, CG, LONG, DENSE>(sb, b, n_items, Q0, Q1, Q2, W, H, tile_w, ty0, tile_offsets, flatten_ids,
+                                             capacity, render, alphas, last_ids, v_render, v_alphas, vacc, row0, row1, Qh,
+                                             isect_hits, isect_hit_counts, long_min, lw, rgb_flag, clear_counts,
+                                             clear_state);
     __syncthreads();
   }
 }
+#define GSL_QBWD_ARGS                                                                                                 \
+  Q0, Q1, Q2, W, H, tile_w, ty0, tile_offsets, flatten_ids, capacity, render, alphas, last_ids, v_render, v_alphas,  \
+      vacc, row0, row1, Qh, isect_hits, isect_hit_counts, long_min, lw, rgb_flag, clear_counts, clear_state, n_items
+template <int D, bool ED, int CG, bool LONG>
+__global__ __launch_bounds__(64) void k_qraster_bwd(GSL_QBWD_PARAMS) {
+  __shared__ QStage<D, CG> sb;
+  qraster_bwd_items<D, ED, CG, LONG, false>(sb, GSL_QBWD_ARGS);
+}
+template <int D, bool ED, int CG, bool LONG>
+__global__ __launch_bounds__(64) void k_qraster_bwd_dense(GSL_QBWD_PARAMS) {
+  __shared__ QStage<D, CG> sb;
+  qraster_bwd_items<D, ED, CG, LONG, true>(sb, GSL_QBWD_ARGS);
+}
+#undef GSL_QBWD_PARAMS
+#undef GSL_QBWD_ARGS
 
 }
 
@@ -547,7 +564,7 @@
                                  int height, int tile_w, int ty0, int ty1, const int32_t* tile_offsets,
                                  const int32_t* flatten_ids, int64_t capacity, const float* render,
                                  const float* alphas, const int32_t* last_ids, const float* v_render,
-                                 const float* v_alphas, float* vacc, int row0, int row1, const void* Qh,
+                                 const float* v_alphas, float* vacc, int row_pitch, int row0, int row1, const void* Qh,
                                  const uint32_t* isect_hits, const int32_t* isect_hit_counts, int long_min,
                                  void* long_ws, int max_seg, int rgb_flag_index, void* clear_ws, void* stream) {
   hipStream_t st = (hipStream_t)stream;
@@ -557,8 +574,10 @@
   int32_t* rgb_flag = isect_hit_counts ? const_cast<int32_t*>(isect_hit_counts) + rgb_flag_index : nullptr;
   int32_t* clear_counts = (int32_t*)clear_ws;
   int32_t* clear_state = gsl::fused_bin_state(clear_ws, rgb_flag_index / 4);
+  const bool dense = row_pitch != 16;
 #define CALL_QL(DD, EE, CC, LL)                                                                                  \
-  hipLaunchKernelGGL((gsl::k_qraster_bwd<DD, EE, CC, LL>), dim3(grid), dim3(64), 0, st, (const float4*)Q0,       \
+  hipLaunchKernelGGL((dense ? gsl::k_qraster_bwd_dense<DD, EE, CC, LL> : gsl::k_qraster_bwd<DD, EE, CC, LL>),    \
+                     dim3(grid), dim3(64), 0, st, (const float4*)Q0,                                             \
                      (const float4*)Q1, (const float4*)Q2, width, height, tile_w, ty0, tile_offsets, flatten_ids, \
                      (long long)capacity, render, alphas, last_ids, v_render, v_alphas, vacc, row0, row1,         \
                      (const uint4*)Qh, isect_hits, const_cast<int32_t*>(isect_hit_counts), long_min, lw, rgb_flag, \
@@ -578,16 +597,15 @@
   return GSL_OK;
 }
 
-extern "C" int gsl_fused_raster_bwd(const float* Q0, const float* Q1, const float* Q2, int channels, int ed,
-                                   int width, int height, int tile_w, int tile_h, int ty0, int ty1,
-                                   const int32_t* tile_offsets, const int32_t* flatten_ids, int64_t capacity,
-                                   const float* render, const float* alphas, const int32_t* last_ids,
-                                   const float* v_render, const float* v_alphas, float* vacc, int row0, int row1,
-                                   const void* Qh, float* vrow, const uint32_t* isect_hits,
-                                   const int32_t* isect_hit_counts, int long_min, void* clear_ws, void* stream) {
+static int fused_raster_bwd(const float* Q0, const float* Q1, const float* Q2, int channels, int ed, int width, int height,
+                            int tile_w, int tile_h, int ty0, int ty1, const int32_t* tile_offsets,
+                            const int32_t* flatten_ids, int64_t capacity, const float* render, const float* alphas,
+                            const int32_t* last_ids, const float* v_render, const float* v_alphas, float* vacc, int row0,
+                            int row1, const void* Qh, float* vrow, const uint32_t* isect_hits,
+                            const int32_t* isect_hit_counts, int long_min, void* clear_ws, int row_pitch, void* stream) {
   if (!gsl::frame_ok(width, height, tile_w, tile_h, ty0, ty1, capacity, row0, row1)) return GSL_ERR_BAD_ARG;
   if (!tile_offsets || !render || !alphas || !last_ids || !v_render || !v_alphas) return GSL_ERR_BAD_ARG;
-  if (!gsl::ed_ok(channels, ed)) return GSL_ERR_BAD_ARG;
+  if (!gsl::ed_ok(channels, ed) || !gsl::row_pitch_ok(row_pitch, channels)) return GSL_ERR_BAD_ARG;
   if (capacity == 0 || ty0 == ty1 || row0 == row1) return GSL_OK;
   if (!flatten_ids || (!vacc && !vrow)) return GSL_ERR_BAD_ARG;
   if (isect_hits && !isect_hit_counts) return GSL_ERR_BAD_ARG;
@@ -598,26 +616,61 @@
                                    capacity, render, alphas, last_ids, v_render, v_alphas, vrow, row0, row1, Qh,
                                    (hipStream_t)stream);
   return g16_raster_bwd_launch(Q0, Q1, Q2, channels, ed, width, height, tile_w, ty0, ty1, tile_offsets, flatten_ids,
-                               capacity, render, alphas, last_ids, v_render, v_alphas, vacc, row0, row1, Qh,
-                               isect_hits, isect_hit_counts, long_min, nullptr, 0, 4 * tile_w * tile_h, clear_ws,
-                                   stream);
-}
-
-extern "C" int gsl_long_raster_bwd(const float* Q0, const float* Q1, const float* Q2, int channels, int ed, int width,
-                                   int height, int tile_w, int tile_h, int ty0, int ty1, const int32_t* tile_offsets,
-                                   const int32_t* flatten_ids, int64_t capacity, const float* render,
-                                   const float* alphas, const int32_t* last_ids, const float* v_render,
-                                   const float* v_alphas, float* vacc, int row0, int row1, const void* Qh,
-                                   const uint32_t* isect_hits, int long_min, void* long_ws, int max_seg,
-                                   void* stream) {
+                               capacity, render, alphas, last_ids, v_render, v_alphas, vacc, row_pitch, row0, row1, Qh,
+                               isect_hits, isect_hit_counts, long_min, nullptr, 0, 4 * tile_w * tile_h, clear_ws, stream);
+}
+
+#define GSL_RASTER_BWD_PARAMS                                                                                          \
+  const float *Q0, const float *Q1, const float *Q2, int channels, int ed, int width, int height, int tile_w,         \
+      int tile_h, int ty0, int ty1, const int32_t *tile_offsets, const int32_t *flatten_ids, int64_t capacity,        \
+      const float *render, const float *alphas, const int32_t *last_ids, const float *v_render,                       \
+      const float *v_alphas, float *vacc, int row0, int row1, const void *Qh, float *vrow,                            \
+      const uint32_t *isect_hits, const int32_t *isect_hit_counts, int long_min, void *clear_ws
+#define GSL_RASTER_BWD_ARGS                                                                                            \
+  Q0, Q1, Q2, channels, ed, width, height, tile_w, tile_h, ty0, ty1, tile_offsets, flatten_ids, capacity, render,     \
+      alphas, last_ids, v_render, v_alphas, vacc, row0, row1, Qh, vrow, isect_hits, isect_hit_counts, long_min,       \
+      clear_ws
+extern "C" int gsl_fused_raster_bwd(GSL_RASTER_BWD_PARAMS, void* stream) {
+  return fused_raster_bwd(GSL_RASTER_BWD_ARGS, 16, stream);
+}
+extern "C" int gsl_fused_raster_bwd_pitch(GSL_RASTER_BWD_PARAMS, int row_pitch, void* stream) {
+  return fused_raster_bwd(GSL_RASTER_BWD_ARGS, row_pitch, stream);
+}
+#undef GSL_RASTER_BWD_PARAMS
+#undef GSL_RASTER_BWD_ARGS
+
+static int long_raster_bwd(const float* Q0, const float* Q1, const float* Q2, int channels, int ed, int width, int height,
+                           int tile_w, int tile_h, int ty0, int ty1, const int32_t* tile_offsets,
+                           const int32_t* flatten_ids, int64_t capacity, const float* render, const float* alphas,
+                           const int32_t* last_ids, const float* v_render, const float* v_alphas, float* vacc, int row0,
+                           int row1, const void* Qh, const uint32_t* isect_hits, int long_min, void* long_ws, int max_seg,
+                           int row_pitch, void* stream) {
   if (!gsl::frame_ok(width, height, tile_w, tile_h, ty0, ty1, capacity, row0, row1, false) || long_min <= 0 ||
       max_seg <= 0 || !long_ws)
     return GSL_ERR_BAD_ARG;
   if (!tile_offsets || !render || !alphas || !last_ids || !v_render || !v_alphas || !vacc) return GSL_ERR_BAD_ARG;
-  if (!gsl::ed_ok(channels, ed)) return GSL_ERR_BAD_ARG;
+  if (!gsl::ed_ok(channels, ed) || !gsl::row_pitch_ok(row_pitch, channels)) return GSL_ERR_BAD_ARG;
   if (capacity == 0 || ty0 == ty1 || row0 == row1) return GSL_OK;
   if (!flatten_ids || !gsl::records_ok(Qh, Q0, Q1, Q2, channels)) return GSL_ERR_BAD_ARG;
   return g16_raster_bwd_launch(Q0, Q1, Q2, channels, ed, width, height, tile_w, ty0, ty1, tile_offsets, flatten_ids,
-                               capacity, render, alphas, last_ids, v_render, v_alphas, vacc, row0, row1, Qh,
+                               capacity, render, alphas, last_ids, v_render, v_alphas, vacc, row_pitch, row0, row1, Qh,
                                isect_hits, nullptr, long_min, long_ws, max_seg, 0, nullptr, stream);
 }
+
+#define GSL_LONG_BWD_PARAMS                                                                                            \
+  const float *Q0, const float *Q1, const float *Q2, int channels, int ed, int width, int height, int tile_w,         \
+      int tile_h, int ty0, int ty1, const int32_t *tile_offsets, const int32_t *flatten_ids, int64_t capacity,        \
+      const float *render, const float *alphas, const int32_t *last_ids, const float *v_render,                       \
+      const float *v_alphas, float *vacc, int row0, int row1, const void *Qh, const uint32_t *isect_hits,             \
+      int long_min, void *long_ws, int max_seg
+#define GSL_LONG_BWD_ARGS                                                                                              \
+  Q0, Q1, Q2, channels, ed, width, height, tile_w, tile_h, ty0, ty1, tile_offsets, flatten_ids, capacity, render,     \
+      alphas, last_ids, v_render, v_alphas, vacc, row0, row1, Qh, isect_hits, long_min, long_ws, max_seg
+extern "C" int gsl_long_raster_bwd(GSL_LONG_BWD_PARAMS, void* stream) {
+  return long_raster_bwd(GSL_LONG_BWD_ARGS, 16, stream);
+}
+extern "C" int gsl_long_raster_bwd_pitch(GSL_LONG_BWD_PARAMS, int row_pitch, void* stream) {
+  return long_raster_bwd(GSL_LONG_BWD_ARGS, row_pitch, stream);
+}
+#undef GSL_LONG_BWD_PARAMS
+#undef GSL_LONG_BWD_ARGS
diff --git a/gsplatloc_amd/csrc/sort_dev.h b/gsplatloc_amd/csrc/sort_dev.h
--- a/gsplatloc_amd/csrc/sort_dev.h
+++ b/gsplatloc_amd/csrc/sort_dev.h
@@ -161,11 +161,12 @@
 
 struct RowClear {
   float4* rows;
-  int n4, per;
+  int n4, per, tail;
   __device__ __forceinline__ void run(int part, int t, int width) const {
     const int b = part * per, e = min(n4, b + per);
     const float4 z = make_float4(0.f, 0.f, 0.f, 0.f);
     for (int i = b + t; i < e; i += width) rows[i] = z;
+    if (tail && t == 0 && b < n4 && e == n4) *reinterpret_cast<float2*>(rows + n4) = make_float2(0.f, 0.f);
   }
 };
 __device__ __forceinline__ void keys_arrived() { __builtin_amdgcn_s_waitcnt(0x0F70); }
@@ -186,7 +187,7 @@
                                              uint64_t* __restrict__ lds, uint64_t* __restrict__ keys_out,
                                              int32_t* __restrict__ flatten_ids, int64_t* __restrict__ isect_ids,
                                              int64_t cam_enc, const int32_t* __restrict__ storage_of = nullptr,
-                                             const RowClear clr = RowClear{nullptr, 0, 0}, int clr_part = 0) {
+                                             const RowClear clr = RowClear{nullptr, 0, 0, 0}, int clr_part = 0) {
   constexpr int KPT = 1 << LK, RUN = 64 * KPT;
   const int lane = tid & 63, wv = tid >> 6;
   uint64_t k[KPT];
diff --git a/gsplatloc_amd/csrc/tile_sort.hip b/gsplatloc_amd/csrc/tile_sort.hip
--- a/gsplatloc_amd/csrc/tile_sort.hip
+++ b/gsplatloc_amd/csrc/tile_sort.hip
@@ -398,19 +398,21 @@
   if (n_strip_tiles == 0 || capacity == 0) return GSL_OK;
   if (!sort_keys || !flatten_ids) return GSL_ERR_BAD_ARG;
   return gsl::tile_sort_keys(const_cast<int32_t*>(tile_offsets), tile_begin, n_strip_tiles, capacity, sort_keys, flatten_ids,
-                             isect_ids, cam_enc, 0, nullptr, 0, nullptr, nullptr, nullptr, 0, 0, nullptr, nullptr, 0, stream);
+                             isect_ids, cam_enc, 0, nullptr, 0, nullptr, nullptr, nullptr, 0, 0, nullptr, nullptr, 0, 16, stream);
 }
 
 int gsl::tile_sort_keys(int32_t* tile_offsets, int tile_begin, int n_strip_tiles, int64_t capacity, uint64_t* sort_keys,
                         int32_t* flatten_ids, int64_t* isect_ids, int64_t cam_enc, int write_sorted_keys, uint64_t* bins,
                         int bin_cap, const int32_t* counts, int32_t* n_isects, int32_t* flags, int long_min,
-                        int occupied_tiles, const int32_t* storage_of, float* clear_rows, int clear_n, void* stream) {
+                        int occupied_tiles, const int32_t* storage_of, float* clear_rows, int clear_n, int clear_pitch,
+                        void* stream) {
   if (!tile_offsets || tile_begin < 0 || n_strip_tiles < 0 || capacity < 0) return GSL_ERR_BAD_ARG;
   if (counts && (!bins || tile_begin != 0)) return GSL_ERR_BAD_ARG;
   if (clear_n < 0 || clear_n > GSL_MAX_GAUSSIANS || (clear_n > 0 && !clear_rows)) return GSL_ERR_BAD_ARG;
+  if (!gsl::row_pitch_ok(clear_pitch, 0)) return GSL_ERR_BAD_ARG;
   if (clear_n == 0) clear_rows = nullptr;
   if (n_strip_tiles == 0 || (capacity == 0 && !counts))
-    return clear_rows ? gsl::zero_u32(clear_rows, (size_t)16 * (size_t)clear_n, (hipStream_t)stream) : GSL_OK;
+    return clear_rows ? gsl::zero_u32(clear_rows, (size_t)clear_pitch * (size_t)clear_n, (hipStream_t)stream) : GSL_OK;
   if (capacity > 0 && (!sort_keys || !flatten_ids)) return GSL_ERR_BAD_ARG;
   const int occ = occupied_tiles > 0 ? occupied_tiles : n_strip_tiles;
   const long long mean_list = capacity / (long long)occ;
@@ -422,8 +424,8 @@
   else if (!(force && !strcmp(force, "wave")) && mean_list > 320 && occ <= 2048) variant = 2;
   else variant = mean_list <= 1150 ? 0 : 1;
   const int parts = variant == 2 ? n_strip_tiles : (n_strip_tiles + 3) / 4 * 4, width = variant == 2 ? 256 : 64;
-  const int n4 = 4 * clear_n;
-  const gsl::RowClear clr{(float4*)clear_rows, n4, ((n4 + parts - 1) / parts + width - 1) / width * width};
+  const int n_floats = clear_pitch * clear_n, n4 = n_floats / 4;
+  const gsl::RowClear clr{(float4*)clear_rows, n4, ((n4 + parts - 1) / parts + width - 1) / width * width, n_floats & 3};
   auto launch = [&](auto kernel, int tiles_per_wg) {
     hipLaunchKernelGGL(kernel, dim3((n_strip_tiles + tiles_per_wg - 1) / tiles_per_wg), dim3(256), 0, (hipStream_t)stream,
                        tile_offsets, tile_begin, n_strip_tiles, (long long)capacity, sort_keys, flatten_ids, isect_ids,
diff --git a/gsplatloc_amd/stages.py b/gsplatloc_amd/stages.py
--- a/gsplatloc_amd/stages.py
+++ b/gsplatloc_amd/stages.py
@@ -8,6 +8,21 @@
 
 MAX_STRIP_TILES = 8192
 _MODES = {"RGB": (3, False), "D": (1, False), "ED": (1, True), "RGB+D": (4, False), "RGB+ED": (4, True)}
+
+
+def pitch_of(rows) -> int:
+    shape = getattr(rows, "shape", None)
+    return int(shape[1]) if shape is not None and len(shape) == 2 else 16
+
+
+def _dense(name, sibling, *args, **modes):
+    try:
+        sibling(*args, **modes)
+    except RuntimeError as err:
+        what, sep, rest = str(err).partition(" failed: ")
+        if not sep:
+            raise
+        raise RuntimeError(f"{what} for {name} failed: {rest}") from None
 
 
 def tile_n_bits(n_tiles: int) -> int:
@@ -44,6 +59,11 @@
 def fused_bin_clear(Q0, radii, N, tile_w, tile_h, ty0, ty1, tile_n_bits, tile_offsets, capacity, sort_keys, flatten_ids, ws,
                     rows, *, isect_ids=None, write_sorted_keys=0, bins=None, bin_cap=0, n_isects=None, flags=None,
                     long_min=0, order_ids=None, storage_of=None):
+    if pitch_of(rows) != 16:
+        return _dense("gsl_fused_bin_clear", fused_bin_clear_pitch, Q0, radii, N, tile_w, tile_h, ty0, ty1, tile_n_bits,
+                      tile_offsets, capacity, sort_keys, flatten_ids, ws, rows, pitch_of(rows), isect_ids=isect_ids,
+                      write_sorted_keys=write_sorted_keys, bins=bins, bin_cap=bin_cap, n_isects=n_isects, flags=flags,
+                      long_min=long_min, order_ids=order_ids, storage_of=storage_of)
     check(load_library().gsl_fused_bin_clear(
         Q0.data_ptr(), radii.data_ptr(), N, tile_w, tile_h, ty0, ty1, tile_n_bits, tile_offsets.data_ptr(), capacity,
         sort_keys.data_ptr(), ptr(flatten_ids), ptr(isect_ids), ws.data_ptr(), ws.numel(), write_sorted_keys, ptr(bins),
@@ -51,8 +71,25 @@
         "gsl_fused_bin_clear")
 
 
+def fused_bin_clear_pitch(Q0, radii, N, tile_w, tile_h, ty0, ty1, tile_n_bits, tile_offsets, capacity, sort_keys,
+                          flatten_ids, ws, rows, row_pitch, *, isect_ids=None, write_sorted_keys=0, bins=None, bin_cap=0,
+                          n_isects=None, flags=None, long_min=0, order_ids=None, storage_of=None):
+    check(load_library().gsl_fused_bin_clear_pitch(
+        Q0.data_ptr(), radii.data_ptr(), N, tile_w, tile_h, ty0, ty1, tile_n_bits, tile_offsets.data_ptr(), capacity,
+        sort_keys.data_ptr(), ptr(flatten_ids), ptr(isect_ids), ws.data_ptr(), ws.numel(), write_sorted_keys, ptr(bins),
+        bin_cap, ptr(n_isects), ptr(flags), long_min, ptr(order_ids), ptr(storage_of), ptr(rows), row_pitch,
+        current_stream()), "gsl_fused_bin_clear_pitch")
+
+
 def fused_clear_rows(rows, N):
+    if pitch_of(rows) != 16:
+        return _dense("gsl_fused_clear_rows", fused_clear_rows_pitch, rows, N, pitch_of(rows))
     check(load_library().gsl_fused_clear_rows(ptr(rows), N, current_stream()), "gsl_fused_clear_rows")
+
+
+def fused_clear_rows_pitch(rows, N, row_pitch):
+    check(load_library().gsl_fused_clear_rows_pitch(ptr(rows), N, row_pitch, current_stream()),
+          "gsl_fused_clear_rows_pitch")
 
 
 def fused_raster_fwd(Q0, Q1, Q2, channels, ed, width, height, tile_w, tile_h, ty0, ty1, tile_offsets, flatten_ids, capacity,
@@ -68,11 +105,26 @@
 def fused_raster_bwd(Q0, Q1, Q2, channels, ed, width, height, tile_w, tile_h, ty0, ty1, tile_offsets, flatten_ids, capacity,
                      render, alphas, last_ids, v_render, v_alphas, vacc, row0, row1, *, Qh=None, vrow=None, isect_hits=None,
                      isect_hit_counts=None, long_min=0, clear_ws=None):
+    if pitch_of(vacc) != 16:
+        return _dense("gsl_fused_raster_bwd", fused_raster_bwd_pitch, Q0, Q1, Q2, channels, ed, width, height, tile_w,
+                      tile_h, ty0, ty1, tile_offsets, flatten_ids, capacity, render, alphas, last_ids, v_render, v_alphas,
+                      vacc, row0, row1, pitch_of(vacc), Qh=Qh, vrow=vrow, isect_hits=isect_hits,
+                      isect_hit_counts=isect_hit_counts, long_min=long_min, clear_ws=clear_ws)
     check(load_library().gsl_fused_raster_bwd(
         ptr(Q0), ptr(Q1), ptr(Q2), channels, ed, width, height, tile_w, tile_h, ty0, ty1, tile_offsets.data_ptr(),
         ptr(flatten_ids), capacity, render.data_ptr(), alphas.data_ptr(), last_ids.data_ptr(), v_render.data_ptr(),
         v_alphas.data_ptr(), ptr(vacc), row0, row1, ptr(Qh), ptr(vrow), ptr(isect_hits), ptr(isect_hit_counts), long_min,
         ptr(clear_ws), current_stream()), "gsl_fused_raster_bwd")
+
+
+def fused_raster_bwd_pitch(Q0, Q1, Q2, channels, ed, width, height, tile_w, tile_h, ty0, ty1, tile_offsets, flatten_ids,
+                           capacity, render, alphas, last_ids, v_render, v_alphas, vacc, row0, row1, row_pitch, *, Qh=None,
+                           vrow=None, isect_hits=None, isect_hit_counts=None, long_min=0, clear_ws=None):
+    check(load_library().gsl_fused_raster_bwd_pitch(
+        ptr(Q0), ptr(Q1), ptr(Q2), channels, ed, width, height, tile_w, tile_h, ty0, ty1, tile_offsets.data_ptr(),
+        ptr(flatten_ids), capacity, render.data_ptr(), alphas.data_ptr(), last_ids.data_ptr(), v_render.data_ptr(),
+        v_alphas.data_ptr(), ptr(vacc), row0, row1, ptr(Qh), ptr(vrow), ptr(isect_hits), ptr(isect_hit_counts), long_min,
+        ptr(clear_ws), row_pitch, current_stream()), "gsl_fused_raster_bwd_pitch")
 
 
 def tiny_raster_bwd(Q0, Q1, Q2, channels, ed, width, height, tile_w, tile_h, ty0, ty1, tile_offsets, flatten_ids, capacity,
@@ -105,11 +157,25 @@
 def long_raster_bwd(Q0, Q1, Q2, channels, ed, width, height, tile_w, tile_h, ty0, ty1, tile_offsets, flatten_ids, capacity,
                     render, alphas, last_ids, v_render, v_alphas, vacc, row0, row1, long_min, long_ws, max_seg, *, Qh=None,
                     isect_hits=None):
+    if pitch_of(vacc) != 16:
+        return _dense("gsl_long_raster_bwd", long_raster_bwd_pitch, Q0, Q1, Q2, channels, ed, width, height, tile_w, tile_h,
+                      ty0, ty1, tile_offsets, flatten_ids, capacity, render, alphas, last_ids, v_render, v_alphas, vacc,
+                      row0, row1, long_min, long_ws, max_seg, pitch_of(vacc), Qh=Qh, isect_hits=isect_hits)
     check(load_library().gsl_long_raster_bwd(
         ptr(Q0), ptr(Q1), ptr(Q2), channels, ed, width, height, tile_w, tile_h, ty0, ty1, tile_offsets.data_ptr(),
         flatten_ids.data_ptr(), capacity, render.data_ptr(), alphas.data_ptr(), last_ids.data_ptr(), v_render.data_ptr(),
         v_alphas.data_ptr(), vacc.data_ptr(), row0, row1, ptr(Qh), ptr(isect_hits), long_min, long_ws.data_ptr(), max_seg,
         current_stream()), "gsl_long_raster_bwd")
+
+
+def long_raster_bwd_pitch(Q0, Q1, Q2, channels, ed, width, height, tile_w, tile_h, ty0, ty1, tile_offsets, flatten_ids,
+                          capacity, render, alphas, last_ids, v_render, v_alphas, vacc, row0, row1, long_min, long_ws,
+                          max_seg, row_pitch, *, Qh=None, isect_hits=None):
+    check(load_library().gsl_long_raster_bwd_pitch(
+        ptr(Q0), ptr(Q1), ptr(Q2), channels, ed, width, height, tile_w, tile_h, ty0, ty1, tile_offsets.data_ptr(),
+        flatten_ids.data_ptr(), capacity, render.data_ptr(), alphas.data_ptr(), last_ids.data_ptr(), v_render.data_ptr(),
+        v_alphas.data_ptr(), vacc.data_ptr(), row0, row1, ptr(Qh), ptr(isect_hits), long_min, long_ws.data_ptr(), max_seg,
+        row_pitch, current_stream()), "gsl_long_raster_bwd_pitch")
 
 
 def fused_project_bwd(means, quats, scales, opacities, colors, sh_degree, K_sh, viewmat, K, N, width, height, eps2d,
@@ -117,6 +183,13 @@
                       v_colors, v_viewmat, ws, n_tiles, reduce_viewmat, *, vrow=None, sorted_keys=None, tile_offsets=None,
                       Q0=None, tile_w=0, tile_h=0, ty0=0, ty1=0, capacity=0, tiny_trec=None, tiny_vcT=None,
                       v_colors_state=None):
+    if pitch_of(vacc) != 16 or Q1 is None:
+        return _dense("gsl_fused_project_bwd", fused_project_bwd_pitch, means, quats, scales, opacities, colors, sh_degree,
+                      K_sh, viewmat, K, N, width, height, eps2d, antialiased, channels, radii, Q1, compensations, vacc,
+                      v_means, v_quats, v_scales, v_opacities, v_colors, v_viewmat, ws, n_tiles, reduce_viewmat, 0,
+                      pitch_of(vacc), vrow=vrow, sorted_keys=sorted_keys, tile_offsets=tile_offsets, Q0=Q0, tile_w=tile_w,
+                      tile_h=tile_h, ty0=ty0, ty1=ty1, capacity=capacity, tiny_trec=tiny_trec, tiny_vcT=tiny_vcT,
+                      v_colors_state=v_colors_state)
     check(load_library().gsl_fused_project_bwd(
         means.data_ptr(), quats.data_ptr(), scales.data_ptr(), opacities.data_ptr(), ptr(colors), sh_degree, K_sh,
         viewmat.data_ptr(), K.data_ptr(), N, width, height, eps2d, antialiased, channels, radii.data_ptr(), Q1.data_ptr(),
@@ -131,6 +204,13 @@
                            v_colors, v_viewmat, ws, n_tiles, reduce_viewmat, *, vrow=None, sorted_keys=None,
                            tile_offsets=None, Q0=None, tile_w=0, tile_h=0, ty0=0, ty1=0, capacity=0, tiny_trec=None,
                            tiny_vcT=None, v_colors_state=None):
+    if pitch_of(vacc) != 16 or Q1 is None:
+        return _dense("gsl_fused_project_bwd_keep", fused_project_bwd_pitch, means, quats, scales, opacities, colors,
+                      sh_degree, K_sh, viewmat, K, N, width, height, eps2d, antialiased, channels, radii, Q1, compensations,
+                      vacc, v_means, v_quats, v_scales, v_opacities, v_colors, v_viewmat, ws, n_tiles, reduce_viewmat, 1,
+                      pitch_of(vacc), vrow=vrow, sorted_keys=sorted_keys, tile_offsets=tile_offsets, Q0=Q0, tile_w=tile_w,
+                      tile_h=tile_h, ty0=ty0, ty1=ty1, capacity=capacity, tiny_trec=tiny_trec, tiny_vcT=tiny_vcT,
+                      v_colors_state=v_colors_state)
     check(load_library().gsl_fused_project_bwd_keep(
         means.data_ptr(), quats.data_ptr(), scales.data_ptr(), opacities.data_ptr(), ptr(colors), sh_degree, K_sh,
         viewmat.data_ptr(), K.data_ptr(), N, width, height, eps2d, antialiased, channels, radii.data_ptr(), Q1.data_ptr(),
@@ -138,6 +218,20 @@
         ptr(v_viewmat), ws.data_ptr(), ws.numel(), n_tiles, ptr(vrow), ptr(sorted_keys), ptr(tile_offsets), ptr(Q0), tile_w,
         tile_h, ty0, ty1, capacity, ptr(tiny_trec), ptr(tiny_vcT), reduce_viewmat, ptr(v_colors_state), current_stream()),
         "gsl_fused_project_bwd_keep")
+
+
+def fused_project_bwd_pitch(means, quats, scales, opacities, colors, sh_degree, K_sh, viewmat, K, N, width, height, eps2d,
+                            antialiased, channels, radii, Q1, compensations, vacc, v_means, v_quats, v_scales,
+                            v_opacities, v_colors, v_viewmat, ws, n_tiles, reduce_viewmat, keep, row_pitch, *, vrow=None,
+                            sorted_keys=None, tile_offsets=None, Q0=None, tile_w=0, tile_h=0, ty0=0, ty1=0, capacity=0,
+                            tiny_trec=None, tiny_vcT=None, v_colors_state=None):
+    check(load_library().gsl_fused_project_bwd_pitch(
+        means.data_ptr(), quats.data_ptr(), scales.data_ptr(), opacities.data_ptr(), ptr(colors), sh_degree, K_sh,
+        viewmat.data_ptr(), K.data_ptr(), N, width, height, eps2d, antialiased, channels, radii.data_ptr(), ptr(Q1),
+        ptr(compensations), ptr(vacc), ptr(v_means), ptr(v_quats), ptr(v_scales), ptr(v_opacities), ptr(v_colors),
+        ptr(v_viewmat), ws.data_ptr(), ws.numel(), n_tiles, ptr(vrow), ptr(sorted_keys), ptr(tile_offsets), ptr(Q0), tile_w,
+        tile_h, ty0, ty1, capacity, ptr(tiny_trec), ptr(tiny_vcT), reduce_viewmat, ptr(v_colors_state), keep, row_pitch,
+        current_stream()), "gsl_fused_project_bwd_pitch")
 
 
 def fused_absgrad(Q0, Q1, Q2, channels, ed, width, height, tile_w, tile_h, tile_offsets, flatten_ids, capacity, render,
diff --git a/include/gsloc_hip.h b/include/gsloc_hip.h
--- a/include/gsloc_hip.h
+++ b/include/gsloc_hip.h
@@ -307,6 +307,38 @@
                                const uint64_t* sorted_keys, const int32_t* tile_offsets, const float* Q0, int tile_w,
                                int tile_h, int ty0, int ty1, int64_t capacity, float* tiny_trec, const float* tiny_vcT,
                                int reduce_viewmat, int32_t* v_colors_state, void* stream);
+int gsl_fused_bin_clear_pitch(const float* Q0, const int32_t* radii, int N, int tile_w, int tile_h, int ty0,
+                              int ty1, int tile_n_bits, int32_t* tile_offsets, int64_t capacity,
+                              uint64_t* sort_keys, int32_t* flatten_ids, int64_t* isect_ids, void* ws,
+                              size_t ws_bytes, int write_sorted_keys, void* bins, int bin_cap, int32_t* n_isects,
+                              int32_t* flags, int long_min, const int32_t* order_ids, const int32_t* storage_of,
+                              float* rows, int row_pitch, void* stream);
+int gsl_fused_clear_rows_pitch(float* rows, int N, int row_pitch, void* stream);
+int gsl_fused_raster_bwd_pitch(const float* Q0, const float* Q1, const float* Q2, int channels, int ed,
+                               int width, int height, int tile_w, int tile_h, int ty0, int ty1,
+                               const int32_t* tile_offsets, const int32_t* flatten_ids, int64_t capacity,
+                               const float* render, const float* alphas, const int32_t* last_ids,
+                               const float* v_render, const float* v_alphas, float* vacc, int row0, int row1,
+                               const void* Qh, float* vrow, const uint32_t* isect_hits,
+                               const int32_t* isect_hit_counts, int long_min, void* clear_ws, int row_pitch,
+                               void* stream);
+int gsl_long_raster_bwd_pitch(const float* Q0, const float* Q1, const float* Q2, int channels, int ed, int width,
+                              int height, int tile_w, int tile_h, int ty0, int ty1, const int32_t* tile_offsets,
+                              const int32_t* flatten_ids, int64_t capacity, const float* render,
+                              const float* alphas, const int32_t* last_ids, const float* v_render,
+                              const float* v_alphas, float* vacc, int row0, int row1, const void* Qh,
+                              const uint32_t* isect_hits, int long_min, void* long_ws, int max_seg, int row_pitch,
+                              void* stream);
+int gsl_fused_project_bwd_pitch(const float* means, const float* quats, const float* scales,
+                                const float* opacities, const float* colors, int sh_degree, int K_sh,
+                                const float* viewmat, const float* K, int N, int width, int height,
+                                float eps2d, int antialiased, int channels, const int32_t* radii,
+                                const float* Q1, const float* compensations, float* vacc, float* v_means,
+                                float* v_quats, float* v_scales, float* v_opacities, float* v_colors,
+                                float* v_viewmat, void* ws, size_t ws_bytes, int n_tiles, const float* vrow,
+                                const uint64_t* sorted_keys, const int32_t* tile_offsets, const float* Q0, int tile_w,
+                                int tile_h, int ty0, int ty1, int64_t capacity, float* tiny_trec, const float* tiny_vcT,
+                                int reduce_viewmat, int32_t* v_colors_state, int keep, int row_pitch, void* stream);
 const float* gsl_fused_viewmat_rows(const void* ws, int n_tiles);
 
 int gsl_tiny_raster_bwd(const float* Q0, const float* Q1, const float* Q2, int channels, int ed,
```

Result: no change. 2.499 billion (median of 3 runs) (+0.4%).
